# PaddlePaddle/PaddleRec

Measured on AMD Instinct MI355X. Metric: CTR samples/sec, Criteo DeepFM bs=65536 (train step: fwd+bwd+optimizer), higher is better.
Workload: dtype f32 (MLP GEMMs: f32 operands as 3 bf16 terms, 6 bf16 MFMAs per product, f32 accumulate); 1 GPU; DeepFM full Criteo: 26 sparse slots x 1000000 rows x dim 16, 13 dense, MLP 400,400,400, batch 65536 per GPU, lazy Adam, uniform ids; global_batch=65536, parallelism=single, table_rows_total=26000000, index_oob_flag=0

## Files before the change

include/recengine.h:

```cpp
#ifndef RECENGINE_H_
#define RECENGINE_H_

#include <stddef.h>
#include <stdint.h>

#ifdef __cplusplus
extern "C" {
#endif

typedef enum {
  REC_OK = 0,
  REC_EINVAL = -1,
  REC_ESHAPE = -2,
  REC_EWORKSPACE = -3,
  REC_EHIP = -4,
  REC_ENCCL = -5
} rec_status;

#define REC_FLAG_INDEX_OOB 1
#define REC_FLAG_EXCHANGE_OVERFLOW 2

const char* rec_last_error(void);
int rec_version(void);

// ... 220 lines not shown

int rec_adam_rows_all_l2(int64_t num_rows, int32_t emb_dim, int32_t row_stride, int32_t state_stride,
                         const int32_t* n_uniq, const int64_t* uniq_rows, const int32_t* seg_offset,
                         const int32_t* sorted_pos, const float* grad, const rec_grad_layout* grad_layout,
                         const float* grad_scale, float* P, float* M, float* V, const rec_adam_hyper* hyper,
                         float l2_coeff, void* stream);

int rec_adam_record_all(int64_t num_rows, int32_t emb_dim, int32_t rec_stride, int32_t state_stride,
                        int32_t v_offset, const int32_t* n_uniq, const int64_t* uniq_rows,
                        const int32_t* seg_offset, const int32_t* sorted_pos, const float* grad,
                        const rec_grad_layout* grad_layout, const float* grad1,
                        const rec_grad_layout* grad1_layout, const float* grad_scale, float* rec, float* MV,
                        const rec_adam_hyper* hyper, void* stream);

int rec_adam_dense(int64_t n, float* p, float* m, float* v, const float* g, const float* grad_scale,
                   const rec_adam_hyper* hyper, void* stream);

int rec_sumsq_workspace_bytes(size_t* bytes);
int rec_sumsq(int64_t n, const float* x, float* out, int32_t accumulate, void* workspace,
              size_t workspace_bytes, void* stream);
int rec_sparse_rows_sumsq(int64_t n_max, int32_t emb_dim, const int32_t* n_uniq,
                          const int32_t* seg_offset, const int32_t* sorted_pos, const float* grad,
                          const rec_grad_layout* grad_layout, float* out, int32_t accumulate,
                          void* workspace, size_t workspace_bytes, void* stream);
int rec_clip_scale(const float* sumsq, float clip_norm, float* scale, void* stream);

int rec_cross_bwd_prep(int64_t m, int32_t n, const float* dX, int32_t ld_dx, const float* X0,
                       int32_t ld_x0, const float* U, int32_t ld_u, float* dU, int32_t ld_du,
                       float* dX0_acc, int32_t ld_acc, int32_t accumulate, void* stream);

typedef struct {
  int64_t batch;
  int32_t max_len;
  int32_t item_dim, cat_dim;
  int32_t hidden1, hidden2;
  int64_t item_rows, cat_rows;
  int32_t item_stride, cat_stride;
} rec_din_desc;

int rec_din_saves_act1(const rec_din_desc* desc);
int rec_din_attention_pool_fwd(const rec_din_desc* desc, const int64_t* hist_item,
                               const int64_t* hist_cat, const int64_t* tgt_item_seq,
                               const int64_t* tgt_cat_seq, const int64_t* mask,
                               const float* w_hist_item, const float* w_hist_cat,
                               const float* w_tgt_item_seq, const float* w_tgt_cat_seq,
                               const float* att_w1, const float* att_b1, const float* att_w2,
                               const float* att_b2, const float* att_w3, const float* att_b3,
                               float* out, float* att_weight, float* act1, int32_t* status, void* stream);
int rec_din_attention_pool_fwd_workspace_bytes(const rec_din_desc* desc, size_t* bytes);
int rec_din_attention_pool_fwd_ws(const rec_din_desc* desc, const int64_t* hist_item,
                                  const int64_t* hist_cat, const int64_t* tgt_item_seq,
                                  const int64_t* tgt_cat_seq, const int64_t* mask,
                                  const float* w_hist_item, const float* w_hist_cat,
                                  const float* w_tgt_item_seq, const float* w_tgt_cat_seq,
                                  const float* att_w1, const float* att_b1, const float* att_w2,
                                  const float* att_b2, const float* att_w3, const float* att_b3,
                                  float* out, float* att_weight, float* act1, int32_t* status, void* workspace,
                                  size_t workspace_bytes, void* stream);

int rec_din_attention_pool_bwd(const rec_din_desc* desc, const int64_t* hist_item,
                               const int64_t* hist_cat, const int64_t* tgt_item_seq,
                               const int64_t* tgt_cat_seq, const float* w_hist_item,
                               const float* w_hist_cat, const float* w_tgt_item_seq,
                               const float* w_tgt_cat_seq, const float* att_w1,
                               const float* att_w1_t, const float* att_b1, const float* att_w2,
                               const float* att_b2, const float* att_w3, const float* att_weight,
                               const float* out_saved, const float* act1_saved,
                               const float* d_out, float* d_hist, float* d_tgt_seq, void* stream);

int rec_din_attention_pool_bwd_workspace_bytes(const rec_din_desc* desc, size_t* bytes);
int rec_din_attention_pool_bwd_ws(const rec_din_desc* desc, const int64_t* hist_item,
                                  const int64_t* hist_cat, const int64_t* tgt_item_seq,
                                  const int64_t* tgt_cat_seq, const float* w_hist_item,
                                  const float* w_hist_cat, const float* w_tgt_item_seq,
                                  const float* w_tgt_cat_seq, const float* att_w1,
                                  const float* att_w1_t, const float* att_b1, const float* att_w2,
                                  const float* att_b2, const float* att_w3, const float* att_weight,
                                  const float* out_saved, const float* act1_saved,
                                  const float* d_out, float* d_hist, float* d_tgt_seq, void* workspace,
                                  size_t workspace_bytes, void* stream);

int rec_moe_bwd_prep(int64_t m, int32_t n, const float* dX, int32_t ld_dx, const float* X0,
                     int32_t ld_x0, const float* U, int32_t ld_u, const float* prob, int32_t prob_stride,
                     float* dU, int32_t ld_du, float* dX0_acc, int32_t ld_acc, int32_t accumulate,
                     float* dp, int32_t dp_stride, void* stream);
int rec_softmax_rows_bwd(int64_t m, int32_t n, const float* p, int32_t ldp, const float* dp,
                         int32_t lddp, float* dz, int32_t lddz, void* stream);

int rec_softmax_rows(int64_t m, int32_t n, const float* x, int32_t ldx, float* y, int32_t ldy,
                     void* stream);

typedef struct {
  int64_t stride_b;
  int32_t stride_j, stride_d;
} rec_cin_view;

int rec_cin_outer_fwd(int64_t batch, int32_t emb_dim, int32_t F, int32_t S, const float* X0,
                      const rec_cin_view* v0, const float* Xk, const rec_cin_view* vk, float* Z, int64_t ldz,
                      void* stream);
int rec_cin_outer_bwd(int64_t batch, int32_t emb_dim, int32_t F, int32_t S, const float* dZ, int64_t ldz,
                      const float* X0, const rec_cin_view* v0, const float* Xk, const rec_cin_view* vk,
                      float* dX0, const rec_cin_view* dv0, int32_t accumulate_dx0, float* dXk,
                      const rec_cin_view* dvk, int32_t accumulate_dxk, const float* dpool, int64_t ld_dpool,
                      void* stream);
int rec_cin_contract_fwd(int64_t batch, int32_t emb_dim, int32_t F, int32_t C, const float* Y, int64_t ldy,
                         const float* X0, const rec_cin_view* v0, float* XT, int64_t ldx, void* stream);
int rec_cin_contract_bwd(int64_t batch, int32_t emb_dim, int32_t F, int32_t C, const float* Y, int64_t ldy,
                         const float* dXT, int64_t ldx, const float* X0, const rec_cin_view* v0, float* dY,
                         int64_t lddy, float* dX0, const rec_cin_view* dv0, int32_t accumulate_dx0, void* stream);
int rec_cin_sumpool(int64_t batch, int32_t emb_dim, int32_t C, const float* XT, int64_t ldx, float* out,
                    int64_t ldo, void* stream);
int rec_cin_sumpool_bwd(int64_t batch, int32_t emb_dim, int32_t C, const float* dpool, int64_t ldp,
                        float* dXT, int64_t ldx, void* stream);

int rec_batchnorm_workspace_bytes(int64_t m, int32_t n, size_t* bytes);
int rec_batchnorm_fwd(int64_t m, int32_t n, const float* X, int64_t ldx, const float* gamma, const float* beta,
                      float* running_mean, float* running_var, float momentum, float eps, int32_t training,
                      float* Y, int64_t ldy, float* save_mean, float* save_invstd, void* workspace,
                      size_t workspace_bytes, void* stream);
int rec_batchnorm_bwd(int64_t m, int32_t n, const float* X, int64_t ldx, const float* dY, int64_t lddy,
                      const float* gamma, const float* save_mean, const float* save_invstd, int32_t relu_mask,
                      float* dX, int64_t lddx, float* dgamma, float* dbeta, void* workspace,
                      size_t workspace_bytes, void* stream);
int rec_dot_interact_fwd(int64_t batch, int32_t F, int32_t D, const float* T, int64_t ldt, float* R, int64_t ldr,
                         void* stream);
int rec_dot_interact_bwd(int64_t batch, int32_t F, int32_t D, const float* T, int64_t ldt, const float* dR,
                         int64_t ldr, float* dT, int64_t lddt, void* stream);
int rec_accuracy_count(int64_t n, const float* pred, const int64_t* label, int64_t* counts, void* stream);

typedef enum {
  REC_EPI_NONE = 0,
  REC_EPI_BIAS = 1,
  REC_EPI_BIAS_RELU = 2,
  REC_EPI_RELU_MASK = 3,
  REC_EPI_CROSS = 4,
  REC_EPI_BIAS_SIGMOID = 5,
  REC_EPI_BIAS_TANH = 6,
  REC_EPI_ADD = 7,
  REC_EPI_DTANH = 10,
  REC_EPI_DSIGMOID = 9,
  REC_EPI_MOE = 8
} rec_epilogue;

typedef struct {
  int64_t m;
  int32_t n, k;
  int32_t lda, ldb, ldc;
  int32_t trans_a, trans_b;
  int32_t epilogue;
  int32_t split_k;
  int32_t num_cus;
} rec_gemm_desc;

typedef struct {
  const float* bias;
  const float* aux0;
  int32_t ld_aux0;
  const float* aux1;
  int32_t ld_aux1;
  const float* row_scale;
  int32_t row_scale_stride;
  float* out2;
  int32_t ld_out2;
  float* b_colsum;
  const void* b_image;
  void* relu_bits;
} rec_gemm_epilogue_args;

int rec_gemm_f32_workspace_bytes(const rec_gemm_desc* desc, size_t* bytes);
int rec_gemm_relu_bits_bytes(const rec_gemm_desc* desc, int32_t* eligible, size_t* bytes);
int rec_gemm_plan_splits(const rec_gemm_desc* desc, int32_t num_cus, int32_t* splits);
int rec_gemm_f32(const rec_gemm_desc* desc, const float* A, const float* B, float* C,
                 const rec_gemm_epilogue_args* args , void* workspace,
                 size_t workspace_bytes, void* stream);
int rec_gemm_f32_pair(const rec_gemm_desc* desc0, const float* A0, const float* B0, float* C0,
                      const rec_gemm_epilogue_args* args0 , const rec_gemm_desc* desc1, const float* A1,
                      const float* B1, float* C1, const rec_gemm_epilogue_args* args1 , void* workspace,
                      size_t workspace_bytes, void* stream);
typedef enum {
  REC_GEMM_ROUTE_SKINNY_ROWS = 0,
  REC_GEMM_ROUTE_SKINNY_DW = 1,
  REC_GEMM_ROUTE_X3_DW = 2,
  REC_GEMM_ROUTE_X3 = 3,
  REC_GEMM_ROUTE_PANEL = 4,
  REC_GEMM_ROUTE_GLDS = 5,
  REC_GEMM_ROUTE_DIRECT = 6,
  REC_GEMM_ROUTE_TILED = 7
} rec_gemm_route_family;
enum {
  REC_GEMM_ROUTE_FAST = 1,
  REC_GEMM_ROUTE_PIPE = 2,
  REC_GEMM_ROUTE_VEC = 4,
  REC_GEMM_ROUTE_KS4 = 8,
  REC_GEMM_ROUTE_FOLD = 16,
  REC_GEMM_ROUTE_VEC_A = 32,
  REC_GEMM_ROUTE_PAIR = 64
};
typedef struct {
  int32_t family;
  int32_t cfg;
  int32_t splits;
  int32_t flags;
} rec_gemm_route;
int rec_gemm_last_route(rec_gemm_route* out);
typedef struct {
  const float* B;
  int32_t ldb, k, n, trans_b;
  void* image;
} rec_gemm_b_image;
int rec_gemm_b_image_bytes(int32_t k, int32_t n, int32_t* eligible, size_t* bytes);
int rec_gemm_b_images(int32_t count, const rec_gemm_b_image* items, void* stream);

int rec_colsum_workspace_bytes(int64_t m, int32_t n, size_t* bytes);
int rec_colsum(int64_t m, int32_t n, int32_t ld, const float* G, float* out, void* workspace,
               size_t workspace_bytes, void* stream);

typedef struct {
  int64_t batch;
  int32_t d;
  int32_t ld_x0, ld_xl, ld_out, ld_u;
} rec_crossnet_v2_desc;
int rec_crossnet_v2_layer_workspace_bytes(const rec_crossnet_v2_desc* desc, size_t* fwd_bytes, size_t* bwd_bytes);
int rec_crossnet_v2_layer_fwd(const rec_crossnet_v2_desc* desc, const float* X0, const float* Xl, const float* W,
                              const float* bias, float* Xnext, float* U_saved, void* workspace,
                              size_t workspace_bytes, void* stream);
int rec_crossnet_v2_layer_bwd(const rec_crossnet_v2_desc* desc, const float* X0, const float* Xl, const float* W,
                              const float* U_saved, const float* dXnext, int32_t ld_dxnext, float* dX0_acc,
                              int32_t ld_acc, int32_t accumulate_dx0, int32_t fold_dx0, float* dXl,
                              int32_t ld_dxl, float* dW, float* db, void* workspace, size_t workspace_bytes,
                              void* stream);

typedef struct {
  int64_t batch;
  int32_t d, rank, experts;
  int32_t ld_x0, ld_xl, ld_out;
} rec_crossnet_mix_desc;
int rec_crossnet_mix_layer_workspace_bytes(const rec_crossnet_mix_desc* desc, size_t* fwd_bytes, size_t* bwd_bytes);
int rec_crossnet_mix_layer_fwd(const rec_crossnet_mix_desc* desc, const float* X0, const float* Xl, const float* U,
                               const float* V, const float* C, const float* bias, const float* gate_w,
                               const float* gate_b, float* Xnext, float* t1, float* t2, float* prob,
                               void* workspace, size_t workspace_bytes, void* stream);
int rec_crossnet_mix_layer_bwd(const rec_crossnet_mix_desc* desc, const float* X0, const float* Xl, const float* U,
                               const float* V, const float* C, const float* bias, const float* gate_w,
                               const float* t1, const float* t2, const float* prob, const float* dXnext,
                               int32_t ld_dxnext, float* dX0_acc, int32_t ld_acc, int32_t accumulate_dx0,
                               int32_t fold_dx0, float* dXl, int32_t ld_dxl, float* gU, float* gV, float* gC,
                               float* gbias, float* g_gate_w, float* g_gate_b, int32_t accumulate_gate,
                               void* workspace, size_t workspace_bytes, void* stream);

int rec_logloss_workspace_bytes(int64_t batch, size_t* bytes);
int rec_sigmoid_logloss(int64_t batch, int64_t mean_over, const float* y1, const float* y2,
                        const float* y_dnn,
                        const int64_t* label, float eps, float clip_lo, float clip_hi, float* pred,
                        float* dz, float* loss_out, void* workspace, size_t workspace_bytes, void* stream);

int rec_bce_with_logits(int64_t batch, int64_t mean_over, const float* logit, const float* label,
                        float* pred, float* dz, float* loss_out, void* workspace, size_t workspace_bytes,
                        void* stream);

int rec_auc_histogram(int64_t batch, const float* pred, const int64_t* label,
                      int32_t num_thresholds, int64_t* stat_pos, int64_t* stat_neg, void* stream);

int rec_shard_route_workspace_bytes(int64_t n, int32_t num_shards, size_t* bytes);
int rec_shard_route(int64_t n, int32_t num_slots, int64_t num_rows, int64_t padding_idx,
                    int32_t num_shards, const int64_t* ids, const int64_t* slot_offset,
                    int64_t* send_local_row, int64_t* send_pos, int64_t* send_sample,
                    int64_t* slot_of_pos, int64_t* send_counts, int32_t* status, void* workspace,
                    size_t workspace_bytes, void* stream);

int rec_dedup_plan_workspace_bytes(int64_t n, int32_t num_shards, int64_t local_rows, size_t* bytes);
int rec_dedup_plan(int64_t n, int32_t num_slots, int64_t num_rows, int64_t padding_idx, int32_t num_shards,
                   int64_t local_rows, int32_t cap, const int64_t* ids, const int64_t* slot_offset, int32_t* sorted_pos,
                   int64_t* uniq_rows, int32_t* seg_offset, int32_t* n_uniq, int64_t* send_rows, int64_t* slot_of_pos,
                   int64_t* slot_of_uniq, int64_t* counts, int32_t* status, void* workspace, size_t workspace_bytes,
                   void* stream);

int rec_comm_unique_id(void* id128);
int rec_comm_init(const void* id128, int32_t world, int32_t rank, void** comm);
int rec_comm_destroy(void* comm);
int rec_comm_size(void* comm, int32_t* world);
int rec_comm_available(void);
int rec_alltoall_exchange(void* comm, const void* send, const int64_t* send_counts, void* recv,
                          const int64_t* recv_counts, int32_t row_bytes, void* stream);
int rec_allreduce_sum_f32(void* comm, float* buf, int64_t n, void* stream);

uint32_t rec_xxh32(const void* bytes, size_t len, uint32_t seed);
int rec_xxh32_hash_mod(const char* const* strings, const int32_t* field_idx, int64_t n,
                       uint32_t hash_dim, int64_t* out);

int rec_count_lines(const char* buf, size_t len, int32_t threads, int64_t* n_lines);
int rec_blank_lines(const char* buf, size_t len, int32_t threads, int64_t max_out, int64_t* idx, int64_t* n_blank);
int rec_csr_cut(int32_t num_slots, int32_t n_pieces, const int64_t* const* values, const int64_t* const* lod,
                const int64_t* lod_stride, const int64_t* const* base, const int64_t* l0, const int64_t* l1,
                int32_t threads, int64_t* out_values, int64_t max_values, int64_t* out_lod, int64_t* out_base);
int rec_count_byte(const char* buf, size_t len, int32_t byte, int32_t threads, int64_t* n);
int rec_parse_slot_text(const char* buf, size_t len, int32_t n_sparse, int32_t n_dense,
                        int32_t log1p_dense, int64_t max_lines, int32_t threads, int64_t* label,
                        int64_t* ids, float* dense, int64_t* n_lines);
int rec_parse_criteo_tsv(const char* buf, size_t len, int32_t n_dense, int32_t n_sparse,
                         const float* cont_min, const float* cont_diff, uint32_t hash_dim,
                         int64_t max_lines, int32_t threads, int64_t* label, int64_t* ids, float* dense,
                         int64_t* n_lines);

int rec_parse_feasign_slots(const char* buf, size_t len, int32_t first_slot, int32_t num_slots,
                            uint64_t hash_rows, int64_t max_lines, int64_t max_values, int32_t threads,
                            int64_t* values, int64_t* lod, int64_t* slot_base, int64_t* n_lines,
                            int64_t* n_values);

int rec_fill_uniform(int64_t n, float* buf, float lo, float hi, uint64_t seed, void* stream);

int rec_copy_async(void* dst, const void* src, size_t bytes, void* stream);
int rec_copy_2d_async(void* dst, size_t dst_pitch_bytes, const void* src, size_t src_pitch_bytes, size_t width_bytes,
                      size_t rows, void* stream);
int rec_transpose_f32(int64_t rows, int64_t cols, const float* in, float* out, void* stream);
int rec_cast_f32_i64(int64_t n, const float* src, int64_t src_stride, int64_t* dst, void* stream);

int rec_link_emulate(size_t bytes, float gbytes_per_s, float fixed_us, int32_t blocks, const void* src, void* dst,
                     size_t ring_bytes, void* stream);

int rec_stream_spin(int32_t micros, void* stream);
// ... 324 lines not shown
```

paddlerec_amd/_lib.py:

```python
import ctypes as C
import os

_HERE = os.path.dirname(os.path.abspath(__file__))
LIB_PATH = os.path.join(_HERE, "librecengine.so")

REC_FLAG_INDEX_OOB = 1
REC_FLAG_EXCHANGE_OVERFLOW = 2
REC_FLEN_MAX_GROUPS = 8
REC_AUTOFIS_MAX_FIELDS, REC_AUTOFIS_MAX_DIM, REC_AUTOFIS_MAX_PAIRS = 64, 64, 2016


class RecError(RuntimeError):
    pass


class DeepFMDesc(C.Structure):
    _fields_ = [("batch", C.c_int64), ("num_slots", C.c_int32), ("num_dense", C.c_int32),
                ("emb_dim", C.c_int32), ("row_stride", C.c_int32), ("num_rows", C.c_int64),
                ("padding_idx", C.c_int64), ("w1_stride", C.c_int32), ("compact_dense", C.c_int32),
                ("feat_stride", C.c_int64)]


class FFMDesc(C.Structure):
    _fields_ = [("batch", C.c_int64), ("num_slots", C.c_int32), ("num_dense", C.c_int32), ("dim", C.c_int32),
                ("num_rows", C.c_int64), ("row_stride", C.c_int32), ("grad_stride", C.c_int32)]


class FatFFMDesc(C.Structure):
    _fields_ = [("ffm", FFMDesc), ("ld_attn", C.c_int64), ("ld_pair", C.c_int64)]


class FEFMDesc(C.Structure):
    _fields_ = [("batch", C.c_int64), ("num_slots", C.c_int32), ("num_dense", C.c_int32), ("dim", C.c_int32),
                ("num_rows", C.c_int64), ("row_stride", C.c_int32), ("grad_stride", C.c_int32), ("ld", C.c_int64)]


class DcnCrossDesc(C.Structure):
    _fields_ = [("batch", C.c_int64), ("d", C.c_int32), ("num_layers", C.c_int32), ("ld_x0", C.c_int64),
                ("ld_out", C.c_int64), ("ld_dxl", C.c_int64), ("ld_dx0", C.c_int64), ("l2_coeff", C.c_float),
                ("accumulate_dx0", C.c_int32)]


class DeepFMNet(C.Structure):
    MAX_LINEAR = 8
    _fields_ = [("num_slots", C.c_int32), ("dim", C.c_int32), ("dense_dim", C.c_int32), ("n_linear", C.c_int32),
                ("widths", C.c_int32 * 8), ("table_rows", C.c_int64), ("num_rows", C.c_int64),
                ("padding_idx", C.c_int64), ("slot_rows", C.c_int64), ("slot_offset", C.c_void_p),
                ("rec", C.c_void_p), ("rec_stride", C.c_int32), ("mv", C.c_void_p), ("mv_stride", C.c_int32),
                ("v_offset", C.c_int32), ("dense_w", C.c_void_p), ("dense_w_one", C.c_void_p),
                ("g_dense_w", C.c_void_p), ("g_dense_w_one", C.c_void_p), ("w", C.c_void_p * 8), ("b", C.c_void_p * 8),
                ("gw", C.c_void_p * 8), ("gb", C.c_void_p * 8), ("flat_param", C.c_void_p), ("flat_grad", C.c_void_p),
                ("flat_m", C.c_void_p), ("flat_v", C.c_void_p), ("flat_numel", C.c_int64), ("w0_folded", C.c_void_p),
                ("layer0_width", C.c_int32)]


class DinNet(C.Structure):
    _fields_ = ([("item_dim", C.c_int32), ("cat_dim", C.c_int32), ("item_rows", C.c_int64), ("cat_rows", C.c_int64),
                 ("att_hidden1", C.c_int32), ("att_hidden2", C.c_int32), ("mlp_hidden1", C.c_int32),
                 ("mlp_hidden2", C.c_int32)] +
                [(n, C.c_void_p) for n in (
                    "w_hist_item", "w_hist_cat", "w_tgt_item_seq", "w_tgt_cat_seq", "w_tgt_item", "w_tgt_cat", "w_item_b",
                    "att_w1", "att_w1_t", "att_b1", "att_w2", "att_b2", "att_w3", "att_b3",
                    "w_con", "b_con", "w_l0", "b_l0", "w_l1", "b_l1", "w_l2", "b_l2",
                    "g_w_con", "g_b_con", "g_w_l0", "g_b_l0", "g_w_l1", "g_b_l1", "g_w_l2", "g_b_l2",
                    "flat_param", "flat_grad")] + [("flat_numel", C.c_int64)])


DCN_MAX_LAYERS = 8


class DcnV2Net(C.Structure):
    _fields_ = ([("num_slots", C.c_int32), ("dim", C.c_int32), ("dense_dim", C.c_int32), ("num_rows", C.c_int64),
                 ("padding_idx", C.c_int64), ("emb_stride", C.c_int32), ("state_stride", C.c_int32),
                 ("emb", C.c_void_p), ("emb_m", C.c_void_p), ("emb_v", C.c_void_p),
                 ("cross_num", C.c_int32), ("n_dnn", C.c_int32), ("widths", C.c_int32 * DCN_MAX_LAYERS),
                 ("is_stacked", C.c_int32), ("low_rank_mix", C.c_int32), ("num_experts", C.c_int32),
                 ("low_rank", C.c_int32), ("dropout_rate", C.c_float), ("l2_dnn", C.c_float), ("clip_norm", C.c_float),
                 ("dropout_seed", C.c_uint64)] +
                [(n, C.c_void_p) for n in ("dense_emb_w", "dense_emb_b", "g_dense_emb_w", "g_dense_emb_b")] +
                [(n, C.c_void_p * DCN_MAX_LAYERS) for n in ("cross_w", "cross_b", "g_cross_w", "g_cross_b", "mix_u", "mix_v", "mix_c",
                                                "mix_bias", "g_mix_u", "g_mix_v", "g_mix_c", "g_mix_bias")] +
                [(n, C.c_void_p) for n in ("gate_w", "gate_b", "g_gate_w", "g_gate_b")] +
                [(n, C.c_void_p * DCN_MAX_LAYERS) for n in ("dnn_w", "dnn_b", "g_dnn_w", "g_dnn_b")] +
                [(n, C.c_void_p) for n in ("fc_w", "fc_b", "g_fc_w", "g_fc_b", "flat_param", "flat_grad", "flat_m",
                                           "flat_v")] + [("flat_numel", C.c_int64)])


class AdamHyper(C.Structure):
    _fields_ = [("lr", C.c_float), ("beta1", C.c_float), ("beta2", C.c_float), ("eps", C.c_float),
                ("step", C.c_int64)]


class AdagradHyper(C.Structure):
    _fields_ = [("lr", C.c_float), ("initial_g2sum", C.c_float), ("min_bound", C.c_float),
                ("max_bound", C.c_float)]


class GradLayout(C.Structure):
    _fields_ = [("div", C.c_int32), ("group", C.c_int32), ("group_stride", C.c_int64),
                ("partials", C.c_void_p), ("index", C.c_void_p), ("sorted", C.c_int32)]


class SmallSgdJob(C.Structure):
    _fields_ = [("n", C.c_int64), ("emb_dim", C.c_int32), ("row_stride", C.c_int32), ("num_rows", C.c_int64),
                ("padding_idx", C.c_int64), ("ids", C.c_void_p), ("grad", C.c_void_p), ("grad_layout", GradLayout),
                ("P", C.c_void_p)]


class CinView(C.Structure):
    _fields_ = [("stride_b", C.c_int64), ("stride_j", C.c_int32), ("stride_d", C.c_int32)]


class PsAccessor(C.Structure):
    _fields_ = [("lr", C.c_float), ("initial_g2sum", C.c_float), ("min_bound", C.c_float), ("max_bound", C.c_float),
                ("initial_range", C.c_float),
                ("x_lr", C.c_float), ("x_initial_g2sum", C.c_float), ("x_min_bound", C.c_float),
                ("x_max_bound", C.c_float), ("x_initial_range", C.c_float),
                ("embedx_threshold", C.c_float), ("nonclk_coeff", C.c_float), ("click_coeff", C.c_float),
                ("grad_scale", C.c_float), ("show_scale", C.c_int32), ("embed_zero_init", C.c_int32),
                ("seed", C.c_uint64), ("row_mul", C.c_int64), ("row_add", C.c_int64)]


class LazyInit(C.Structure):
    _fields_ = [("state_offset", C.c_int32), ("init_dims", C.c_int32), ("init_range", C.c_float),
                ("seed", C.c_uint64), ("row_mul", C.c_int64), ("row_add", C.c_int64)]


class PsLayout(C.Structure):
    _fields_ = [("row_stride", C.c_int32), ("embed_off", C.c_int32), ("embedx_off", C.c_int32),
                ("embedx_dim", C.c_int32), ("stat_off", C.c_int32)]


class GradSrc(C.Structure):
    _fields_ = [("grad", C.c_void_p), ("layout", GradLayout), ("pitch", C.c_int32), ("col", C.c_int32)]


class MultislotDesc(C.Structure):
    _fields_ = [("batch", C.c_int64), ("num_slots", C.c_int32), ("emb_dim", C.c_int32),
                ("row_stride", C.c_int32), ("key_mode", C.c_int32), ("num_rows", C.c_int64),
                ("padding_idx", C.c_int64), ("lod_stride", C.c_int64), ("out_stride", C.c_int64),
                ("state_offset", C.c_int32), ("init_dims", C.c_int32), ("init_range", C.c_float),
                ("init_seed", C.c_uint64)]


class DinDesc(C.Structure):
    _fields_ = [("batch", C.c_int64), ("max_len", C.c_int32), ("item_dim", C.c_int32),
                ("cat_dim", C.c_int32), ("hidden1", C.c_int32), ("hidden2", C.c_int32),
                ("item_rows", C.c_int64), ("cat_rows", C.c_int64), ("item_stride", C.c_int32),
                ("cat_stride", C.c_int32)]


class CrossV2Desc(C.Structure):
    _fields_ = [("batch", C.c_int64), ("d", C.c_int32), ("ld_x0", C.c_int32), ("ld_xl", C.c_int32),
                ("ld_out", C.c_int32), ("ld_u", C.c_int32)]


class CrossMixDesc(C.Structure):
    _fields_ = [("batch", C.c_int64), ("d", C.c_int32), ("rank", C.c_int32), ("experts", C.c_int32),
                ("ld_x0", C.c_int32), ("ld_xl", C.c_int32), ("ld_out", C.c_int32)]


class GemmDesc(C.Structure):
    _fields_ = [("m", C.c_int64), ("n", C.c_int32), ("k", C.c_int32), ("lda", C.c_int32),
                ("ldb", C.c_int32), ("ldc", C.c_int32), ("trans_a", C.c_int32),
                ("trans_b", C.c_int32), ("epilogue", C.c_int32), ("split_k", C.c_int32), ("num_cus", C.c_int32)]


class GemmEpilogueArgs(C.Structure):
    _fields_ = [("bias", C.c_void_p), ("aux0", C.c_void_p), ("ld_aux0", C.c_int32),
                ("aux1", C.c_void_p), ("ld_aux1", C.c_int32), ("row_scale", C.c_void_p),
                ("row_scale_stride", C.c_int32), ("out2", C.c_void_p), ("ld_out2", C.c_int32),
                ("b_colsum", C.c_void_p), ("b_image", C.c_void_p), ("relu_bits", C.c_void_p)]


class GemmRoute(C.Structure):
    _fields_ = [("family", C.c_int32), ("cfg", C.c_int32), ("splits", C.c_int32), ("flags", C.c_int32)]


GEMM_ROUTE_FAMILIES = ("skinny_rows", "skinny_dw", "x3_dw", "x3", "panel", "glds", "direct", "tiled")
GEMM_ROUTE_FLAGS = dict(fast=1, pipe=2, vec=4, ks4=8, fold=16, vec_a=32, pair=64)
GEMM_CFGS = ("128x80", "256x80", "256x128", "128x128", "80x80", "64x80", "128x80_o4", "144x80")


class GemmBImage(C.Structure):
    _fields_ = [("B", C.c_void_p), ("ldb", C.c_int32), ("k", C.c_int32), ("n", C.c_int32), ("trans_b", C.c_int32),
                ("image", C.c_void_p)]


EPI = dict(none=0, bias=1, bias_relu=2, relu_mask=3, cross=4, bias_sigmoid=5, bias_tanh=6, add=7, moe=8,
           dsigmoid=9, dtanh=10)

_P = C.c_void_p
_I64, _I32, _F, _SZ = C.c_int64, C.c_int32, C.c_float, C.c_size_t

SIGNATURES = {
    "rec_last_error": (C.c_char_p, []),
    "rec_version": (C.c_int, []),
    "rec_deepfm_fm_fwd": (C.c_int, [C.POINTER(DeepFMDesc)] + [_P] * 13),
    "rec_deepfm_fm_bwd_workspace_bytes": (C.c_int, [C.POINTER(DeepFMDesc), C.POINTER(_SZ)]),
    "rec_deepfm_fm_bwd": (C.c_int, [C.POINTER(DeepFMDesc)] + [_P] * 11 + [_SZ, _P]),
    "rec_deepfm_fm_bwd_sorted": (C.c_int, [C.POINTER(DeepFMDesc)] + [_P] * 12 + [_SZ, _P]),
    "rec_ffm_fwd": (C.c_int, [C.POINTER(FFMDesc)] + [_P] * 10),
    "rec_ffm_bwd_workspace_bytes": (C.c_int, [C.POINTER(FFMDesc), C.POINTER(_SZ)]),
    "rec_ffm_bwd": (C.c_int, [C.POINTER(FFMDesc)] + [_P] * 9 + [_SZ, _P, _P]),
    "rec_fatffm_pool_fwd": (C.c_int, [C.POINTER(FatFFMDesc)] + [_P] * 7),
    "rec_fatffm_inter_fwd": (C.c_int, [C.POINTER(FatFFMDesc)] + [_P] * 9),
    "rec_fatffm_attn_bwd": (C.c_int, [C.POINTER(FatFFMDesc)] + [_P] * 10),
    "rec_fatffm_bwd_workspace_bytes": (C.c_int, [C.POINTER(FatFFMDesc), C.POINTER(_SZ)]),
    "rec_fatffm_bwd": (C.c_int, [C.POINTER(FatFFMDesc)] + [_P] * 11 + [_SZ, _P, _P]),
    "rec_fefm_fwd_workspace_bytes": (C.c_int, [C.POINTER(FEFMDesc), C.POINTER(_SZ)]),
    "rec_fefm_fwd": (C.c_int, [C.POINTER(FEFMDesc)] + [_P] * 11 + [_SZ, _P, _P]),
    "rec_fefm_bwd_workspace_bytes": (C.c_int, [C.POINTER(FEFMDesc), _I32, C.POINTER(_SZ)]),
    "rec_fefm_bwd": (C.c_int, [C.POINTER(FEFMDesc)] + [_P] * 10 + [_SZ, _P, _P]),
    "rec_dcn_cross_bwd_workspace_bytes": (C.c_int, [C.POINTER(DcnCrossDesc), C.POINTER(_SZ)]),
    "rec_dcn_cross_fwd": (C.c_int, [C.POINTER(DcnCrossDesc)] + [_P] * 7 + [_SZ, _P]),
    "rec_dcn_cross_bwd": (C.c_int, [C.POINTER(DcnCrossDesc)] + [_P] * 11 + [_SZ, _P]),
    "rec_gate_emb_fwd": (C.c_int, [_I64, _I32, _I32, _I32, _I64, _I64, _P, _P, _P, _P, _I64, _P, _P]),
    "rec_gate_emb_bwd_workspace_bytes": (C.c_int, [_I64, _I32, C.POINTER(_SZ)]),
    "rec_gate_emb_bwd": (C.c_int, [_I64, _I32, _I32, _I32, _I64, _I64, _P, _P, _P, _P, _I64, _P, _P, _P, _SZ, _P]),
    "rec_gate_hidden_fwd": (C.c_int, [_I64, _I32, _P, _I64, _P, _I64, _P, _I64, _P]),
    "rec_gate_hidden_bwd": (C.c_int, [_I64, _I32, _P, _I64, _P, _I64, _P, _I64, _P, _I64, _P, _I64, _P]),
    "rec_relu_mask_inplace": (C.c_int, [_I64, _I32, _P, _I64, _P, _I64, _P]),
    "rec_flen_fwd": (C.c_int, [_I64, _I32, _I32, _I32, _I32, _I64, _P, _P, C.POINTER(C.c_int32), _P, _P, _I64, _P, _I64,
                               _P, _P, _P]),
    "rec_flen_bwd_workspace_bytes": (C.c_int, [_I64, _I32, _I32, _I32, C.POINTER(_SZ)]),
    "rec_flen_bwd": (C.c_int, [_I64, _I32, _I32, _I32, _I64, _P, C.POINTER(C.c_int32), _P, _P, _P, _I64, _P, _I64, _P, _P,
                               _P, _SZ, _P]),
    "rec_adagrad_rows": (C.c_int, [_I64, _I32, _I32, _I32, _P, _P, _P, _P, _P, C.POINTER(GradLayout), _P, _P, _F, _F, _P]),
    "rec_adagrad_dense": (C.c_int, [_I64, _P, _P, _P, _F, _F, _P]),
    "rec_autofis_plan_ints": (C.c_int, [_I32, _I32, C.POINTER(_SZ)]),
    "rec_autofis_plan": (C.c_int, [_I32, _I32, C.POINTER(C.c_int32), C.POINTER(C.c_int32), C.POINTER(C.c_int32)]),
    "rec_autofis_fwd_workspace_bytes": (C.c_int, [_I64, _I32, _I32, _I32, C.POINTER(_SZ)]),
    "rec_autofis_fwd": (C.c_int, [_I64, _I32, _I32, _I32, _I32, _I64, _P, _P, _P, _I32, C.POINTER(C.c_int32),
                                  C.POINTER(C.c_int32), _P, _P, _P, _P, _P, _P, _F, _F, _I32, _I32, _P, _I64, _P, _I64, _P,
                                  _P, _P, _P, _P, _SZ, _P]),
    "rec_autofis_bwd_workspace_bytes": (C.c_int, [_I64, _I32, _I32, _I32, C.POINTER(_SZ)]),
    "rec_autofis_bwd": (C.c_int, [_I64, _I32, _I32, _I32, C.POINTER(C.c_int32), C.POINTER(C.c_int32), _P, _P, _P, _I64, _P,
                                  _I64, _P, _P, _P, _P, _P, _P, _I64, _P, _P, _P, _P, _SZ, _P]),
    "rec_batchnorm_relu_fwd": (C.c_int, [_I64, _I32, _P, _I64, _P, _P, _P, _P, _F, _F, _I32, _P, _I64, _P, _P, _P, _SZ, _P]),
    "rec_batchnorm_relu_bwd": (C.c_int, [_I64, _I32, _P, _I64, _P, _I64, _P, _I64, _P, _P, _P, _P, _I64, _P, _P, _P, _SZ,
                                         _P]),
    "rec_grda_step": (C.c_int, [_I64, _P, _P, _P, _F, _F, _I32, _P]),
    "rec_gru_seq_fwd": (C.c_int, [_I64, _I32, _I32, _P, _P, _P, _P, _P, _P]),
    "rec_gru_seq_bwd": (C.c_int, [_I64, _I32, _I32, _P, _P, _P, _P, _P, _P, _P]),
    "rec_dien_aux_workspace_bytes": (C.c_int, [_I64, _I32, C.POINTER(_SZ)]),
    "rec_dien_aux_fwd": (C.c_int, [_I64, _I32, _I32, _I32, _P, _P, _P, _P, _P, _I32, _I64, _P, _I32, _I64, _I64, _P, _P, _P,
                                   _SZ, _P]),
    "rec_dien_aux_bwd": (C.c_int, [_I64, _I32, _I32, _I32, _P, _P, _P, _P, _P, _I32, _I64, _P, _I32, _I64, _I64, _F, _P, _P,
                                   _I32, _P, _P, _P]),
    "rec_dien_att_feat_fwd": (C.c_int, [_I64, _I32, _P, _P, _P, _P]),
    "rec_dien_att_feat_bwd": (C.c_int, [_I64, _I32, _P, _P, _P, _P, _I32, _P, _P]),
    "rec_dien_attention_seq_fwd": (C.c_int, [_I64, _I32, _I32, _P, _P, _P, _F, _P, _P, _P]),
    "rec_dien_attention_seq_bwd": (C.c_int, [_I64, _I32, _I32, _P, _P, _P, _F, _P, _P, _I32, _P]),
    "rec_dmr_prefix_pool_fwd": (C.c_int, [_I64, _I32, _I32, _P, _P, _I64, _P, _I64, _I32, _P, _P, _I64, _P, _I64, _P, _P]),
    "rec_dmr_prefix_pool_bwd": (C.c_int, [_I64, _I32, _I32, _P, _I64, _P, _I64, _I32, _P, _P, _P, _I64, _P, _I64, _P, _P,
                                          _I64, _I32, _P]),
    "rec_prelu_fwd": (C.c_int, [_I64, _I32, _P, _I64, _P, _I32, _I32, _I32, _I32, _P, _I64, _P]),
    "rec_prelu_workspace_bytes": (C.c_int, [_I64, _I32, _I32, _I32, C.POINTER(_SZ)]),
    "rec_prelu_bwd": (C.c_int, [_I64, _I32, _P, _I64, _P, _I64, _P, _I32, _I32, _I32, _I32, _P, _I64, _P, _P, _SZ, _P]),
    "rec_dmr_match_loss_workspace_bytes": (C.c_int, [_I64, _I64, _I32, C.POINTER(_SZ), C.POINTER(_SZ)]),
    "rec_dmr_match_loss_fwd": (C.c_int, [_I64, _I64, _I32, _P, _I64, _P, _I64, _P, _P, _I64, _P, _P, _P, _P, _SZ, _P]),
    "rec_dmr_match_loss_bwd": (C.c_int, [_I64, _I64, _I32, _P, _I64, _P, _I64, _P, _P, _I64, _P, _F, _P, _I64, _P, _I64,
                                         _I32, _P, _SZ, _P]),
    "rec_dmr_tail_fwd": (C.c_int, [_I64, _I32, _I32, _P, _I64, _P, _I64, _P, _P, _I64, _P, _I64, _I64, _P, _P, _I64, _P,
                                   _I64, _P, _I64, _P, _P, _P]),
    "rec_dmr_tail_bwd_match": (C.c_int, [_I64, _I32, _P, _P, _I64, _P, _P, _I64, _P, _I64, _I64, _P, _P, _P, _I64, _P]),
    "rec_dmr_tail_bwd_hist": (C.c_int, [_I64, _I32, _I32, _P, _P, _P, _I64, _P, _I64, _P, _I64, _P, _I64, _P, _I64, _P,
                                        _I64, _P, _I64, _P, _I64, _P]),
    "rec_mha_fwd": (C.c_int, [_I64, _I32, _I32, _I32, _I32, _P, _I64, _P, _I64, _P, _I64, _F, _F, C.c_uint64, C.c_uint64, _P,
                              _I64, _P, _P]),
    "rec_mha_bwd": (C.c_int, [_I64, _I32, _I32, _I32, _I32, _P, _I64, _P, _I64, _P, _I64, _F, _F, C.c_uint64, C.c_uint64, _P,
                              _I64, _P, _I64, _P, _P, _P, _I64, _P, _I64, _P, _I64, _P]),
    "rec_add_layer_norm_fwd": (C.c_int, [_I64, _I32, _P, _I64, _P, _I64, _F, _P, _I64, _I64, _I64, _P, _P, _P]),
    "rec_add_layer_norm_bwd": (C.c_int, [_I64, _I32, _P, _I64, _I64, _I64, _P, _P, _I64, _P, _I64, _P]),
    "rec_leaky_relu_fwd": (C.c_int, [_I64, _I32, _P, _I64, _F, _P, _I64, _P]),
    "rec_leaky_relu_bwd": (C.c_int, [_I64, _I32, _P, _I64, _P, _I64, _F, _P, _I64, _P]),
    "rec_bst_add": (C.c_int, [_I64, _I64, _P, _I64, _P, _I64, _P, _I64, _P]),
    "rec_bst_embed_fwd": (C.c_int, [_I64, _I32, C.POINTER(_P), C.POINTER(_I64), C.POINTER(_P), C.POINTER(_I64),
                                    C.POINTER(_I32), _P, _I64, _P, _I64, _P, _P]),
    "rec_bst_embed_bwd": (C.c_int, [_I64, _I32, C.POINTER(_I32), _P, _I64, C.POINTER(_P), _P]),
    "rec_bst_possum_fwd": (C.c_int, [_I64, _I32, _P, _P, _P, _P]),
    "rec_bst_possum_bwd": (C.c_int, [_I64, _I32, _P, _P, _P, _P]),
    "rec_dense_fold_fwd": (C.c_int, [_I32, _I32, _I32, _I32, _P, _P, _P, _P]),
    "rec_dense_fold_bwd": (C.c_int, [_I32, _I32, _I32, _I32, _P, _P, _P, _P, _P, _I32, _P]),
    "rec_dense_fold_fwd_full": (C.c_int, [_I32, _I32, _I32, _I32, _P, _P, _P, _P]),
    "rec_dense_fold_bwd_full": (C.c_int, [_I32, _I32, _I32, _I32, _P, _P, _P, _P, _P, _I32, _P]),
    "rec_emb_gather": (C.c_int, [_I64, _I32, _I32, _I64, _I64, _P, _P, _P, _I32, _I64, _P, _P]),
    "rec_emb_gather_sumpool": (C.c_int, [_I64, _I32, _I32, _I64, _I64, _P, _P, _P, _P, _P, _P, _P]),
    "rec_emb_sumpool_bwd": (C.c_int, [_I64, _I32, _P, _P, _P, _P]),
    "rec_ids_group_workspace_bytes": (C.c_int, [_I64, _I64, C.POINTER(_SZ)]),
    "rec_ids_group": (C.c_int, [_I64, _I32, _I64, _I64, _P, _P, _P, _P, _P, _P, _P, _P, _SZ, _P]),
    "rec_ids_group_payload": (C.c_int, [_I64, _I32, _I64, _I64, _P, _P, _P, _P, _P, _P, _P, _P, _P, _SZ, _P]),
    "rec_ids_group_slots_workspace_bytes": (C.c_int, [_I64, _I32, _I64, C.POINTER(_SZ)]),
    "rec_ids_group_slots": (C.c_int, [_I64, _I32, _I64, _I64, _P, _P, _P, _P, _P, _P, _P, _P, _SZ, _P]),
    "rec_ids_rank": (C.c_int, [_I64, _P, _P, _P, _P]),
    "rec_segment_partials_bytes": (C.c_int, [_I64, _I32, C.POINTER(C.c_size_t)]),
    "rec_segment_partials": (C.c_int, [_I64, _I32, _P, _P, _P, _P, C.POINTER(GradLayout), _P, _P]),
    "rec_sparse_adam_rows": (C.c_int, [_I64, _I32, _I32, _I32, _P, _P, _P, _P, _P, C.POINTER(GradLayout), _P,
                                       _P, _P, _P, C.POINTER(AdamHyper), _P]),
    "rec_sparse_adam_rows_l2": (C.c_int, [_I64, _I32, _I32, _I32, _P, _P, _P, _P, _P, C.POINTER(GradLayout), _P,
                                          _P, _P, _P, C.POINTER(AdamHyper), _F, _P]),
    "rec_sparse_adam_record": (C.c_int, [_I64, _I32, _I32, _I32, _I32, _P, _P, _P, _P, _P, C.POINTER(GradLayout), _P,
                                         C.POINTER(GradLayout), _P, _P, _P, C.POINTER(AdamHyper), _P]),
    "rec_adam_record_all": (C.c_int, [_I64, _I32, _I32, _I32, _I32, _P, _P, _P, _P, _P, C.POINTER(GradLayout), _P,
                                      C.POINTER(GradLayout), _P, _P, _P, C.POINTER(AdamHyper), _P]),
    "rec_multislot_sumpool_fwd": (C.c_int, [C.POINTER(MultislotDesc)] + [_P] * 10),
    "rec_multislot_sumpool_bwd": (C.c_int, [C.POINTER(MultislotDesc), _I64, _P, _P, _P, _P]),
    "rec_feasign_rows": (C.c_int, [_I64, _I64, _P, _P, _P]),
    "rec_feasign_rows_host": (C.c_int, [_I64, _I64, _P, _P]),
    "rec_record_gather": (C.c_int, [_I64, _I32, _I32, _I64, _P, _P, _P, _P, C.POINTER(LazyInit), _P, _P]),
    "rec_dedup_plan_workspace_bytes": (C.c_int, [_I64, _I32, _I64, C.POINTER(_SZ)]),
    "rec_dedup_plan": (C.c_int, [_I64, _I32, _I64, _I64, _I32, _I64, _I32] + [_P] * 11 + [_P, _SZ, _P]),
    "rec_link_emulate": (C.c_int, [_SZ, _F, _F, _I32, _P, _P, _SZ, _P]),
    "rec_comm_unique_id": (C.c_int, [_P]),
    "rec_comm_init": (C.c_int, [_P, _I32, _I32, C.POINTER(C.c_void_p)]),
    "rec_comm_destroy": (C.c_int, [_P]),
    "rec_comm_size": (C.c_int, [_P, C.POINTER(C.c_int32)]),
    "rec_comm_available": (C.c_int, []),
    "rec_alltoall_exchange": (C.c_int, [_P, _P, C.POINTER(_I64), _P, C.POINTER(_I64), _I32, _P]),
    "rec_allreduce_sum_f32": (C.c_int, [_P, _P, _I64, _P]),
    "rec_ps_push_rows": (C.c_int, [_I64, _I32, C.POINTER(PsLayout), _P, _P, _P, _P, C.POINTER(GradSrc),
                                   C.POINTER(GradSrc), _P, _P, _P, C.POINTER(PsAccessor), _P]),
    "rec_ps_init_value_host": (C.c_float, [C.c_uint64, _I64, _I32, _F]),
    "rec_ps_shrink_rows": (C.c_int, [_I64, C.POINTER(PsLayout), _P, _F, _F, _F, C.POINTER(PsAccessor), _P, _P]),
    "rec_ps_save_select": (C.c_int, [_I64, C.POINTER(PsLayout), _P, _I32, _F, _F, _F, C.POINTER(PsAccessor), _P, _P,
                                     _P]),
    "rec_sparse_adagrad_rows": (C.c_int, [_I64, _I32, _I32, _I32, _P, _P, _P, _P, _P, C.POINTER(GradLayout), _P,
                                          _P, C.POINTER(AdagradHyper), _P]),
    "rec_adam_rows_all": (C.c_int, [_I64, _I32, _I32, _I32, _P, _P, _P, _P, _P, C.POINTER(GradLayout), _P,
                                    _P, _P, _P, C.POINTER(AdamHyper), _P]),
    "rec_adam_rows_all_l2": (C.c_int, [_I64, _I32, _I32, _I32, _P, _P, _P, _P, _P, C.POINTER(GradLayout), _P,
                                       _P, _P, _P, C.POINTER(AdamHyper), _F, _P]),
    "rec_adam_dense": (C.c_int, [_I64, _P, _P, _P, _P, _P, C.POINTER(AdamHyper), _P]),
    "rec_sumsq_workspace_bytes": (C.c_int, [C.POINTER(_SZ)]),
    "rec_sumsq": (C.c_int, [_I64, _P, _P, _I32, _P, _SZ, _P]),
    "rec_sparse_rows_sumsq": (C.c_int, [_I64, _I32, _P, _P, _P, _P, C.POINTER(GradLayout), _P, _I32, _P,
                                        _SZ, _P]),
    "rec_clip_scale": (C.c_int, [_P, _F, _P, _P]),
    "rec_mlp_head_bwd_workspace_bytes": (C.c_int, [_I64, _I32, C.POINTER(C.c_size_t)]),
    "rec_mlp_head_bwd": (C.c_int, [_I64, _I32, _P, _I64, _P, _P, _I32, _P, _I64, _P, _P, _P, _SZ, _P]),
    "rec_dropout": (C.c_int, [_I64, _I32, _I64, _I64, _P, _P, _F, C.c_uint64, C.c_uint64, C.c_uint64, _I32, _P]),
    "rec_l2_decay_grad": (C.c_int, [_I64, _P, _P, _F, _P, _P]),
    "rec_din_saves_act1": (C.c_int, [C.POINTER(DinDesc)]),
    "rec_din_attention_pool_fwd": (C.c_int, [C.POINTER(DinDesc)] + [_P] * 20),
    "rec_din_attention_pool_fwd_workspace_bytes": (C.c_int, [C.POINTER(DinDesc), C.POINTER(C.c_size_t)]),
    "rec_din_attention_pool_fwd_ws": (C.c_int, [C.POINTER(DinDesc)] + [_P] * 20 + [_SZ, _P]),
    "rec_din_attention_pool_bwd": (C.c_int, [C.POINTER(DinDesc)] + [_P] * 21),
    "rec_din_attention_pool_bwd_workspace_bytes": (C.c_int, [C.POINTER(DinDesc), C.POINTER(C.c_size_t)]),
    "rec_din_attention_pool_bwd_ws": (C.c_int, [C.POINTER(DinDesc)] + [_P] * 21 + [_SZ, _P]),
    "rec_sparse_sgd_rows": (C.c_int, [_I64, _I32, _I32, _P, _P, _P, _P, _P, C.POINTER(GradLayout), _P, _F, _P]),
    "rec_sgd_dense": (C.c_int, [_I64, _P, _P, _F, _P]),
    "rec_crossnet_v2_layer_workspace_bytes": (C.c_int, [C.POINTER(CrossV2Desc), C.POINTER(_SZ), C.POINTER(_SZ)]),
    "rec_crossnet_v2_layer_fwd": (C.c_int, [C.POINTER(CrossV2Desc), _P, _P, _P, _P, _P, _P, _P, _SZ, _P]),
    "rec_crossnet_v2_layer_bwd": (C.c_int, [C.POINTER(CrossV2Desc), _P, _P, _P, _P, _P, _I32, _P, _I32, _I32, _I32, _P,
                                            _I32, _P, _P, _P, _SZ, _P]),
    "rec_crossnet_mix_layer_workspace_bytes": (C.c_int, [C.POINTER(CrossMixDesc), C.POINTER(_SZ), C.POINTER(_SZ)]),
    "rec_crossnet_mix_layer_fwd": (C.c_int, [C.POINTER(CrossMixDesc)] + [_P] * 13 + [_SZ, _P]),
    "rec_crossnet_mix_layer_bwd": (C.c_int, [C.POINTER(CrossMixDesc)] + [_P] * 11 + [_I32, _P, _I32, _I32, _I32, _P, _I32]
                                   + [_P] * 6 + [_I32, _P, _SZ, _P]),
    "rec_sparse_sgd_small": (C.c_int, [_I64, _I32, _I32, _I64, _I64, _P, _P, C.POINTER(GradLayout), _P, _F, _P, _P]),
    "rec_sparse_sgd_small_multi": (C.c_int, [_I32, C.POINTER(SmallSgdJob), _F, _P, _P]),
    "rec_sparse_adam_record_small": (C.c_int, [_I64, _I32, _I32, _I32, _I32, _I32, _I64, _I64, _P, _P, _P, C.POINTER(GradLayout),
                                               _P, C.POINTER(GradLayout), _P, _P, _P, C.POINTER(AdamHyper), _P, _P, _P]),
    "rec_bce_with_logits": (C.c_int, [_I64, _I64, _P, _P, _P, _P, _P, _P, _SZ, _P]),
    "rec_moe_bwd_prep": (C.c_int, [_I64, _I32, _P, _I32, _P, _I32, _P, _I32, _P, _I32, _P, _I32, _P, _I32, _I32,
                                   _P, _I32, _P]),
    "rec_softmax_rows_bwd": (C.c_int, [_I64, _I32, _P, _I32, _P, _I32, _P, _I32, _P]),
    "rec_softmax_rows": (C.c_int, [_I64, _I32, _P, _I32, _P, _I32, _P]),
    "rec_batchnorm_workspace_bytes": (C.c_int, [_I64, _I32, C.POINTER(_SZ)]),
    "rec_batchnorm_fwd": (C.c_int, [_I64, _I32, _P, _I64, _P, _P, _P, _P, _F, _F, _I32, _P, _I64, _P, _P, _P, _SZ, _P]),
    "rec_batchnorm_bwd": (C.c_int, [_I64, _I32, _P, _I64, _P, _I64, _P, _P, _P, _I32, _P, _I64, _P, _P, _P, _SZ, _P]),
    "rec_dot_interact_fwd": (C.c_int, [_I64, _I32, _I32, _P, _I64, _P, _I64, _P]),
    "rec_dot_interact_bwd": (C.c_int, [_I64, _I32, _I32, _P, _I64, _P, _I64, _P, _I64, _P]),
    "rec_accuracy_count": (C.c_int, [_I64, _P, _P, _P, _P]),
    "rec_cin_outer_fwd": (C.c_int, [_I64, _I32, _I32, _I32, _P, C.POINTER(CinView), _P, C.POINTER(CinView), _P, _I64, _P]),
    "rec_cin_outer_bwd": (C.c_int, [_I64, _I32, _I32, _I32, _P, _I64, _P, C.POINTER(CinView), _P, C.POINTER(CinView),
                                    _P, C.POINTER(CinView), _I32, _P, C.POINTER(CinView), _I32, _P, _I64, _P]),
    "rec_cin_contract_fwd": (C.c_int, [_I64, _I32, _I32, _I32, _P, _I64, _P, C.POINTER(CinView), _P, _I64, _P]),
    "rec_cin_contract_bwd": (C.c_int, [_I64, _I32, _I32, _I32, _P, _I64, _P, _I64, _P, C.POINTER(CinView), _P, _I64,
                                       _P, C.POINTER(CinView), _I32, _P]),
    "rec_cin_sumpool": (C.c_int, [_I64, _I32, _I32, _P, _I64, _P, _I64, _P]),
    "rec_cin_sumpool_bwd": (C.c_int, [_I64, _I32, _I32, _P, _I64, _P, _I64, _P]),
    "rec_cross_bwd_prep": (C.c_int, [_I64, _I32, _P, _I32, _P, _I32, _P, _I32, _P, _I32, _P, _I32, _I32, _P]),
    "rec_logloss_workspace_bytes": (C.c_int, [_I64, C.POINTER(_SZ)]),
    "rec_sigmoid_logloss": (C.c_int, [_I64, _I64, _P, _P, _P, _P, _F, _F, _F, _P, _P, _P, _P, _SZ, _P]),
    "rec_auc_histogram": (C.c_int, [_I64, _P, _P, _I32, _P, _P, _P]),
    "rec_shard_route_workspace_bytes": (C.c_int, [_I64, _I32, C.POINTER(_SZ)]),
    "rec_shard_route": (C.c_int, [_I64, _I32, _I64, _I64, _I32] + [_P] * 9 + [_SZ, _P]),
    "rec_gemm_f32_workspace_bytes": (C.c_int, [C.POINTER(GemmDesc), C.POINTER(_SZ)]),
    "rec_gemm_last_route": (C.c_int, [C.POINTER(GemmRoute)]),
    "rec_gemm_plan_splits": (C.c_int, [C.POINTER(GemmDesc), _I32, C.POINTER(_I32)]),
    "rec_gemm_relu_bits_bytes": (C.c_int, [C.POINTER(GemmDesc), C.POINTER(_I32), C.POINTER(_SZ)]),
    "rec_gemm_b_image_bytes": (C.c_int, [_I32, _I32, C.POINTER(_I32), C.POINTER(_SZ)]),
    "rec_gemm_b_images": (C.c_int, [_I32, C.POINTER(GemmBImage), _P]),
    "rec_gemm_f32": (C.c_int, [C.POINTER(GemmDesc), _P, _P, _P, C.POINTER(GemmEpilogueArgs), _P, _SZ, _P]),
    "rec_gemm_f32_pair": (C.c_int, [C.POINTER(GemmDesc), _P, _P, _P, C.POINTER(GemmEpilogueArgs), C.POINTER(GemmDesc), _P, _P,
                                    _P, C.POINTER(GemmEpilogueArgs), _P, _SZ, _P]),
    "rec_colsum_workspace_bytes": (C.c_int, [_I64, _I32, C.POINTER(_SZ)]),
    "rec_colsum": (C.c_int, [_I64, _I32, _I32, _P, _P, _P, _SZ, _P]),
    "rec_xxh32": (C.c_uint32, [C.c_char_p, _SZ, C.c_uint32]),
    "rec_xxh32_hash_mod": (C.c_int, [C.POINTER(C.c_char_p), C.POINTER(_I32), _I64, C.c_uint32,
                                     C.POINTER(_I64)]),
    "rec_count_lines": (C.c_int, [C.c_char_p, _SZ, _I32, C.POINTER(_I64)]),
    "rec_blank_lines": (C.c_int, [C.c_char_p, _SZ, _I32, _I64, _P, C.POINTER(_I64)]),
    "rec_count_byte": (C.c_int, [C.c_char_p, _SZ, _I32, _I32, C.POINTER(_I64)]),
    "rec_csr_cut": (C.c_int, [_I32, _I32, _P, _P, _P, _P, _P, _P, _I32, _P, _I64, _P, _P]),
    "rec_parse_slot_text": (C.c_int, [C.c_char_p, _SZ, _I32, _I32, _I32, _I64, _I32, _P, _P, _P,
                                      C.POINTER(_I64)]),
    "rec_parse_criteo_tsv": (C.c_int, [C.c_char_p, _SZ, _I32, _I32, _P, _P, C.c_uint32, _I64, _I32, _P, _P, _P,
                                       C.POINTER(_I64)]),
    "rec_parse_feasign_slots": (C.c_int, [C.c_char_p, _SZ, _I32, _I32, C.c_uint64, _I64, _I64, _I32, _P, _P, _P,
                                          C.POINTER(_I64), C.POINTER(_I64)]),
    "rec_fill_uniform": (C.c_int, [_I64, _P, _F, _F, C.c_uint64, _P]),
    "rec_stream_spin": (C.c_int, [_I32, _P]),
    "rec_copy_async": (C.c_int, [_P, _P, _SZ, _P]),
    "rec_copy_2d_async": (C.c_int, [_P, _SZ, _P, _SZ, _SZ, _SZ, _P]),
    "rec_transpose_f32": (C.c_int, [_I64, _I64, _P, _P, _P]),
    "rec_cast_f32_i64": (C.c_int, [_I64, _P, _I64, _P, _P]),
    "rec_stream_create_cu_range": (C.c_int, [_I32, _I32, C.POINTER(C.c_void_p)]),
    "rec_stream_create_cu_stride": (C.c_int, [_I32, _I32, _I32, C.POINTER(C.c_void_p)]),
    "rec_ctr_head_workspace_bytes": (C.c_int, [_I64, _I32, C.POINTER(C.c_size_t)]),
    "rec_ctr_head_fwd_bwd": (C.c_int, [_I64, _I32, _I64, _P, _I64, _P, _P, _P, _P, _P, C.c_float, C.c_float, C.c_float,
                                       _I32, _P, _P, _P, _P, _P, _I64, _P, _P, _P, _SZ, _P]),
    "rec_din_train_step_workspace_bytes": (C.c_int, [C.POINTER(DinNet), _I64, _I32, C.POINTER(C.c_size_t)]),
    "rec_din_train_step": (C.c_int, [C.POINTER(DinNet), _I64, _I32, _P, _P, _P, _P, _P, _P, _P, _P, _F, _P, _P, _P, _P,
                                     _SZ, _P, _P]),
    "rec_dcn_v2_train_step_workspace_bytes": (C.c_int, [C.POINTER(DcnV2Net), _I64, C.POINTER(C.c_size_t)]),
    "rec_dcn_v2_train_step": (C.c_int, [C.POINTER(DcnV2Net), _I64, _P, _P, _P, C.POINTER(AdamHyper), _P, _P, _I32, _P, _P,
                                        _P, _P, _SZ, _P]),
    "rec_deepfm_train_step_workspace_bytes": (C.c_int, [C.POINTER(DeepFMNet), _I64, C.POINTER(C.c_size_t)]),
    "rec_deepfm_train_step": (C.c_int, [C.POINTER(DeepFMNet), _I64, _P, _P, _P, C.POINTER(AdamHyper), _P, _P, _I32, _P, _P,
                                        _P, _P, _SZ, _P, _P]),
    "rec_stream_destroy": (C.c_int, [_P]),
}

_lib = None


def lib():
    global _lib
    if _lib is None:
        if not os.path.exists(LIB_PATH):
            raise RecError(
                "librecengine.so not found at %s — run `python -m paddlerec_amd.build` "
                "(there is no CPU fallback)" % LIB_PATH)
        import torch
        h = C.CDLL(LIB_PATH)
        for name, (res, args) in SIGNATURES.items():
            fn = getattr(h, name)
            fn.restype, fn.argtypes = res, args
        _lib = h
    return _lib


def check(rc, what=""):
    if rc != 0:
        msg = lib().rec_last_error().decode("utf-8", "replace")
        raise RecError("%s failed (rc=%d): %s" % (what or "recengine call", rc, msg))
```

paddlerec_amd/csrc/deepfm_step.hip:

```cpp
#include <stdlib.h>

#include <map>
#include <mutex>
#include <tuple>

#include "rec_common.h"
#include "tail_roles.h"

using namespace rec;

namespace {

struct Carve {
  char* base;
  size_t off = 0;
  explicit Carve(void* p) : base((char*)p) {}
  template <class T>
  T* take(size_t count) {
    T* p = base ? (T*)(base + off) : nullptr;
    off += align_up(count * sizeof(T), 256);
    return p;
  }
  void* bytes(size_t n) { return take<char>(n); }
};

struct Shape {
  int S, D, Dn, n;
  bool compact;
  int fp;
  int in0;
  int in0_real;
  bool pad;
  int in0_full;
  int max_w;
  bool small;
  bool head;
  bool ctr_head;
};

int shape_of(const rec_deepfm_net* net, int64_t B, Shape* s) {
  REC_REQUIRE(net, REC_EINVAL, "net is NULL");
  REC_REQUIRE(net->num_slots > 0 && net->dim > 0 && net->dense_dim >= 0 && net->n_linear >= 1 &&
                  net->n_linear <= REC_DEEPFM_MAX_LINEAR, REC_EINVAL, "bad net sizes");
  REC_REQUIRE(B > 0 && B * net->num_slots < (1ll << 31), REC_EINVAL, "bad batch");
  REC_REQUIRE(net->widths[net->n_linear - 1] == 1, REC_EINVAL, "the last Linear must have one output (net.py:150)");
  s->S = net->num_slots; s->D = net->dim; s->Dn = net->dense_dim; s->n = net->n_linear;
  s->compact = s->Dn > 0 && s->Dn <= s->D;
  s->fp = s->compact ? s->S + 1 : s->S + s->Dn;
  s->in0_real = s->fp * s->D;
  s->pad = !s->compact && net->layer0_width > s->in0_real;
  REC_REQUIRE(net->layer0_width == 0 || s->pad || net->layer0_width == s->in0_real, REC_EINVAL,
              "layer0_width %d: a padded width needs a net without the dense fold and >= %d", net->layer0_width,
              s->in0_real);
  REC_REQUIRE(!s->pad || net->layer0_width % 4 == 0, REC_EINVAL, "layer0_width must be a multiple of 4");
  s->in0 = s->pad ? net->layer0_width : s->in0_real;
  s->in0_full = (s->S + s->Dn) * s->D;
  s->max_w = s->in0;
  for (int i = 0; i < s->n; ++i) {
    REC_REQUIRE(net->widths[i] > 0, REC_EINVAL, "bad layer width");
    if (net->widths[i] > s->max_w) s->max_w = net->widths[i];
  }
  static const bool small_env = [] { const char* v = getenv("REC_SMALL_MERGE"); return !(v && *v == '0'); }();
  s->small = small_env && B * s->S <= 15360;
  static const bool head_env = [] { const char* v = getenv("REC_MLP_HEAD_FUSED"); return !(v && *v == '0'); }();
  const int nh = s->n > 1 ? net->widths[s->n - 2] : 0;
  s->head = head_env && s->n > 1 && nh % 4 == 0 && nh <= 512 && B >= 64 &&
            ((uintptr_t)net->w[s->n - 1]) % 16 == 0;
  static const bool ctr_env = [] { const char* v = getenv("REC_CTR_HEAD_FUSED"); return !(v && *v == '0'); }();
  s->ctr_head = ctr_env && s->n > 1 && nh % 4 == 0 && nh <= 512 && ((uintptr_t)net->w[s->n - 1]) % 16 == 0;
  return REC_OK;
}

struct Buffers {
  float *y1, *y2, *feat, *sum_emb, *act[REC_DEEPFM_MAX_LINEAR], *y_dnn, *dz, *g[2], *row_grad, *dm;
  float *pp, *pp1, *dw0p;
  int32_t* small_scratch;
  int32_t *sorted_pos, *seg_offset, *n_uniq;
  int64_t* uniq_rows;
  void* ws;
  size_t ws_bytes;
  void* ws_head;
  size_t ws_head_bytes;
  void* ws_side;
  size_t ws_side_bytes;
  void* img_f[REC_DEEPFM_MAX_LINEAR];
  void* img_t[REC_DEEPFM_MAX_LINEAR];
  void* relu_bits[REC_DEEPFM_MAX_LINEAR];
};

int call_workspace(const rec_deepfm_net* net, const Shape& s, int64_t B, size_t* out) {
  size_t need = 0, b = 0;
  auto up = [&](size_t x) { if (x > need) need = x; };
  rec_gemm_desc d{};
  auto gemm_ws = [&](int64_t m, int n, int k, int ta, int tb) {
    d = rec_gemm_desc{m, n, k, 1, 1, n, ta, tb, REC_EPI_NONE, 0};
    d.lda = ta ? (int)m : k; d.ldb = tb ? k : n; d.ldc = n;
    if (rec_gemm_f32_workspace_bytes(&d, &b) == REC_OK) up(b);
  };
  int in = s.in0;
  for (int i = 0; i < s.n; ++i) {
    const int w = net->widths[i];
    gemm_ws(B, w, in, 0, 0);
    gemm_ws(B, in, w, 0, 1);
    gemm_ws(in, w, (int)B, 1, 0);
    in = w;
  }
  if (int rc = rec_logloss_workspace_bytes(B, &b)) return rc;
  up(b);
  rec_deepfm_desc fd{B, s.S, s.Dn, s.D, s.D, 1, -1, 1, s.compact ? 1 : 0};
  if (int rc = rec_deepfm_fm_bwd_workspace_bytes(&fd, &b)) return rc;
  up(b);
  if (s.head) {
    if (int rc = rec_mlp_head_bwd_workspace_bytes(B, net->widths[s.n - 2], &b)) return rc;
    up(b);
  }
  if (s.ctr_head) {
    if (int rc = rec_ctr_head_workspace_bytes(B, net->widths[s.n - 2], &b)) return rc;
    up(b);
  }
  *out = align_up(need, 256);
  return REC_OK;
}

int group_workspace(const rec_deepfm_net* net, const Shape& s, int64_t B, size_t* out) {
  size_t b = 0;
  if (net->slot_rows > 0) {
    if (int rc = rec_ids_group_slots_workspace_bytes(B, s.S, net->slot_rows, &b)) return rc;
  } else {
    if (int rc = rec_ids_group_workspace_bytes(B * s.S, net->num_rows, &b)) return rc;
  }
  *out = align_up(b, 256);
  return REC_OK;
}

int carve(const rec_deepfm_net* net, const Shape& s, int64_t B, void* workspace, Buffers* bf, size_t* total) {
  Carve c(workspace);
  const size_t n = (size_t)B * s.S;
  bf->y1 = c.take<float>(B);
  bf->y2 = c.take<float>(B);
  bf->feat = c.take<float>((size_t)B * s.in0);
  bf->sum_emb = c.take<float>((size_t)B * s.D);
  bf->act[0] = bf->feat;
  for (int i = 1; i < s.n; ++i) bf->act[i] = c.take<float>((size_t)B * net->widths[i - 1]);
  bf->y_dnn = c.take<float>(B);
  bf->dz = c.take<float>(B);
  bf->g[0] = c.take<float>((size_t)B * s.max_w);
  bf->g[1] = c.take<float>((size_t)B * s.max_w);
  bf->row_grad = c.take<float>(n * s.D);
  bf->dm = c.take<float>((size_t)(s.Dn > 0 ? s.Dn : 1) * net->widths[0]);
  bf->dw0p = (s.pad || s.compact) ? c.take<float>((size_t)s.in0 * net->widths[0]) : nullptr;
  bf->small_scratch = c.take<int32_t>(1);
  bf->pp = bf->pp1 = nullptr;
  bf->sorted_pos = bf->seg_offset = bf->n_uniq = nullptr;
  bf->uniq_rows = nullptr;
  bf->ws_side = nullptr;
  bf->ws_side_bytes = 0;
  if (!s.small) {
    size_t pb = 0, pb1 = 0;
    if (int rc = rec_segment_partials_bytes((int64_t)n, s.D, &pb)) return rc;
    if (int rc = rec_segment_partials_bytes((int64_t)n, 1, &pb1)) return rc;
    bf->pp = (float*)c.bytes(pb > 4 ? pb : 4);
    bf->pp1 = (float*)c.bytes(pb1 > 4 ? pb1 : 4);
    bf->sorted_pos = c.take<int32_t>(n);
    bf->uniq_rows = c.take<int64_t>(n);
    bf->seg_offset = c.take<int32_t>(n + 1);
    bf->n_uniq = c.take<int32_t>(4);
    size_t gw = 0;
    if (int rc = group_workspace(net, s, B, &gw)) return rc;
    bf->ws_side = c.bytes(gw);
    bf->ws_side_bytes = gw;
  }
  static const bool img_env = [] { const char* v = getenv("REC_GEMM_IMAGES"); return !(v && *v == '0'); }();
  {
    int in = s.in0;
    for (int i = 0; i < s.n; ++i) {
      bf->img_f[i] = bf->img_t[i] = nullptr;
      const int w = net->widths[i];
      if (img_env && B >= 8192) {
        int32_t ok = 0;
        size_t ib = 0;
        if (rec_gemm_b_image_bytes(in, w, &ok, &ib) == REC_OK && ok) bf->img_f[i] = c.bytes(ib);
        if (rec_gemm_b_image_bytes(w, in, &ok, &ib) == REC_OK && ok) bf->img_t[i] = c.bytes(ib);
      }
      in = w;
    }
  }
  static const bool bits_env = [] { const char* v = getenv("REC_RELU_BITS"); return !(v && *v == '0'); }();
  for (int i = 0; i < s.n; ++i) {
    bf->relu_bits[i] = nullptr;
    if (i == 0 || !bits_env) continue;
    const int wi = net->widths[i - 1], kin = i == 1 ? s.in0 : net->widths[i - 2];
    rec_gemm_desc df{B, wi, kin, kin, wi, wi, 0, 0, REC_EPI_BIAS_RELU, 0, 0};
    rec_gemm_desc db{B, wi, net->widths[i], net->widths[i], net->widths[i], wi, 0, 1, REC_EPI_RELU_MASK, 0, 0};
    int32_t okf = 0, okb = 0;
    size_t nf = 0, nb = 0;
    if (rec_gemm_relu_bits_bytes(&df, &okf, &nf) == REC_OK && rec_gemm_relu_bits_bytes(&db, &okb, &nb) == REC_OK && okf && okb &&
        nf == nb)
      bf->relu_bits[i] = c.bytes(nf);
  }
  size_t cw = 0;
  if (int rc = call_workspace(net, s, B, &cw)) return rc;
  bf->ws = c.bytes(cw);
  bf->ws_bytes = cw;
  bf->ws_head = nullptr;
  bf->ws_head_bytes = 0;
  if (s.small && s.ctr_head) {
    size_t hb = 0;
    if (int rc = rec_ctr_head_workspace_bytes(B, net->widths[s.n - 2], &hb)) return rc;
    bf->ws_head = c.bytes(hb);
    bf->ws_head_bytes = hb;
  }
  *total = c.off;
  return REC_OK;
}

int gemm(int64_t m, int n, int k, bool ta, bool tb, int epi, const float* A, const float* Bm, float* C,
         const float* bias, const float* aux0, int ld0, float* b_colsum, int split_k, const Buffers& bf, void* st,
         const void* b_image = nullptr, int num_cus = 0, void* relu_bits = nullptr) {
  rec_gemm_desc d{};
  d.num_cus = num_cus;
  d.m = m; d.n = n; d.k = k;
  d.lda = ta ? (int)m : k;
  d.ldb = tb ? k : n;
  d.ldc = n;
  d.trans_a = ta; d.trans_b = tb; d.epilogue = epi; d.split_k = split_k;
  rec_gemm_epilogue_args x{};
  x.bias = bias; x.aux0 = aux0; x.ld_aux0 = ld0; x.b_colsum = b_colsum; x.b_image = b_image; x.relu_bits = relu_bits;
  return rec_gemm_f32(&d, A, Bm, C, &x, bf.ws, bf.ws_bytes, st);
}

int linear_backward(int64_t B, int in, int w, const float* X, const float* G, const float* W, float* dW, float* db,
                    float* dX, const float* mask, const Buffers& bf, void* st, const void* b_image_t,
                    void* mask_bits = nullptr) {
  rec_gemm_desc d0{}, d1{};
  d0.m = in; d0.n = w; d0.k = (int)B; d0.lda = in; d0.ldb = w; d0.ldc = w; d0.trans_a = 1; d0.epilogue = REC_EPI_NONE;
  d1.m = B; d1.n = in; d1.k = w; d1.lda = w; d1.ldb = w; d1.ldc = in; d1.trans_b = 1;
  d1.epilogue = mask ? REC_EPI_RELU_MASK : REC_EPI_NONE;
  rec_gemm_epilogue_args x0{}, x1{};
  x0.b_colsum = db;
  x1.aux0 = mask; x1.ld_aux0 = mask ? in : 0; x1.b_image = b_image_t; x1.relu_bits = mask ? mask_bits : nullptr;
  return rec_gemm_f32_pair(&d0, X, G, dW, &x0, &d1, G, W, dX, &x1, bf.ws, bf.ws_bytes, st);
}

}

extern "C" int rec_deepfm_train_step_workspace_bytes(const rec_deepfm_net* net, int64_t batch, size_t* bytes) {
  REC_REQUIRE(bytes, REC_EINVAL, "bytes is NULL");
  Shape s;
  if (int rc = shape_of(net, batch, &s)) return rc;
  Buffers bf;
  return carve(net, s, batch, nullptr, &bf, bytes);
}

#define REC_TRY(call)            \
  do {                           \
    if (int rc_ = (call)) return rc_; \
  } while (0)

int rec::step_events(void* stream, void* side_stream, hipEvent_t** out) {
  struct Set { hipEvent_t ev[kStepEvents]; };
  static std::mutex mu;
  static std::map<std::tuple<int, void*, void*>, Set> cache;
  int dev = 0;
  REC_REQUIRE(hipGetDevice(&dev) == hipSuccess, REC_EHIP, "hipGetDevice failed");
  std::lock_guard<std::mutex> lock(mu);
  auto key = std::make_tuple(dev, stream, side_stream);
  auto it = cache.find(key);
  if (it == cache.end()) {
    Set st{};
    for (auto& e : st.ev)
      REC_REQUIRE(hipEventCreateWithFlags(&e, hipEventDisableTiming) == hipSuccess, REC_EHIP, "hipEventCreate failed");
    it = cache.emplace(key, st).first;
  }
  *out = it->second.ev;
  return REC_OK;
}

extern "C" int rec_deepfm_train_step(const rec_deepfm_net* net, int64_t batch, const int64_t* ids, const float* dense,
                                     const int64_t* label, const rec_adam_hyper* hyper, int64_t* auc_pos,
                                     int64_t* auc_neg, int32_t num_thresholds, float* loss_out, float* pred_out,
                                     int32_t* status, void* workspace, size_t workspace_bytes, void* stream,
                                     void* side_stream) {
  Shape s;
  if (int rc = shape_of(net, batch, &s)) return rc;
  REC_REQUIRE(ids && label && hyper && loss_out && pred_out && (dense || s.Dn == 0), REC_EINVAL,
              "null pointer argument");
  REC_REQUIRE(net->rec && net->mv && net->flat_param && net->flat_grad && net->flat_m && net->flat_v, REC_EINVAL,
              "net: null parameter pointer");
  REC_REQUIRE(!(s.compact || s.pad) || net->w0_folded, REC_EINVAL,
              "net: w0_folded is needed with 0 < dense_dim <= dim and with a padded layer0_width");
  REC_REQUIRE((auc_pos == nullptr) == (auc_neg == nullptr), REC_EINVAL, "auc_pos / auc_neg: both or neither");
  Buffers bf;
  size_t need = 0;
  if (int rc = carve(net, s, batch, workspace, &bf, &need)) return rc;
  REC_REQUIRE(workspace && workspace_bytes >= need, REC_EWORKSPACE, "workspace %zu < %zu", workspace_bytes, need);
  const int64_t B = batch;
  const int S = s.S, D = s.D, Dn = s.Dn, n = s.n;
  const size_t f4 = sizeof(float);

  const bool overlap = side_stream != nullptr && side_stream != stream && !s.small;
  void* sst = overlap ? side_stream : stream;
  hipEvent_t* ev = nullptr;
  if (overlap) REC_TRY(step_events(stream, side_stream, &ev));
  auto order = [&](int k, void* from, void* to) -> int {
    REC_REQUIRE(hipEventRecord(ev[k], (hipStream_t)from) == hipSuccess &&
                    hipStreamWaitEvent((hipStream_t)to, ev[k], 0) == hipSuccess, REC_EHIP, "stream ordering failed");
    return REC_OK;
  };
  const int64_t nlook = B * S;
  if (!s.small) {
    if (overlap) REC_TRY(order(0, stream, sst));
    if (net->slot_rows > 0) {
      REC_TRY(rec_ids_group_slots(B, S, net->slot_rows, net->padding_idx, ids, bf.sorted_pos, bf.uniq_rows,
                                  bf.seg_offset, bf.n_uniq, nullptr, status, bf.ws_side, bf.ws_side_bytes, sst));
    } else {
      REC_TRY(rec_ids_group_payload(nlook, S, net->num_rows, net->padding_idx, ids, net->slot_offset, nullptr,
                                    bf.sorted_pos, bf.uniq_rows, bf.seg_offset, bf.n_uniq, status, bf.ws_side,
                                    bf.ws_side_bytes, sst));
    }
  }
  rec_deepfm_desc fd{B, S, Dn, D, net->rec_stride, net->table_rows, net->padding_idx, net->rec_stride,
                     s.compact ? 1 : 0, s.pad ? (int64_t)s.in0 : 0};
  static const bool fold_ride = [] { const char* v = getenv("REC_SMALL_TAIL"); return !(v && *v == '0'); }();
  bool fold_rode = false, pad_zeroed = false;
  FoldFwd ff{};
  if (s.compact && s.small && fold_ride)
    ff = dense_fold_fwd_plan(S, Dn, D, net->widths[0], net->dense_w, net->w[0], net->w0_folded);
  ff.zero_feat_pad = s.pad && s.small && fold_ride ? 1 : 0;
  REC_TRY(deepfm_fm_fwd_fold(&fd, ids, dense, net->rec, net->rec + D, net->dense_w, net->dense_w_one, net->slot_offset,
                             bf.y1, bf.y2, bf.feat, bf.sum_emb, status, stream, ff, &fold_rode, &pad_zeroed));
  if (s.pad && !pad_zeroed)
    REC_REQUIRE(hipMemset2DAsync(bf.feat + s.in0_real, (size_t)s.in0 * f4, 0, (size_t)(s.in0 - s.in0_real) * f4,
                                 (size_t)B, (hipStream_t)stream) == hipSuccess, REC_EHIP, "hipMemset2DAsync failed");
  const float* w0 = net->w[0];
  float* gw0 = net->gw[0];
  if (s.compact) {
    if (!fold_rode)
      REC_TRY(rec_dense_fold_fwd_full(S, Dn, D, net->widths[0], net->dense_w, net->w[0], net->w0_folded, stream));
    w0 = net->w0_folded;
    gw0 = bf.dw0p;
  }
  const bool pad_copy = s.pad && net->w0_folded != net->w[0];
  if (pad_copy) {
    REC_TRY(rec_copy_async(net->w0_folded, net->w[0], (size_t)s.in0_real * net->widths[0] * f4, stream));
    w0 = net->w0_folded;
    gw0 = bf.dw0p;
  }
  const int n_fwd = s.ctr_head ? n - 1 : n;
  {
    rec_gemm_b_image items[2 * REC_DEEPFM_MAX_LINEAR];
    int cnt = 0, in = s.in0;
    for (int i = 0; i < n; ++i) {
      const int w = net->widths[i];
      const float* wi = i == 0 ? w0 : net->w[i];
      if (bf.img_f[i]) items[cnt++] = rec_gemm_b_image{wi, w, in, w, 0, bf.img_f[i]};
      if (bf.img_t[i]) items[cnt++] = rec_gemm_b_image{wi, w, w, in, 1, bf.img_t[i]};
      in = w;
    }
    if (cnt) REC_TRY(rec_gemm_b_images(cnt, items, stream));
  }
  {
    int in = s.in0;
    for (int i = 0; i < n_fwd; ++i) {
      const bool last = i == n - 1;
      float* out = last ? bf.y_dnn : bf.act[i + 1];
      REC_TRY(gemm(B, net->widths[i], in, false, false, last ? REC_EPI_BIAS : REC_EPI_BIAS_RELU, bf.act[i],
                   i == 0 ? w0 : net->w[i], out, net->b[i], nullptr, 0, nullptr, 0, bf, stream, bf.img_f[i], 0,
                   last ? nullptr : bf.relu_bits[i + 1]));
      in = net->widths[i];
    }
  }
  const float* g = bf.dz;
  int gi = 0;
  int n_run = n;
  const float* P0 = net->flat_param;
  const float* G0 = net->flat_grad;
  auto flat_pair = [&](const float* pp, const float* gg, int64_t cnt) {
    return pp && gg && pp >= P0 && pp + cnt <= P0 + net->flat_numel && pp - P0 == gg - G0;
  };
  const bool pad_copy_ = s.pad && net->w0_folded != net->w[0];
  bool tail = s.small && s.ctr_head && !pad_copy_ && small_tail_eligible(nlook, D, net->slot_offset, S) &&
              flat_pair(net->w[n - 1], net->gw[n - 1], net->widths[n - 2]) && flat_pair(net->b[n - 1], net->gb[n - 1], 1) &&
              flat_pair(net->w[0], net->gw[0], (int64_t)s.in0_full * net->widths[0]) &&
              (Dn == 0 || (flat_pair(net->dense_w, net->g_dense_w, (int64_t)Dn * D) &&
                           flat_pair(net->dense_w_one, net->g_dense_w_one, Dn)));
  int head_nblk = 0;
  float head_inv = 0.f;
  if (s.ctr_head) {
    const int nh = net->widths[n - 2];
    if (tail)
      REC_TRY(ctr_head_fwd_bwd_partial(B, nh, 0, bf.act[n - 1], nh, net->w[n - 1], net->b[n - 1], bf.y1, bf.y2, label, 1e-4f,
                                       0.f, 0.f, 1, nullptr, pred_out, bf.dz, bf.g[gi], nh, bf.ws_head, bf.ws_head_bytes,
                                       stream, &head_nblk, &head_inv));
    else
    REC_TRY(rec_ctr_head_fwd_bwd(B, nh, 0, bf.act[n - 1], nh, net->w[n - 1], net->b[n - 1], bf.y1, bf.y2, label, 1e-4f,
                                 0.f, 0.f, 1, nullptr, pred_out, bf.dz, loss_out, bf.g[gi], nh, net->gw[n - 1],
                                 net->gb[n - 1], bf.ws, bf.ws_bytes, stream));
    g = bf.g[gi];
    gi ^= 1;
    n_run = n - 1;
  } else {
    REC_TRY(rec_sigmoid_logloss(B, 0, bf.y1, bf.y2, bf.y_dnn, label, 1e-4f, 0.f, 0.f, pred_out, bf.dz, loss_out, bf.ws,
                                bf.ws_bytes, stream));
  }
  if (auc_pos) REC_TRY(rec_auc_histogram(B, pred_out, label, num_thresholds, auc_pos, auc_neg, stream));
  if (!s.ctr_head && s.head) {
    const int nh = net->widths[n - 2];
    REC_TRY(rec_mlp_head_bwd(B, nh, bf.act[n - 1], nh, bf.dz, net->w[n - 1], 1, bf.g[gi], nh, net->gw[n - 1],
                             net->gb[n - 1], bf.ws, bf.ws_bytes, stream));
    g = bf.g[gi];
    gi ^= 1;
    n_run = n - 1;
  }
  const float* g0 = nullptr;
  float* d_flat = nullptr;
  bool dw0_done = false;
  for (int i = n_run - 1; i >= 0; --i) {
    const int in = i == 0 ? s.in0 : net->widths[i - 1], w = net->widths[i];
    if (i == 0) {
      g0 = g;
      d_flat = bf.g[gi];
      if (s.small) {
        dw0_done = true;
        REC_TRY(linear_backward(B, in, w, bf.feat, g, w0, gw0, net->gb[0], d_flat, nullptr, bf, stream, bf.img_t[0]));
        break;
      }
      REC_TRY(gemm(B, in, w, false, true, REC_EPI_NONE, g, w0, d_flat, nullptr, nullptr, 0, nullptr, 0, bf, stream,
                   bf.img_t[0]));
      break;
    }
    REC_TRY(linear_backward(B, in, w, bf.act[i], g, net->w[i], net->gw[i], net->gb[i], bf.g[gi], bf.act[i], bf, stream,
                            bf.img_t[i], bf.relu_bits[i]));
    g = bf.g[gi];
    gi ^= 1;
  }
  rec_deepfm_desc bd{B, S, Dn, D, D, 1, -1, 1, s.compact ? 1 : 0, s.pad ? (int64_t)s.in0 : 0};
  int fm_nblk = 0;
  if (tail)
    REC_TRY(deepfm_fm_bwd_partial(&bd, dense, bf.feat, bf.sum_emb, d_flat, bf.dz, bf.dz, net->dense_w, bf.row_grad, bf.ws,
                                  bf.ws_bytes, stream, &fm_nblk));
  else
  REC_TRY(rec_deepfm_fm_bwd(&bd, dense, bf.feat, bf.sum_emb, d_flat, bf.dz, bf.dz, net->dense_w, bf.row_grad,
                            net->g_dense_w, net->g_dense_w_one, bf.ws, bf.ws_bytes, stream));
  rec_grad_layout gl{1, 0, 0, nullptr, nullptr, 0}, gl1{S, 0, 0, nullptr, nullptr, 0};
  if (tail) {
    TailRoles t{};
    const int nh = net->widths[n - 2], NO = net->widths[0];
    t.head_blocks = (nh + 2 + 15) / 16;
    t.head_nblk = head_nblk; t.head_n2 = nh + 2; t.head_partial = (const float*)bf.ws_head; t.head_invB = head_inv;
    t.head_dw = net->gw[n - 1]; t.head_db = net->gb[n - 1]; t.loss = loss_out;
    t.head_w_off = net->w[n - 1] - P0; t.head_b_off = net->b[n - 1] - P0;
    t.n_skip = 0;
    auto skip = [&](int64_t lo, int64_t cnt) { t.skip_lo[t.n_skip] = lo; t.skip_hi[t.n_skip] = lo + cnt; ++t.n_skip; };
    skip(t.head_w_off, nh);
    skip(t.head_b_off, 1);
    t.fm_blocks = Dn * D + Dn;
    t.fm_nblk = fm_nblk; t.fm_split = Dn * D; t.fm_partial = (const float*)bf.ws;
    t.ddw = net->g_dense_w; t.ddw1 = net->g_dense_w_one;
    if (Dn > 0) {
      t.dw_off = net->dense_w - P0; t.dw1_off = net->dense_w_one - P0;
      skip(t.dw_off, (int64_t)Dn * D);
      skip(t.dw1_off, Dn);
    }
    t.w0_off = net->w[0] - P0;
    t.f = FoldedLayer0{S, Dn, D, NO, nullptr, nullptr, nullptr, nullptr};
    t.w0_blocks = 0;
    if (s.compact) {
      t.f.dW0f = gw0; t.f.dW0 = net->gw[0]; t.f.W0 = net->w[0]; t.f.dense_w = net->dense_w;
      skip(t.w0_off, (int64_t)s.in0_full * NO);
      const int64_t we = (int64_t)S * D * NO;
      t.w0_blocks = (int)((we + 4 * 1024 - 1) / (4 * 1024));
    }
    t.flat_numel = net->flat_numel; t.flat_grad = net->flat_grad;
    t.adam.p = net->flat_param; t.adam.m = net->flat_m; t.adam.v = net->flat_v;
    t.rest_blocks = (int)((net->flat_numel + 4 * 1024 - 1) / (4 * 1024));
    if (t.rest_blocks > 256) t.rest_blocks = 256;
    REC_TRY(sparse_adam_record_small_tail(nlook, S, D, net->rec_stride, net->mv_stride, net->v_offset, net->table_rows,
                                          net->padding_idx, ids, net->slot_offset, bf.row_grad, &gl, bf.dz, &gl1, net->rec,
                                          net->mv, hyper, status, t, stream));
    return REC_OK;
  }
  if (s.small) {
    REC_TRY(rec_sparse_adam_record_small(nlook, S, D, net->rec_stride, net->mv_stride, net->v_offset, net->table_rows,
                                         net->padding_idx, ids, net->slot_offset, bf.row_grad, &gl, bf.dz, &gl1,
                                         nullptr, net->rec, net->mv, hyper, status, bf.small_scratch, stream));
  } else {
    if (overlap) REC_TRY(order(1, stream, sst));
    REC_TRY(rec_segment_partials(nlook, D, bf.n_uniq, bf.seg_offset, bf.sorted_pos, bf.row_grad, &gl, bf.pp, sst));
    REC_TRY(rec_segment_partials(nlook, 1, bf.n_uniq, bf.seg_offset, bf.sorted_pos, bf.dz, &gl1, bf.pp1, sst));
    gl.partials = bf.pp;
    gl1.partials = bf.pp1;
    REC_TRY(rec_sparse_adam_record(nlook, D, net->rec_stride, net->mv_stride, net->v_offset, bf.n_uniq, bf.uniq_rows,
                                   bf.seg_offset, bf.sorted_pos, bf.row_grad, &gl, bf.dz, &gl1, nullptr, net->rec,
                                   net->mv, hyper, sst));
  }
  static const int dw0_split = [] { const char* v = getenv("REC_DW0_SPLIT"); return v && *v ? atoi(v) : 16; }();
  static const int dw0_cus = [] { const char* v = getenv("REC_DW0_CUS"); return v && *v ? atoi(v) : 192; }();
  if (!dw0_done)
    REC_TRY(gemm(s.in0, net->widths[0], (int)B, true, false, REC_EPI_NONE, bf.feat, g0, gw0, nullptr, nullptr, 0,
                 net->gb[0], overlap && B >= 16384 ? dw0_split : 0, bf, stream, nullptr,
                 overlap && B >= 16384 ? dw0_cus : 0));
  if (s.compact)
    REC_TRY(rec_dense_fold_bwd_full(S, Dn, D, net->widths[0], net->dense_w, net->w[0], gw0, net->gw[0],
                                    net->g_dense_w, 1, stream));
  if (pad_copy) REC_TRY(rec_copy_async(net->gw[0], gw0, (size_t)s.in0_real * net->widths[0] * f4, stream));
  REC_TRY(rec_adam_dense(net->flat_numel, net->flat_param, net->flat_m, net->flat_v, net->flat_grad, nullptr, hyper,
                         stream));
  if (overlap) REC_TRY(order(2, sst, stream));
  return REC_OK;
}
```

paddlerec_amd/csrc/gemm_f32.hip:

```cpp
#include <stdlib.h>

#include "rec_common.h"

#include "gemm_epi.h"
#include "gemm_direct.h"
#include "gemm_glds.h"
#include "gemm_panel.h"
#include "gemm_pipe.h"
#include "gemm_bf16x3.h"
namespace rec {

template <int BM, int BN, int WAVES_M, int WAVES_N, int OCC, bool TA, bool TB, int EPI>
__global__ __launch_bounds__(WAVES_M* WAVES_N* kWave, (OCC * WAVES_M * WAVES_N + 3) / 4) void gemm_f32_kernel(
    int64_t M, int N, int K, const float* __restrict__ A, int64_t lda, const float* __restrict__ B,
    int64_t ldb, float* __restrict__ C, int64_t ldc, EpiArgs epi, int tiles_n, int64_t tiles_total,
    int k_chunk, bool vec_a, bool vec_b, bool fast, float* __restrict__ partial,
    float* __restrict__ colsum_partial, int splits_in_x) {
  constexpr int NTHR = WAVES_M * WAVES_N * kWave;
  constexpr int WTM = BM / WAVES_M, WTN = BN / WAVES_N;
  constexpr int MT = WTM / 16, NT = WTN / 16;
  static_assert(WTM % 16 == 0 && WTN % 16 == 0, "wave tile must be a multiple of the 16x16 MFMA tile");
  constexpr int LDA_S = TA ? BM + 4 : kBK + 4, LDB_S = BN + 4;
  constexpr int A_ELEMS = TA ? kBK * LDA_S : BM * LDA_S, B_ELEMS = kBK * LDB_S;
  extern __shared__ __attribute__((aligned(16))) float gemm_smem[];
// ... 22 lines not shown
  const int wm = wave / WAVES_N, wn = wave % WAVES_N;
  const int li = lane & 15, g = lane >> 4;

  TileLoader<BM, kBK, TA, NTHR> la;
  TileLoader<kBK, BN, TB, NTHR> lb;

  f32x4_t acc[MT][NT];
#pragma unroll
  for (int a = 0; a < MT; ++a)
#pragma unroll
    for (int b = 0; b < NT; ++b) acc[a][b] = f32x4_t{0.f, 0.f, 0.f, 0.f};

  const bool do_colsum = TA && colsum_partial != nullptr && tm == 0;
  float csum = 0.f;

  const int nkt = (k_end - k_begin + kBK - 1) / kBK;
  const bool tail = !fast || (k_end - k_begin) % kBK != 0;
  const int n_fast = fast ? (tail ? nkt - 1 : nkt) : 0;

  auto load_tile = [&](int kt, auto mode_tag) {
    constexpr int MODE = decltype(mode_tag)::value;
    const int k0 = k_begin + kt * kBK;
    la.template load<MODE>(A, lda, m0, k0, M, k_end, vec_a, tid);
    lb.template load<MODE>(B, ldb, k0, n0, k_end, N, vec_b, tid);
  };
  auto store_tile = [&](int buf) {
    la.template store<false>(As + buf * A_ELEMS, tid);
    lb.template store<TB>(Bs + buf * B_ELEMS, tid);
  };
  auto compute = [&](int cur) {
    const float* as = As + cur * A_ELEMS;
    const float* bs = Bs + cur * B_ELEMS;
    float af[MT][4], bf[NT][4];
#pragma unroll
    for (int a = 0; a < MT; ++a) {
      const int row = wm * WTM + a * 16 + li;
      if (!TA) {
        const float4 t = *reinterpret_cast<const float4*>(as + row * LDA_S + g * 4);
        af[a][0] = t.x; af[a][1] = t.y; af[a][2] = t.z; af[a][3] = t.w;
      } else {
#pragma unroll
        for (int s_ = 0; s_ < 4; ++s_) af[a][s_] = as[(g * 4 + s_) * LDA_S + row];
      }
    }
#pragma unroll
    for (int b = 0; b < NT; ++b) {
      const int col = wn * WTN + b * 16 + li;
#pragma unroll
      for (int s_ = 0; s_ < 4; ++s_) bf[b][s_] = bs[(g * 4 + s_) * LDB_S + col];
    }
#pragma unroll
    for (int s_ = 0; s_ < 4; ++s_)
#pragma unroll
      for (int a = 0; a < MT; ++a)
#pragma unroll
        for (int b = 0; b < NT; ++b)
          acc[a][b] = __builtin_amdgcn_mfma_f32_16x16x4f32(af[a][s_], bf[b][s_], acc[a][b], 0, 0, 0);
    if constexpr (TA) {
      if (do_colsum && tid < BN) {
#pragma unroll
        for (int kk = 0; kk < kBK; ++kk) csum += bs[kk * LDB_S + tid];
      }
    }
  };
  using Checked = std::integral_constant<int, 2>;
  auto steady = [&](auto mode_tag) {
    load_tile(0, mode_tag);
    store_tile(0);
    __syncthreads();
    int kt = 0;
    for (; kt + 1 < n_fast; ++kt) {
      load_tile(kt + 1, mode_tag);
      __builtin_amdgcn_sched_barrier(0);
      compute(kt & 1);
      __builtin_amdgcn_sched_barrier(0);
      store_tile((kt + 1) & 1);
      __syncthreads();
    }
    return kt;
  };
  int kt = 0;
  if (n_fast > 0) {
    const bool interior = m0 + BM <= M && n0 + BN <= N;
    kt = interior ? steady(std::integral_constant<int, 0>{}) : steady(std::integral_constant<int, 1>{});
  } else if (nkt > 0) {
    load_tile(0, Checked{});
    store_tile(0);
    __syncthreads();
  }
  for (; kt < nkt; ++kt) {
    const bool next = kt + 1 < nkt;
    if (next) load_tile(kt + 1, Checked{});
    compute(kt & 1);
    __builtin_amdgcn_sched_barrier(0);
    if (next) store_tile((kt + 1) & 1);
    __syncthreads();
  }
  if (do_colsum && tid < BN && n0 + tid < N)
    colsum_partial[(int64_t)kz * N + n0 + tid] = csum;

  float* out = partial ? partial + (int64_t)kz * M * ldc : C;
  float bj[NT];
#pragma unroll
  for (int b = 0; b < NT; ++b) {
    const int j = n0 + wn * WTN + b * 16 + li;
    bj[b] = (!partial && j < N) ? load_bias<EPI>(j, epi) : 0.f;
  }
#pragma unroll
  for (int a = 0; a < MT; ++a) {
    float x0[4][NT], x1[4][NT];
    if ((EpiUses<EPI>::aux0 || EpiUses<EPI>::aux1) && !partial) {
#pragma unroll
      for (int r = 0; r < 4; ++r) {
        const int64_t i = m0 + wm * WTM + a * 16 + g * 4 + r;
#pragma unroll
        for (int b = 0; b < NT; ++b) {
          const int j = n0 + wn * WTN + b * 16 + li;
          const bool ok = i < M && j < N;
          x0[r][b] = ok ? load_aux0<EPI>(i, j, epi) : 0.f;
          x1[r][b] = ok ? load_aux1<EPI>(i, j, epi) : 0.f;
        }
      }
    }
#pragma unroll
    for (int r = 0; r < 4; ++r) {
      const int64_t i = m0 + wm * WTM + a * 16 + g * 4 + r;
      if (i < M) {
#pragma unroll
        for (int b = 0; b < NT; ++b) {
          const int j = n0 + wn * WTN + b * 16 + li;
          if (j < N) {
            const float v = acc[a][b][r];
            out[i * ldc + j] = partial ? v : apply_epi<EPI>(v, x0[r][b], x1[r][b], bj[b], i, epi);
            if (EPI == REC_EPI_CROSS && !partial && epi.out2) epi.out2[i * epi.ld2 + j] = v + bj[b];
          }
        }
      }
    }
  }
}

__device__ __forceinline__ float colsum_fold(int N, int splits, const float* __restrict__ partial, int j) {
  float a8[8] = {0.f, 0.f, 0.f, 0.f, 0.f, 0.f, 0.f, 0.f};
  int z = 0;
  for (; z + 8 <= splits; z += 8) {
#pragma unroll
    for (int u = 0; u < 8; ++u) a8[u] += partial[(int64_t)(z + u) * N + j];
  }
  for (; z < splits; ++z) a8[z & 7] += partial[(int64_t)z * N + j];
  return ((a8[0] + a8[1]) + (a8[2] + a8[3])) + ((a8[4] + a8[5]) + (a8[6] + a8[7]));
}

template <int EPI>
__global__ __launch_bounds__(kBlock) void splitk_reduce_kernel(int64_t M, int N, int64_t ldc,
                                                               int splits,
                                                               const float* __restrict__ partial,
                                                               float* __restrict__ C, EpiArgs epi,
                                                               const float* __restrict__ cpartial,
                                                               float* __restrict__ colsum_out, int colsum_blocks) {
  const int rblocks = (int)gridDim.x - colsum_blocks;
  if ((int)blockIdx.x >= rblocks) {
    const int j = ((int)blockIdx.x - rblocks) * kBlock + threadIdx.x;
    if (j < N) colsum_out[j] = colsum_fold(N, splits, cpartial, j);
    return;
  }
  const int64_t total = M * N;
  for (int64_t e = (int64_t)blockIdx.x * kBlock + threadIdx.x; e < total;
       e += (int64_t)rblocks * kBlock) {
    const int64_t i = e / N;
    const int j = (int)(e % N);
    const float* pp = partial + i * ldc + j;
    const int64_t zs = M * ldc;
    float a8[8] = {0.f, 0.f, 0.f, 0.f, 0.f, 0.f, 0.f, 0.f};
    int z = 0;
    for (; z + 8 <= splits; z += 8) {
#pragma unroll
      for (int u = 0; u < 8; ++u) a8[u] += pp[(int64_t)(z + u) * zs];
    }
    for (; z < splits; ++z) a8[z & 7] += pp[(int64_t)z * zs];
    const float t = ((a8[0] + a8[1]) + (a8[2] + a8[3])) + ((a8[4] + a8[5]) + (a8[6] + a8[7]));
    C[i * ldc + j] = apply_epi<EPI>(t, i, j, epi);
    if (EPI == REC_EPI_CROSS && epi.out2) epi.out2[i * epi.ld2 + j] = t + epi.bias[j];
  }
}

__global__ __launch_bounds__(kBlock) void colsum_reduce_kernel(int N, int splits,
                                                               const float* __restrict__ partial,
                                                               float* __restrict__ out) {
  const int j = blockIdx.x * kBlock + threadIdx.x;
  if (j < N) out[j] = colsum_fold(N, splits, partial, j);
}

constexpr int kSkinnyN = 4;

template <int EPI>
__global__ __launch_bounds__(kBlock) void gemv_rows_kernel(int64_t M, int N, int K, const float* __restrict__ A,
                                                           int64_t lda, const float* __restrict__ B, int64_t ldb,
                                                           bool trans_b, float* __restrict__ C, int64_t ldc,
                                                           EpiArgs epi, bool vec_a) {
  extern __shared__ __attribute__((aligned(16))) float bs[];
  for (int i = threadIdx.x; i < N * K; i += kBlock) {
    const int n = i / K, k = i % K;
    bs[i] = trans_b ? B[(int64_t)n * ldb + k] : B[(int64_t)k * ldb + n];
  }
  __syncthreads();
  const int lane = threadIdx.x % kWave;
  const int64_t wpb = kBlock / kWave;
  for (int64_t i = (int64_t)blockIdx.x * wpb + threadIdx.x / kWave; i < M; i += (int64_t)gridDim.x * wpb) {
    float acc[kSkinnyN] = {0.f, 0.f, 0.f, 0.f};
    const float* a = A + i * lda;
    if (vec_a) {
      for (int k = lane * 4; k + 3 < K; k += kWave * 4) {
        const float4 x = *reinterpret_cast<const float4*>(a + k);
#pragma unroll
        for (int n = 0; n < kSkinnyN; ++n)
          if (n < N) {
            const float4 w = *reinterpret_cast<const float4*>(bs + n * K + k);
            acc[n] += x.x * w.x + x.y * w.y + x.z * w.z + x.w * w.w;
          }
      }
      for (int k = (K / 4) * 4 + lane; k < K; k += kWave)
#pragma unroll
        for (int n = 0; n < kSkinnyN; ++n)
          if (n < N) acc[n] += a[k] * bs[n * K + k];
    } else {
      for (int k = lane; k < K; k += kWave)
#pragma unroll
        for (int n = 0; n < kSkinnyN; ++n)
          if (n < N) acc[n] += a[k] * bs[n * K + k];
    }
#pragma unroll
    for (int n = 0; n < kSkinnyN; ++n)
#pragma unroll
      for (int o = kWave / 2; o > 0; o >>= 1) acc[n] += __shfl_xor(acc[n], o, kWave);
    if (lane == 0)
#pragma unroll
      for (int n = 0; n < kSkinnyN; ++n)
        if (n < N) {
          C[i * ldc + n] = apply_epi<EPI>(acc[n], i, n, epi);
          if (EPI == REC_EPI_CROSS && epi.out2) epi.out2[i * epi.ld2 + n] = acc[n] + epi.bias[n];
        }
  }
}

constexpr int kSkinnyKC = 128;
constexpr int kSkinnyMT = 4;
__global__ __launch_bounds__(kBlock) void skinny_dw_kernel(int M, int N, int64_t K, const float* __restrict__ A,
                                                           int64_t lda, const float* __restrict__ B, int64_t ldb,
                                                           int64_t ldc, float* __restrict__ partial,
                                                           float* __restrict__ colsum_partial) {
  __shared__ float bs[kSkinnyKC * kSkinnyN];
  const int64_t k0 = (int64_t)blockIdx.x * kSkinnyKC;
  const int kc = (int)((K - k0 < kSkinnyKC) ? K - k0 : kSkinnyKC);
  for (int i = threadIdx.x; i < kc * N; i += kBlock) bs[(i / N) * kSkinnyN + i % N] = B[(k0 + i / N) * ldb + i % N];
  __syncthreads();
  float acc[kSkinnyMT][kSkinnyN];
#pragma unroll
  for (int c = 0; c < kSkinnyMT; ++c)
#pragma unroll
    for (int n = 0; n < kSkinnyN; ++n) acc[c][n] = 0.f;
  for (int kb = 0; kb < kc; kb += 8) {
    float x[8][kSkinnyMT];
#pragma unroll
    for (int u = 0; u < 8; ++u) {
      const float* a = A + (k0 + kb + u) * lda;
#pragma unroll
      for (int c = 0; c < kSkinnyMT; ++c) {
        const int m = threadIdx.x + c * kBlock;
        x[u][c] = (kb + u < kc && m < M) ? a[m] : 0.f;
      }
    }
#pragma unroll
    for (int u = 0; u < 8; ++u)
#pragma unroll
      for (int c = 0; c < kSkinnyMT; ++c)
#pragma unroll
        for (int n = 0; n < kSkinnyN; ++n)
          if (n < N) acc[c][n] += x[u][c] * ((kb + u < kc) ? bs[(kb + u) * kSkinnyN + n] : 0.f);
  }
  float* out = partial + (int64_t)blockIdx.x * M * ldc;
#pragma unroll
  for (int c = 0; c < kSkinnyMT; ++c) {
    const int m = threadIdx.x + c * kBlock;
    if (m < M)
#pragma unroll
      for (int n = 0; n < kSkinnyN; ++n)
        if (n < N) out[(int64_t)m * ldc + n] = acc[c][n];
  }
  if (colsum_partial && (int)threadIdx.x < N) {
    float t = 0.f;
    for (int k = 0; k < kc; ++k) t += bs[k * kSkinnyN + threadIdx.x];
    colsum_partial[(int64_t)blockIdx.x * N + threadIdx.x] = t;
  }
}

__global__ __launch_bounds__(kBlock) void skinny_dw_narrow_kernel(int M, int N, int64_t K, const float* __restrict__ A,
                                                                  int64_t lda, const float* __restrict__ B, int64_t ldb,
                                                                  int64_t ldc, float* __restrict__ partial,
                                                                  float* __restrict__ colsum_partial) {
  __shared__ float bs[kSkinnyKC * kSkinnyN];
  __shared__ float red[kBlock * kSkinnyN];
  const int64_t k0 = (int64_t)blockIdx.x * kSkinnyKC;
  const int kc = (int)((K - k0 < kSkinnyKC) ? K - k0 : kSkinnyKC);
  for (int i = threadIdx.x; i < kc * N; i += kBlock) bs[(i / N) * kSkinnyN + i % N] = B[(k0 + i / N) * ldb + i % N];
  __syncthreads();
  const int G = kBlock / M, g = (int)threadIdx.x / M, m = (int)threadIdx.x % M;
  float acc[kSkinnyN] = {0.f, 0.f, 0.f, 0.f};
  if (g < G) {
    for (int kb = g; kb < kc; kb += 8 * G) {
      float x[8];
#pragma unroll
      for (int u = 0; u < 8; ++u) {
        const int k = kb + u * G;
        x[u] = k < kc ? A[(k0 + k) * lda + m] : 0.f;
      }
#pragma unroll
      for (int u = 0; u < 8; ++u) {
        const int k = kb + u * G;
#pragma unroll
        for (int n = 0; n < kSkinnyN; ++n)
          if (n < N && k < kc) acc[n] += x[u] * bs[k * kSkinnyN + n];
      }
    }
#pragma unroll
    for (int n = 0; n < kSkinnyN; ++n) red[threadIdx.x * kSkinnyN + n] = acc[n];
  }
  __syncthreads();
  if (g == 0) {
    for (int o = 1; o < G; ++o)
#pragma unroll
      for (int n = 0; n < kSkinnyN; ++n) acc[n] += red[(o * M + m) * kSkinnyN + n];
    float* out = partial + (int64_t)blockIdx.x * M * ldc;
#pragma unroll
    for (int n = 0; n < kSkinnyN; ++n)
      if (n < N) out[(int64_t)m * ldc + n] = acc[n];
  }
// ... 214 lines not shown
  if constexpr (kPipeCfg) {
    static const bool pipe_env = [] { const char* v = getenv("REC_GEMM_PIPE"); return !(v && *v == '0'); }();
    if (pipe_env && fast && d->m % BM == 0 && d->n % BN == 0 && d->k % kBK == 0 && d->lda < (1 << 23) &&
        d->ldb < (1 << 23)) {
      hipLaunchKernelGGL((gemm_f32_pipe_kernel<BM, BN, WM_, WN_, OCC, TA, TB, EPI>), grid, dim3(WM_ * WN_ * kWave), shmem,
                         st, d->m, d->n, d->k, A, (int64_t)d->lda, B, (int64_t)d->ldb, C, (int64_t)d->ldc, e, p.tiles_n,
                         p.tiles_total, p.k_chunk, partial, cpart, fold ? p.splits : 1);
      set_route(REC_GEMM_ROUTE_TILED, p.cfg, p.splits,
                REC_GEMM_ROUTE_FAST | REC_GEMM_ROUTE_PIPE | (fold ? REC_GEMM_ROUTE_FOLD : 0));
      return;
    }
  }
  set_route(REC_GEMM_ROUTE_TILED, p.cfg, p.splits, (fast ? REC_GEMM_ROUTE_FAST : 0) | (fold ? REC_GEMM_ROUTE_FOLD : 0));
  hipLaunchKernelGGL((gemm_f32_kernel<BM, BN, WM_, WN_, OCC, TA, TB, EPI>), grid, dim3(WM_ * WN_ * kWave),
                     shmem, st, d->m, d->n, d->k, A, (int64_t)d->lda, B, (int64_t)d->ldb, C,
                     (int64_t)d->ldc, e, p.tiles_n, p.tiles_total, p.k_chunk, vec_a, vec_b, fast, partial, cpart,
                     fold ? p.splits : 1);
}

template <bool TA, bool TB, int EPI>
static void launch_cfg(const rec_gemm_desc* d, const GemmPlan& p, const float* A, const float* B,
                       float* C, const EpiArgs& e, float* partial, float* cpart, hipStream_t st) {
  switch (p.cfg) {
    case CFG_128x80: launch_one<128, 80, 4, 1, 5, TA, TB, EPI>(d, p, A, B, C, e, partial, cpart, st); break;
    case CFG_256x80: launch_one<256, 80, 8, 1, 2, TA, TB, EPI>(d, p, A, B, C, e, partial, cpart, st); break;
    case CFG_256x128: launch_one<256, 128, 4, 2, 2, TA, TB, EPI>(d, p, A, B, C, e, partial, cpart, st); break;
    case CFG_80x80: launch_one<80, 80, 5, 1, 4, TA, TB, EPI>(d, p, A, B, C, e, partial, cpart, st); break;
    case CFG_64x80: launch_one<64, 80, 4, 1, 6, TA, TB, EPI>(d, p, A, B, C, e, partial, cpart, st); break;
    case CFG_128x80_O4: launch_one<128, 80, 4, 1, 4, TA, TB, EPI>(d, p, A, B, C, e, partial, cpart, st); break;
    case CFG_144x80:
      if constexpr (TA && !TB && EPI == REC_EPI_NONE) {
        launch_one<144, 80, 9, 1, 2, TA, TB, EPI>(d, p, A, B, C, e, partial, cpart, st);
      } else {
        launch_one<80, 80, 5, 1, 4, TA, TB, EPI>(d, p, A, B, C, e, partial, cpart, st);
      }
      break;
    default: launch_one<128, 128, 2, 2, 4, TA, TB, EPI>(d, p, A, B, C, e, partial, cpart, st); break;
  }
}

template <int EPI>
static void launch_epi(const rec_gemm_desc* d, const GemmPlan& p, const float* A, const float* B,
                       float* C, const EpiArgs& e, float* partial, float* cpart, hipStream_t st) {
  if (!d->trans_a && !d->trans_b) launch_cfg<false, false, EPI>(d, p, A, B, C, e, partial, cpart, st);
  else if (!d->trans_a && d->trans_b) launch_cfg<false, true, EPI>(d, p, A, B, C, e, partial, cpart, st);
  else if (d->trans_a && !d->trans_b) launch_cfg<true, false, EPI>(d, p, A, B, C, e, partial, cpart, st);
  else launch_cfg<true, true, EPI>(d, p, A, B, C, e, partial, cpart, st);
}

static int device_cus() {
  static const int cus = [] {
    int dev = 0, v = kNumCU;
    if (hipGetDevice(&dev) == hipSuccess) (void)hipDeviceGetAttribute(&v, hipDeviceAttributeMultiprocessorCount, dev);
    return v > 0 ? v : kNumCU;
  }();
  return cus;
}

template <int BM, int BN, bool TB>
static bool launch_glds_cfg(const rec_gemm_desc* d, const float* A, const float* B, float* C, const EpiArgs& e,
                            hipStream_t st) {
  const int tiles_n = d->n / BN;
  const int64_t tiles_total = (d->m / BM) * tiles_n;
  constexpr size_t shmem = (size_t)kGldsStages * (BM + BN) * 64;
  static_assert(shmem <= 64 * 1024, "LDS ring too large for the default dynamic-LDS limit");
  static const int cus = [] {
    int dev = 0, v = kNumCU;
    if (hipGetDevice(&dev) == hipSuccess) (void)hipDeviceGetAttribute(&v, hipDeviceAttributeMultiprocessorCount, dev);
    return v > 0 ? v : kNumCU;
  }();
  static const int bpc = [] { const char* v = getenv("REC_GEMM_GLDS_BPC"); return v && *v ? atoi(v) : 2; }();
  static const int skew = [] { const char* v = getenv("REC_GEMM_GLDS_SKEW"); return v && *v ? atoi(v) : 0; }();
  int64_t grid = (int64_t)cus * bpc;
  grid -= grid % 8;
  if (grid > tiles_total) grid = tiles_total;
#define REC_GLDS_CASE(E)                                                                                         \
  case E:                                                                                                        \
    hipLaunchKernelGGL((gemm_f32_glds_kernel<BM, BN, TB, E>), dim3((unsigned)grid), dim3(512), shmem, st,        \
                       d->m, d->n, d->k, A, (int64_t)d->lda, B, (int64_t)d->ldb, C, (int64_t)d->ldc, e, tiles_n, \
                       tiles_total, skew);                                                                       \
    return true;
  switch (d->epilogue) {
    REC_GLDS_CASE(REC_EPI_NONE)
    REC_GLDS_CASE(REC_EPI_BIAS)
    REC_GLDS_CASE(REC_EPI_BIAS_RELU)
    REC_GLDS_CASE(REC_EPI_RELU_MASK)
  }
#undef REC_GLDS_CASE
  return false;
}

static bool launch_glds(const rec_gemm_desc* d, const float* A, const float* B, float* C, const EpiArgs& e,
                        hipStream_t st) {
  static const bool on = [] { const char* v = getenv("REC_GEMM_GLDS"); return !(v && *v == '0'); }();
  if (!on || d->trans_a || d->split_k > 1 || d->m < 8192 || d->k % kBK != 0 || d->k < 2 * kBK) return false;
  if (d->lda % 4 || d->ldb % 4 || ((uintptr_t)A) % 16 || ((uintptr_t)B) % 16) return false;
  if (d->ldc % 4 || ((uintptr_t)C) % 16) return false;
  if (d->epilogue == REC_EPI_RELU_MASK && (e.ld0 % 4 || ((uintptr_t)e.aux0) % 16)) return false;
  const int e_ = d->epilogue;
  if (!(e_ == REC_EPI_NONE || e_ == REC_EPI_BIAS || e_ == REC_EPI_BIAS_RELU || e_ == REC_EPI_RELU_MASK)) return false;
  static const int bm128 = [] { const char* v = getenv("REC_GEMM_GLDS_BM"); return v && atoi(v) == 128; }();
  if (bm128 && d->n % 80 == 0 && d->m % 128 == 0)
    return d->trans_b ? launch_glds_cfg<128, 80, true>(d, A, B, C, e, st)
                      : launch_glds_cfg<128, 80, false>(d, A, B, C, e, st);
  const char* v80 = getenv("REC_GEMM_GLDS_80");
  const bool n80 = v80 && *v80 == '1';
  if (n80 && d->n % 80 == 0 && d->m % 256 == 0 && (d->m / 256) * (int64_t)(d->n / 80) < (1ll << 31))
    return d->trans_b ? launch_glds_cfg<256, 80, true>(d, A, B, C, e, st)
                      : launch_glds_cfg<256, 80, false>(d, A, B, C, e, st);
  if (d->n % 208 == 0 && d->m % 128 == 0 && (d->m / 128) * (int64_t)(d->n / 208) < (1ll << 31))
    return d->trans_b ? launch_glds_cfg<128, 208, true>(d, A, B, C, e, st)
                      : launch_glds_cfg<128, 208, false>(d, A, B, C, e, st);
  if (d->n % 144 == 0 && d->m % 128 == 0 && (d->m / 128) * (int64_t)(d->n / 144) < (1ll << 31))
    return d->trans_b ? launch_glds_cfg<128, 144, true>(d, A, B, C, e, st)
                      : launch_glds_cfg<128, 144, false>(d, A, B, C, e, st);
  return false;
}

constexpr bool kX3Default = true;
static bool x3_enabled() {
  const char* v = getenv("REC_GEMM_BF16X3");
  return v && *v ? *v != '0' : kX3Default;
}
static bool x3_eligible(const rec_gemm_desc* d) {
  if (!x3_enabled() || d->trans_a || d->split_k > 1 || d->m < 8192 || d->n % 4 || d->k % 8 || d->k < 64)
    return false;
  return x3_cols(d->n).nt > 0 && x3_epilogue_ok(d->epilogue);
}
static bool launch_x3(const rec_gemm_desc* d, const float* A, const float* B, float* C, const EpiArgs& e,
                      const void* b_image, void* workspace, size_t workspace_bytes, hipStream_t st) {
  if (!x3_eligible(d)) return false;
  if (!x3_shape_ok(d->m, d->n, d->k, d->lda, d->ldc, A, C)) return false;
  if (e.aux0 && (e.ld0 % 4 || ((uintptr_t)e.aux0) % 16)) return false;
  if (e.aux1 && (e.ld1 % 4 || ((uintptr_t)e.aux1) % 16)) return false;
  if (e.out2 && (e.ld2 % 4 || ((uintptr_t)e.out2) % 16)) return false;
  if (b_image && ((uintptr_t)b_image) % 16 == 0)
    return x3_launch_gemm(d->epilogue, d->m, d->n, d->k, A, d->lda, (const char*)b_image, C, d->ldc, e, st) == REC_OK;
  if (!workspace || ((uintptr_t)workspace) % 16 || workspace_bytes < x3_image_bytes(d->k, d->n)) return false;
  char* img = (char*)workspace;
  if (x3_launch_split(B, d->ldb, d->k, d->n, d->trans_b ? 1 : 0, img, st) != REC_OK) return false;
  return x3_launch_gemm(d->epilogue, d->m, d->n, d->k, A, d->lda, img, C, d->ldc, e, st) == REC_OK;
}

template <int EPI>
static void launch_reduce(const rec_gemm_desc* d, const GemmPlan& p, const float* partial, float* C,
                          const EpiArgs& e, hipStream_t st, const float* cpart = nullptr, float* colsum_out = nullptr) {
  int64_t grid = (d->m * d->n + kBlock - 1) / kBlock;
  if (grid > kNumCU * 8) grid = kNumCU * 8;
  const int cblocks = cpart && colsum_out ? (d->n + kBlock - 1) / kBlock : 0;
  hipLaunchKernelGGL(splitk_reduce_kernel<EPI>, dim3((unsigned)(grid + cblocks)), dim3(kBlock), 0, st, d->m,
                     d->n, (int64_t)d->ldc, p.splits, partial, C, e, cpart, colsum_out, cblocks);
}

static bool x3_dw_eligible(const rec_gemm_desc* d, X3DwPlan* pl) {
  const char* v = getenv("REC_GEMM_BF16X3");
  const bool forced = !(v && *v == '1');
  const char* vd = getenv("REC_GEMM_BF16X3_DW");
  if (vd && *vd == '0') return false;
  if (!x3_enabled() || !d->trans_a || d->trans_b || (d->split_k != 0 && !forced && d->num_cus <= 0) ||
      d->epilogue != REC_EPI_NONE)
    return false;
  if (d->k < 8192 || d->m < 336 || d->m > 448 || d->n < 336 || d->n > 416) return false;
  if (d->lda % 4 || d->ldb % 4 || d->ldc % 4) return false;
  const int cus = d->num_cus > 0 && d->num_cus < device_cus() ? d->num_cus : device_cus();
  return x3_dw_plan((int)d->m, d->n, d->k, cus, pl);
}
static size_t x3_dw_bytes(const rec_gemm_desc* d, const X3DwPlan& pl) {
  return align_up((size_t)pl.slices * d->m * d->ldc * sizeof(float), 256) + align_up((size_t)pl.slices * d->n * sizeof(float), 256);
}
static bool launch_x3_dw(const rec_gemm_desc* d, const float* A, const float* B, float* C, const EpiArgs& e, float* b_colsum,
                         void* workspace, size_t workspace_bytes, hipStream_t st) {
  X3DwPlan pl;
  if (!x3_dw_eligible(d, &pl)) return false;
  if (((uintptr_t)A) % 16 || ((uintptr_t)B) % 16 || ((uintptr_t)C) % 16) return false;
  if (!workspace || ((uintptr_t)workspace) % 16 || workspace_bytes < x3_dw_bytes(d, pl)) return false;
  float* partial = (float*)workspace;
  float* cpart = (float*)((char*)workspace + align_up((size_t)pl.slices * d->m * d->ldc * sizeof(float), 256));
  if (x3_launch_dw(pl, (int)d->m, d->n, d->k, A, d->lda, B, d->ldb, partial, d->ldc, b_colsum ? cpart : nullptr, st) != REC_OK)
    return false;
  GemmPlan sp{};
  sp.splits = pl.slices;
  launch_reduce<REC_EPI_NONE>(d, sp, partial, C, e, st, b_colsum ? cpart : nullptr, b_colsum);
  set_route(REC_GEMM_ROUTE_X3_DW, -1, pl.slices);
  return true;
}

}

using namespace rec;

static size_t plain_workspace_bytes(const rec_gemm_desc* desc) {
  if (skinny_dw(desc)) {
    const size_t z = (size_t)((desc->k + kSkinnyKC - 1) / kSkinnyKC);
    return align_up(z * desc->m * desc->ldc * sizeof(float), 256) + align_up(z * desc->n * sizeof(float), 256);
  }
  const GemmPlan p = plan_gemm(desc);
  return (p.splits > 1 ? align_up((size_t)p.splits * desc->m * desc->ldc * sizeof(float), 256) : 0) +
         align_up((size_t)p.splits * desc->n * sizeof(float), 256);
}

static bool relu_bits_ok(const rec_gemm_desc* d) {
  return (d->epilogue == REC_EPI_BIAS_RELU || d->epilogue == REC_EPI_RELU_MASK) && x3_eligible(d) && d->lda % 4 == 0 &&
         d->ldc % 4 == 0;
}
extern "C" int rec_gemm_relu_bits_bytes(const rec_gemm_desc* desc, int32_t* eligible, size_t* bytes) {
  if (int rc = check_gemm(desc)) return rc;
  REC_REQUIRE(bytes, REC_EINVAL, "bytes is NULL");
  const bool ok = relu_bits_ok(desc);
  if (eligible) *eligible = ok ? 1 : 0;
  *bytes = ok ? align_up(x3_relu_bits_bytes(desc->m, desc->n), 256) : 0;
  return REC_OK;
}

extern "C" int rec_gemm_f32_workspace_bytes(const rec_gemm_desc* desc, size_t* bytes) {
  if (int rc = check_gemm(desc)) return rc;
  REC_REQUIRE(bytes, REC_EINVAL, "bytes is NULL");
  if (skinny_dw(desc)) {
    const size_t z = (size_t)((desc->k + kSkinnyKC - 1) / kSkinnyKC);
    *bytes = align_up(z * desc->m * desc->ldc * sizeof(float), 256) + align_up(z * desc->n * sizeof(float), 256);
    return REC_OK;
  }
  const GemmPlan p = plan_gemm(desc);
  *bytes = (p.splits > 1 ? align_up((size_t)p.splits * desc->m * desc->ldc * sizeof(float), 256) : 0) +
           align_up((size_t)p.splits * desc->n * sizeof(float), 256);
  if (x3_eligible(desc) && *bytes < x3_image_bytes(desc->k, desc->n)) *bytes = align_up(x3_image_bytes(desc->k, desc->n), 256);
  X3DwPlan dwp;
  if (x3_dw_eligible(desc, &dwp) && *bytes < x3_dw_bytes(desc, dwp)) *bytes = x3_dw_bytes(desc, dwp);
  return REC_OK;
}

extern "C" int rec_gemm_b_image_bytes(int32_t k, int32_t n, int32_t* eligible, size_t* bytes) {
  REC_REQUIRE(k > 0 && n > 0 && bytes, REC_EINVAL, "bad arguments");
  const bool ok = n % 4 == 0 && k % 8 == 0 && k >= 64 && x3_cols(n).nt > 0;
  if (eligible) *eligible = ok ? 1 : 0;
  *bytes = ok ? align_up(x3_image_bytes(k, n), 256) : 0;
  return REC_OK;
}

extern "C" int rec_gemm_b_images(int32_t count, const rec_gemm_b_image* items, void* stream) {
  REC_REQUIRE(count >= 0 && (count == 0 || items), REC_EINVAL, "bad arguments");
  for (int32_t at = 0; at < count; at += kX3BatchMax) {
    X3SplitBatch b{};
    b.count = count - at < kX3BatchMax ? count - at : kX3BatchMax;
    int64_t blocks = 0;
    for (int i = 0; i < b.count; ++i) {
      const rec_gemm_b_image& it = items[at + i];
      REC_REQUIRE(it.B && it.image && ((uintptr_t)it.image) % 16 == 0, REC_EINVAL, "item %d: null / unaligned pointer", at + i);
      REC_REQUIRE(it.k > 0 && it.n > 0 && it.n % 4 == 0 && it.k % 8 == 0 && it.k >= 64 && x3_cols(it.n).nt > 0, REC_ESHAPE,
                  "item %d: k %d x n %d has no image form (rec_gemm_b_image_bytes)", at + i, it.k, it.n);
      REC_REQUIRE(it.ldb >= (it.trans_b ? it.k : it.n), REC_EINVAL, "item %d: ldb too small", at + i);
      const X3Cols c = x3_cols(it.n);
      b.W[i] = it.B; b.img[i] = (char*)it.image; b.ldw[i] = it.ldb; b.K[i] = it.k; b.N[i] = it.n;
      b.trans[i] = it.trans_b ? 1 : 0;
      b.nkt[i] = (it.k + 31) / 32; b.np[i] = c.nt * 16; b.ncb[i] = 2 * c.ncb;
      b.first[i] = (unsigned)blocks;
      blocks += ((int64_t)b.ncb[i] * b.nkt[i] * b.np[i] * 4 + kBlock - 1) / kBlock;
    }
    b.first[b.count] = (unsigned)blocks;
    REC_REQUIRE(blocks < (1ll << 31), REC_ESHAPE, "too many blocks");
    hipLaunchKernelGGL(x3_split_batch_kernel, dim3((unsigned)blocks), dim3(kBlock), 0, (hipStream_t)stream, b);
    if (int rc = check_launch("rec_gemm_b_images")) return rc;
  }
  return REC_OK;
}

extern "C" int rec_gemm_last_route(rec_gemm_route* out) {
  REC_REQUIRE(out, REC_EINVAL, "out is NULL");
  *out = g_gemm_route;
  return REC_OK;
}

extern "C" int rec_gemm_plan_splits(const rec_gemm_desc* desc, int32_t num_cus, int32_t* splits) {
  if (int rc = check_gemm(desc)) return rc;
  REC_REQUIRE(splits && num_cus <= kNumCU, REC_EINVAL, "bad arguments");
  rec_gemm_desc d = *desc;
  d.split_k = 0;
  *splits = plan_gemm(&d, num_cus > 0 ? num_cus : kNumCU).splits;
  return REC_OK;
}

extern "C" int rec_gemm_f32_pair(const rec_gemm_desc* desc0, const float* A0, const float* B0, float* C0,
                                 const rec_gemm_epilogue_args* x0, const rec_gemm_desc* desc1, const float* A1,
                                 const float* B1, float* C1, const rec_gemm_epilogue_args* x1, void* workspace,
                                 size_t workspace_bytes, void* stream) {
  if (int rc = check_gemm(desc0)) return rc;
  if (int rc = check_gemm(desc1)) return rc;
  static const rec_gemm_epilogue_args kNoArgs = {};
  const rec_gemm_epilogue_args* y0 = x0 ? x0 : &kNoArgs;
  const rec_gemm_epilogue_args* y1 = x1 ? x1 : &kNoArgs;
  const bool shape = desc0->m > 0 && desc1->m > 0 && A0 && B0 && C0 && A1 && B1 && C1 && desc0->trans_a &&
                     desc0->epilogue == REC_EPI_NONE && !desc1->trans_a &&
                     (desc1->epilogue == REC_EPI_NONE ||
                      ((desc1->epilogue == REC_EPI_RELU_MASK || desc1->epilogue == REC_EPI_DSIGMOID) && y1->aux0 &&
                       y1->ld_aux0 >= desc1->n)) &&
                     !y1->b_colsum;
  if (shape) {
    EpiArgs e0{}, e1{};
    e1.aux0 = y1->aux0;
    e1.ld0 = y1->ld_aux0;
    if (launch_direct_pair(desc0, A0, B0, C0, e0, y0->b_colsum, desc1, A1, B1, C1, e1, (hipStream_t)stream))
      return check_launch("rec_gemm_f32_pair");
  }
  if (int rc = rec_gemm_f32(desc0, A0, B0, C0, x0, workspace, workspace_bytes, stream)) return rc;
  return rec_gemm_f32(desc1, A1, B1, C1, x1, workspace, workspace_bytes, stream);
}

extern "C" int rec_gemm_f32(const rec_gemm_desc* desc, const float* A, const float* B, float* C,
                            const rec_gemm_epilogue_args* x, void* workspace,
                            size_t workspace_bytes, void* stream) {
  if (int rc = check_gemm(desc)) return rc;
  if (desc->m == 0) return REC_OK;
  REC_REQUIRE(A && B && C, REC_EINVAL, "null pointer argument");
  static const rec_gemm_epilogue_args kNoArgs = {};
  if (!x) x = &kNoArgs;
  const int epi = desc->epilogue;
  const float* bias = x->bias;
  const float *aux0 = x->aux0, *aux1 = x->aux1;
  const int ld_aux0 = x->ld_aux0, ld_aux1 = x->ld_aux1;
  float* b_colsum = x->b_colsum;
  REC_REQUIRE(!b_colsum || desc->trans_a, REC_EINVAL,
              "b_colsum (the bias gradient) is produced by the trans_a form dW = X^T dY only");
  REC_REQUIRE(!(epi == REC_EPI_BIAS || epi == REC_EPI_BIAS_RELU || epi == REC_EPI_CROSS ||
                epi == REC_EPI_BIAS_SIGMOID || epi == REC_EPI_MOE) || bias, REC_EINVAL,
              "epilogue needs bias");
  unsigned long long* relu_bits = (unsigned long long*)x->relu_bits;
  REC_REQUIRE(!relu_bits || ((epi == REC_EPI_BIAS_RELU || epi == REC_EPI_RELU_MASK) && relu_bits_ok(desc) &&
                             ((uintptr_t)relu_bits) % 8 == 0), REC_EINVAL,
              "relu_bits: only a BIAS_RELU / RELU_MASK call that takes the bf16 x 3 forward / dX kernel "
              "(rec_gemm_relu_bits_bytes says which)");
  REC_REQUIRE(!(epi == REC_EPI_RELU_MASK || epi == REC_EPI_CROSS || epi == REC_EPI_MOE ||
                epi == REC_EPI_DSIGMOID || epi == REC_EPI_DTANH) || (epi == REC_EPI_RELU_MASK && relu_bits) ||
                  (aux0 && ld_aux0 >= desc->n), REC_EINVAL, "epilogue needs aux0");
  REC_REQUIRE(!(epi == REC_EPI_CROSS || epi == REC_EPI_ADD || epi == REC_EPI_MOE) ||
                  (aux1 && ld_aux1 >= desc->n), REC_EINVAL, "epilogue needs aux1");
  REC_REQUIRE(epi != REC_EPI_ADD || !aux0 || ld_aux0 >= desc->n, REC_EINVAL, "bad ld_aux0");
  REC_REQUIRE(epi != REC_EPI_MOE || (x->row_scale && x->row_scale_stride >= 1), REC_EINVAL,
              "epilogue needs row_scale");
  hipStream_t st = (hipStream_t)stream;
  static const int nt_env = [] { const char* v = getenv("REC_GEMM_NT_STORE"); return v && *v ? atoi(v) : 0; }();
  const int nt_store = nt_env == 2 || (nt_env == 1 && epi == REC_EPI_RELU_MASK) ? 1 : 0;
  EpiArgs e{bias, aux0, aux1, x->row_scale, x->out2, ld_aux0, ld_aux1, x->row_scale_stride, x->ld_out2, nt_store, relu_bits};
  REC_REQUIRE(!x->out2 || x->ld_out2 >= desc->n, REC_EINVAL, "bad ld_out2");
  if (skinny_rows(desc) && !b_colsum) {
    const bool vec_a = desc->lda % 4 == 0 && ((uintptr_t)A) % 16 == 0 && desc->k % 4 == 0;
    int64_t grid = (desc->m + kBlock / kWave - 1) / (kBlock / kWave);
    if (grid > kNumCU * 8) grid = kNumCU * 8;
    const size_t shmem = (size_t)desc->n * desc->k * sizeof(float);
#define REC_GEMV_CASE(E)                                                                                   \
  case E:                                                                                                  \
    hipLaunchKernelGGL(gemv_rows_kernel<E>, dim3((unsigned)grid), dim3(kBlock), shmem, st, desc->m, desc->n, \
                       desc->k, A, (int64_t)desc->lda, B, (int64_t)desc->ldb, desc->trans_b != 0, C,       \
                       (int64_t)desc->ldc, e, vec_a);                                                      \
    break;
    switch (epi) {
      REC_GEMV_CASE(REC_EPI_NONE) REC_GEMV_CASE(REC_EPI_BIAS) REC_GEMV_CASE(REC_EPI_BIAS_RELU)
      REC_GEMV_CASE(REC_EPI_RELU_MASK) REC_GEMV_CASE(REC_EPI_CROSS) REC_GEMV_CASE(REC_EPI_BIAS_SIGMOID)
      REC_GEMV_CASE(REC_EPI_BIAS_TANH) REC_GEMV_CASE(REC_EPI_ADD) REC_GEMV_CASE(REC_EPI_MOE)
      REC_GEMV_CASE(REC_EPI_DSIGMOID) REC_GEMV_CASE(REC_EPI_DTANH)
    }
#undef REC_GEMV_CASE
    set_route(REC_GEMM_ROUTE_SKINNY_ROWS, -1, 1, vec_a ? REC_GEMM_ROUTE_VEC_A : 0);
    return check_launch("rec_gemm_f32 (skinny rows)");
  }
  if (skinny_dw(desc) && epi == REC_EPI_NONE) {
    const size_t need = plain_workspace_bytes(desc);
    REC_REQUIRE(workspace && workspace_bytes >= need, REC_EWORKSPACE, "workspace %zu < %zu", workspace_bytes, need);
    const int z = (int)((desc->k + kSkinnyKC - 1) / kSkinnyKC);
    float* part = (float*)workspace;
    float* cpart2 = (float*)((char*)workspace + align_up((size_t)z * desc->m * desc->ldc * sizeof(float), 256));
    hipLaunchKernelGGL(desc->m <= kBlock / 2 ? skinny_dw_narrow_kernel : skinny_dw_kernel, dim3(z), dim3(kBlock), 0, st,
                       (int)desc->m, desc->n, (int64_t)desc->k, A, (int64_t)desc->lda, B, (int64_t)desc->ldb,
                       (int64_t)desc->ldc, part, b_colsum ? cpart2 : nullptr);
    GemmPlan sp;
    sp.splits = z;
    launch_reduce<REC_EPI_NONE>(desc, sp, part, C, e, st);
    if (b_colsum)
      hipLaunchKernelGGL(colsum_reduce_kernel, dim3((desc->n + kBlock - 1) / kBlock), dim3(kBlock), 0, st,
                         desc->n, z, (const float*)cpart2, b_colsum);
    set_route(REC_GEMM_ROUTE_SKINNY_DW, -1, z);
    return check_launch("rec_gemm_f32 (skinny dW)");
  }
  if (launch_x3_dw(desc, A, B, C, e, b_colsum, workspace, workspace_bytes, st)) return check_launch("rec_gemm_f32 (bf16x3 dW)");
  if (!b_colsum && launch_x3(desc, A, B, C, e, x->b_image, workspace, workspace_bytes, st)) {
    set_route(REC_GEMM_ROUTE_X3);
    return check_launch("rec_gemm_f32 (bf16x3)");
  }
  REC_REQUIRE(!relu_bits, REC_EINVAL, "relu_bits: the call did not take the bf16 x 3 kernel (alignment / workspace)");
  if (!b_colsum && launch_panel(desc, A, B, C, e, st, device_cus())) {
    set_route(REC_GEMM_ROUTE_PANEL);
    return check_launch("rec_gemm_f32 (panel)");
  }
  if (!b_colsum && launch_glds(desc, A, B, C, e, st)) {
    set_route(REC_GEMM_ROUTE_GLDS);
    return check_launch("rec_gemm_f32 (glds)");
  }
  if (launch_direct(desc, A, B, C, e, b_colsum, st)) return check_launch("rec_gemm_f32 (direct)");
  const GemmPlan p = plan_gemm(desc);
  REC_REQUIRE(p.tiles_total < (1ll << 31), REC_ESHAPE, "too many tiles");
  float* partial = nullptr;
  float* cpart = nullptr;
  if (p.splits > 1 || b_colsum) {
    const size_t need = plain_workspace_bytes(desc);
    REC_REQUIRE(workspace && workspace_bytes >= need, REC_EWORKSPACE, "workspace %zu < %zu",
                workspace_bytes, need);
    size_t off = 0;
    if (p.splits > 1) {
      partial = (float*)workspace;
      off = align_up((size_t)p.splits * desc->m * desc->ldc * sizeof(float), 256);
    }
    if (b_colsum) cpart = p.splits == 1 ? b_colsum : (float*)((char*)workspace + off);
  }
  static const bool skip_reduce = [] { const char* v = getenv("REC_GEMM_SKIP_REDUCE"); return v && *v == '1'; }();
#define REC_EPI_CASE(E)                                                   \
  case E:                                                                 \
    if (partial) {                                                        \
      launch_epi<REC_EPI_NONE>(desc, p, A, B, C, e, partial, cpart, st);  \
      if (!skip_reduce) launch_reduce<E>(desc, p, partial, C, e, st, cpart, b_colsum); \
    } else {                                                              \
      launch_epi<E>(desc, p, A, B, C, e, nullptr, cpart, st);             \
    }                                                                     \
    break;
  switch (epi) {
    REC_EPI_CASE(REC_EPI_NONE)
    REC_EPI_CASE(REC_EPI_BIAS)
    REC_EPI_CASE(REC_EPI_BIAS_RELU)
    REC_EPI_CASE(REC_EPI_RELU_MASK)
    REC_EPI_CASE(REC_EPI_CROSS)
    REC_EPI_CASE(REC_EPI_BIAS_SIGMOID)
    REC_EPI_CASE(REC_EPI_BIAS_TANH)
    REC_EPI_CASE(REC_EPI_ADD)
    REC_EPI_CASE(REC_EPI_MOE)
    REC_EPI_CASE(REC_EPI_DSIGMOID)
    REC_EPI_CASE(REC_EPI_DTANH)
  }
#undef REC_EPI_CASE
  if (b_colsum && !partial && cpart != b_colsum && !skip_reduce)
    hipLaunchKernelGGL(colsum_reduce_kernel, dim3((desc->n + kBlock - 1) / kBlock), dim3(kBlock), 0,
                       st, desc->n, p.splits, (const float*)cpart, b_colsum);
  return check_launch("rec_gemm_f32");
}

extern "C" int rec_colsum_workspace_bytes(int64_t m, int32_t n, size_t* bytes) {
  REC_REQUIRE(bytes && m >= 0 && n > 0, REC_EINVAL, "bad arguments");
  const int64_t nblk = (m + kColsumRows - 1) / kColsumRows;
  *bytes = align_up((size_t)(nblk > 0 ? nblk : 1) * n * sizeof(float), 256);
  return REC_OK;
}

extern "C" int rec_colsum(int64_t m, int32_t n, int32_t ld, const float* G, float* out,
                          void* workspace, size_t workspace_bytes, void* stream) {
  REC_REQUIRE(m >= 0 && n > 0 && ld >= n && out, REC_EINVAL, "bad arguments");
  hipStream_t st = (hipStream_t)stream;
  if (m == 0) {
    (void)hipMemsetAsync(out, 0, (size_t)n * sizeof(float), st);
    return REC_OK;
  }
  REC_REQUIRE(G, REC_EINVAL, "G is NULL");
  size_t need = 0;
  rec_colsum_workspace_bytes(m, n, &need);
  REC_REQUIRE(workspace && workspace_bytes >= need, REC_EWORKSPACE, "workspace %zu < %zu",
              workspace_bytes, need);
  const int nblk = (int)((m + kColsumRows - 1) / kColsumRows);
  hipLaunchKernelGGL(colsum_partial_kernel, dim3(nblk), dim3(kBlock), 0, st, m, n, (int64_t)ld, G,
                     (float*)workspace);
  hipLaunchKernelGGL(colsum_final_kernel, dim3((n + 15) / 16), dim3(kBlock), 0, st,
                     nblk, n, (const float*)workspace, out);
  return check_launch("rec_colsum");
}

extern "C" int rec_mlp_head_bwd_workspace_bytes(int64_t batch, int32_t n, size_t* bytes) {
  REC_REQUIRE(bytes && batch >= 0 && n > 0, REC_EINVAL, "bad arguments");
  *bytes = align_up((size_t)kNumCU * 8 * (n + 1) * sizeof(float), 256);
  return REC_OK;
}

extern "C" int rec_mlp_head_bwd(int64_t batch, int32_t n, const float* act, int64_t ld_act, const float* dz,
                                const float* w, int32_t relu, float* dx, int64_t ld_dx, float* dw, float* db,
                                void* workspace, size_t workspace_bytes, void* stream) {
  REC_REQUIRE(batch >= 0 && n > 0 && n % 4 == 0 && n <= kHeadChunks * 4, REC_ESHAPE,
              "rec_mlp_head_bwd: n must be a multiple of 4 and <= %d", kHeadChunks * 4);
  REC_REQUIRE(act && dz && w && dx && dw && db && ld_act >= n && ld_dx >= n && ld_act % 4 == 0 && ld_dx % 4 == 0 &&
                  ((uintptr_t)act) % 16 == 0 && ((uintptr_t)dx) % 16 == 0 && ((uintptr_t)w) % 16 == 0,
              REC_EINVAL, "bad arguments (16-byte aligned rows required)");
  size_t need = 0;
  rec_mlp_head_bwd_workspace_bytes(batch, n, &need);
  REC_REQUIRE(workspace && workspace_bytes >= need, REC_EWORKSPACE, "workspace %zu < %zu", workspace_bytes, need);
  hipStream_t st = (hipStream_t)stream;
  float* partial = (float*)workspace;
  int64_t grid = (batch + 31) / 32;
  if (grid > kNumCU * 8) grid = kNumCU * 8;
  if (grid < 1) grid = 1;
  hipLaunchKernelGGL(mlp_head_bwd_kernel, dim3((unsigned)grid), dim3(kBlock), 0, st, batch, n, act, ld_act, dz, w, dx,
                     ld_dx, relu, partial);
  const int cols_per_block = kBlock / kWave;
  hipLaunchKernelGGL(mlp_head_fold_kernel, dim3((n + 1 + cols_per_block - 1) / cols_per_block), dim3(kBlock), 0, st,
                     (int)grid, n, (const float*)partial, dw, db);
  return check_launch("rec_mlp_head_bwd");
}
```

paddlerec_amd/deepfm.py:

```python
import math
import os
import time

import torch

from . import ops
from .slot_net import (NUM_THRESHOLDS, SlotDygraphModel, SlotLayerBase, _OnSide, _round_up,
                       auc_metrics, slot_feeds)


class _FlatParams:
    ALIGN = 64

    def __init__(self, shapes, device, reserve=None):
        self.names = [n for n, _ in shapes]
        self.shapes = dict(shapes)
        self.offsets, o = {}, 0
        for n, s in shapes:
            self.offsets[n] = o
            o += -(-max(math.prod(s), (reserve or {}).get(n, 0)) // self.ALIGN) * self.ALIGN
        self.data = torch.zeros(max(o, 1), dtype=torch.float32, device=device)
        self.grad = torch.zeros_like(self.data)
        self.m = torch.zeros_like(self.data)
        self.v = torch.zeros_like(self.data)
# ... 301 lines not shown
    def c_net(self):
        net = getattr(self, "_c_net", None)
        if net is not None:
            return net
        from . import _lib
        if self.n_linear > _lib.DeepFMNet.MAX_LINEAR:
            raise ops.RecError("rec_deepfm_train_step takes at most %d Linear layers" % _lib.DeepFMNet.MAX_LINEAR)
        self._ensure_sparse_state()
        D, st = self.sparse_feature_dim, self.sparse_state
        p, g = self.dense.p, self.dense.g
        net = _lib.DeepFMNet()
        net.num_slots, net.dim, net.dense_dim, net.n_linear = self.sparse_num_field, D, self.dense_feature_dim, self.n_linear
        sizes = self.layer_sizes + [1]
        for i in range(self.n_linear):
            net.widths[i] = sizes[i]
            net.w[i], net.b[i] = self.mlp_w[i].data_ptr(), self.mlp_b[i].data_ptr()
            net.gw[i], net.gb[i] = self.mlp_dw[i].data_ptr(), self.mlp_db[i].data_ptr()
        net.table_rows, net.num_rows = self.fm.rec.shape[0], self.sparse_feature_number
        net.padding_idx = -1 if self.fm.padding_idx is None else self.fm.padding_idx
        net.slot_rows = self.slot_rows or 0
        net.slot_offset = None if self.fm.slot_offset is None else self.fm.slot_offset.data_ptr()
        net.rec, net.rec_stride = self.fm.rec.data_ptr(), self.fm.rec.stride(0)
        net.mv, net.mv_stride, net.v_offset = st["mv"].data_ptr(), st["mv"].stride(0), _round_up(D, 4)
        net.dense_w, net.dense_w_one = p["fm.dense_w"].data_ptr(), p["fm.dense_w_one"].data_ptr()
        net.g_dense_w, net.g_dense_w_one = g["fm.dense_w"].data_ptr(), g["fm.dense_w_one"].data_ptr()
        net.flat_param, net.flat_grad = self.dense.data.data_ptr(), self.dense.grad.data_ptr()
        net.flat_m, net.flat_v, net.flat_numel = self.dense.m.data_ptr(), self.dense.v.data_ptr(), self.dense.data.numel()
        net.w0_folded = self._w0p.data_ptr() if (self.compact or self.padded) else None
        net.layer0_width = self.ld0 if self.padded else 0
        self._c_net = net
        return net

    def train_step_c(self, sparse_inputs, dense_inputs, label, lr=1e-3, auc_stats=None):
        self.sync()
        ids = self._concat_ids(sparse_inputs)
        self.step_count += 1
        if getattr(self, "_ws_c", None) is None:
            self._ws_c = self.k.Workspace(self.device)
        side = None
        if self.device.type == "cuda" and os.environ.get("REC_DEEPFM_OVERLAP", "1") != "0":
            if self._side is None:
                self._side = self.k.concurrent_stream(self.device)
            side = self._side
        self._w_key = None
        return self.k.deepfm_train_step(self.c_net(), ids, dense_inputs, label.reshape(-1), self.step_count, self._ws_c,
                                        lr=lr, auc_stats=auc_stats, num_thresholds=NUM_THRESHOLDS, status=self.status,
                                        side_stream=side)

    def train_step(self, sparse_inputs, dense_inputs, label, lr=1e-3, auc_stats=None,
                   allreduce=None):
        if self._plan_eligible(sparse_inputs, dense_inputs, label, auc_stats, allreduce):
            if self._c_step_small(sparse_inputs):
                return self.train_step_c(sparse_inputs, dense_inputs, label, lr=lr, auc_stats=auc_stats)
            self.sync()
            out = self._train_step_planned(sparse_inputs, dense_inputs, label, lr, auc_stats)
            if out is not None:
                return out
        ids = self._concat_ids(sparse_inputs)
        B, S = ids.shape
        self._ensure_sparse_state()
        self.step_count += 1
        on_gpu = self.device.type == "cuda"
        cur = torch.cuda.current_stream() if on_gpu else None
        overlap = on_gpu and os.environ.get("REC_DEEPFM_OVERLAP", "1") != "0" and not self._recording
        if overlap and self._side is None:
            self._side = self.k.concurrent_stream(self.device)
        side = self._side if overlap else None
        use_images = (on_gpu and B >= 8192 and hasattr(self.k, "GemmImages") and not self._recording
                      and os.environ.get("REC_GEMM_IMAGES", "1") != "0")
        groups = getattr(self, "_groups", None)
        if groups is None or groups.n != B * S:
            groups = self._groups = self.k.IdGroups(B * S, self.device)
        group_at = os.environ.get("REC_DEEPFM_GROUP_AT", "pre")

        small = (self.lazy_mode and B * S <= getattr(self.k, "SMALL_MERGE_MAX", 0)
                 and hasattr(self.k, "sparse_adam_record_small")
                 and os.environ.get("REC_SMALL_MERGE", "1") != "0")

        slot_sort = (not small and self.slot_rows is not None
                     and hasattr(self.k, "group_slots_eligible") and self.k.group_slots_eligible(B, S, self.slot_rows)
                     and os.environ.get("REC_DEEPFM_GROUP", "slots") != "general")
        sorted_rg = slot_sort and self.lazy_mode and os.environ.get("REC_DEEPFM_SORTED_GRAD", "0") == "1"
        gspec = os.environ.get("REC_DEEPFM_GROUP_CUS", "")
        gside = side
        pipe = (self.pipelined and side is not None and self.lazy_mode and not small and allreduce is None
                and B >= 16384 and os.environ.get("REC_DEEPFM_DEFER_ALL", "0") != "1")
        if pipe:
            if self._gside is None:
                self._gside = self.k.concurrent_stream(self.device, index=1)
            gside = self._gside
        elif self._side_pending:
            self.sync()
        if gspec and side is not None and hasattr(self.k, "cu_stride_stream"):
            if "," in gspec:
                gside = self.k.cu_range_stream(self.device, 0, int(gspec.split(",")[1]))
            else:
                gside = self.k.cu_stride_stream(self.device, 0, int(gspec))

        def issue_group():
            if small:
                return
            if self.step_count > 3 and os.environ.get("REC_DEEPFM_SKIP_GROUP", "0") == "1":
                return
            with _OnSide(gside, cur):
                if slot_sort:
                    self.k.ids_group_slots(ids, self.slot_rows, self.fm.padding_idx, self.ws_group, self.status, groups,
                                           want_rank=sorted_rg)
                else:
                    self.k.ids_group(ids, self.sparse_feature_number, self.fm.padding_idx, self.ws_group,
                                     self.fm.slot_offset, self.status, groups)
        if group_at == "pre":
            issue_group()
        if self._adam_done is not None and "adam" in os.environ.get("REC_PIPE_SKIP", ""):
            self._adam_done = None
        if self._adam_done is not None:
            cur.wait_event(self._adam_done)
            self._adam_done = None
        if os.environ.get("REC_PIPE_JOIN", "early") == "early":
            self.sync()
        with self._timed("fm_fwd"):
            y1, y2, feat, sum_emb, _ = self._fm_fwd(ids, dense_inputs)
        self.sync()
        if group_at == "fwd":
            issue_group()
        mlp_w, mlp_dw = self._mlp_weights(use_images)
        img_f, img_t = self._image_lists() if use_images else (None, None)
        nl = self.n_linear
        ikw_f = lambda n_: dict(images=img_f[:n_]) if img_f is not None else {}
        ikw_t = lambda n_: dict(images_t=img_t[:n_]) if img_t is not None else {}
        fused_head = self.n_linear > 1 and hasattr(self.k, "ctr_head") and self.k.ctr_head_ok(mlp_w[-1], mlp_dw[-1])
        with self._timed("mlp_fwd"):
            if fused_head:
                h, acts = self.k.mlp_forward(feat.view(B, -1), mlp_w[:-1], self.mlp_b[:-1], self.ws_mlp, relu_last=True,
                                             **ikw_f(nl - 1))
                pred, dz, loss, g_head = self.k.ctr_head(h, mlp_w[-1], self.mlp_b[-1], y1, y2, label, self.ws,
                                                         mlp_dw[-1], self.mlp_db[-1])
            else:
                y_dnn, acts = self.k.mlp_forward(feat.view(B, -1), mlp_w, self.mlp_b, self.ws_mlp, **ikw_f(nl))
        if not fused_head:
            pred, dz, loss = self.k.sigmoid_logloss(y1, y2, y_dnn, label, self.ws)
        if group_at == "bwd":
            issue_group()
        if auc_stats is not None:
            self.k.auc_histogram(pred, label, auc_stats[0], auc_stats[1], NUM_THRESHOLDS)
        defer_all = os.environ.get("REC_DEEPFM_DEFER_ALL", "0") == "1"
        kw = dict(defer_all=True) if defer_all else dict(defer_first=True) if not small else {}
        if overlap and not defer_all and not small and B >= 16384:
            kw.update(defer_split=int(os.environ.get("REC_DW0_SPLIT", "16")))
            kw.update(defer_cus=int(os.environ.get("REC_DW0_CUS", "192")))
        if on_gpu and not defer_all and not self._recording and os.environ.get("REC_MLP_DW_STREAM", "0") == "1":
            if getattr(self, "_dw_stream", None) is None:
                self._dw_stream, self._ws_dw = self.k.concurrent_stream(self.device), self.k.Workspace(self.device)
            kw.update(dw_stream=self._dw_stream, dw_ws=self._ws_dw)
        with self._timed("mlp_bwd"):
            if fused_head:
                res = self.k.mlp_backward(g_head, acts, mlp_w[:-1], mlp_dw[:-1], self.mlp_db[:-1], self.ws_mlp, **kw,
                                          **ikw_t(nl - 1))
            else:
                res = self.k.mlp_backward(dz, acts, mlp_w, mlp_dw, self.mlp_db, self.ws_mlp, **kw, **ikw_t(nl))
            d_flat, finish_dw0 = res if kw else (res, (lambda: None))
        if group_at == "tail":
            issue_group()
        if sorted_rg and side is not None:
            cur.wait_stream(gside)
        with self._timed("fm_bwd"):
            row_grad, _, _ = self.k.deepfm_fm_bwd(
                dense_inputs, feat, sum_emb, d_flat if self.padded else d_flat.view(B, self.fp, -1), dz, dz, S, self.ws,
                out=(self._buf("_rg", (B * S, self.sparse_feature_dim)),
                     self.dense.g["fm.dense_w"].view(self.dense_feature_dim, -1),
                     self.dense.g["fm.dense_w_one"]),
                dense_w=self.dense.p["fm.dense_w"], compact=self.compact,
                **(dict(row_rank=groups.rank) if sorted_rg else {}),
                **(dict(feat_ld=self.ld0) if self.padded else {}))
        t = self.step_count
        st = self.sparse_state
        skw = dict(grad_sorted=True) if sorted_rg else {}
        swap = (side is not None and allreduce is None and not small
                and os.environ.get("REC_DEEPFM_TAIL_SWAP", "0") == "1")
        if not sorted_rg and side is not None and (gside is not side or swap):
            cur.wait_stream(gside)

        def tail_sparse():
            with self._timed("sparse_adam"):
                upd = self.k.sparse_adam_rows if self.lazy_mode else self.k.adam_rows_all
                if small:
                    D = self.sparse_feature_dim
                    self.k.sparse_adam_record_small(ids, self.fm.slot_offset, self.fm.padding_idx, row_grad, dz, S,
                                                    self.fm.rec, st["mv"], D, t, lr, v_offset=_round_up(D, 4),
                                                    status=self.status)
                    return
                pp = self._pp = self.k.segment_partials(groups, row_grad, row_grad.shape[1],
                                                        out=getattr(self, "_pp", None), **skw)
                pp1 = self._pp1 = self.k.segment_partials(groups, dz, 1, grad_div=S, out=getattr(self, "_pp1", None))
                if self.lazy_mode:
                    D = self.sparse_feature_dim
                    self.k.sparse_adam_record(groups, row_grad, dz, S, self.fm.rec, st["mv"], D, t, lr,
                                              v_offset=_round_up(D, 4), partials=pp, partials1=pp1, **skw)
                elif hasattr(self.k, "adam_record_all") and os.environ.get("REC_NONLAZY_RECORD", "1") != "0":
                    D = self.sparse_feature_dim
                    self.k.adam_record_all(groups, row_grad, dz, S, self.fm.rec, st["mv"], D, t, lr,
                                           v_offset=_round_up(D, 4), partials=pp, partials1=pp1)
                else:
                    upd(groups, row_grad, 1, self.fm.embedding, st["m"], st["v"], t, lr, partials=pp)
                    upd(groups, dz, S, self.fm.embedding_one, st["m1"], st["v1"], t, lr, partials=pp1)

        def tail_dense():
            with self._timed("mlp_bwd_dw0"):
                finish_dw0()
                self._fold_backward()
            if allreduce is not None:
                allreduce(self.dense.grad)
            self.k.adam_dense(self.dense.data, self.dense.m, self.dense.v, self.dense.grad, t, lr)
            self._w_key = None

        if pipe:
            after_bwd = torch.cuda.Event()
            after_bwd.record(cur)
            if "gwait" not in os.environ.get("REC_PIPE_SKIP", ""):
                cur.wait_stream(gside)
            tail_sparse()
            with torch.cuda.stream(side):
                side.wait_event(after_bwd)
                tail_dense()
                self._adam_done = torch.cuda.Event()
                self._adam_done.record()
                self._refresh_weights(use_images)
                self._w_key = (self.dense.data._version, self.step_count + 1, bool(use_images))
                self._side_pending = torch.cuda.Event()
                self._side_pending.record()
            self._pending_refs = (acts, finish_dw0, d_flat, feat)
            return loss, pred
        if swap:
            with _OnSide(side, cur):
                tail_dense()
            tail_sparse()
        else:
            with _OnSide(side, cur):
                tail_sparse()
            tail_dense()
            if side is not None and use_images and os.environ.get("REC_DEEPFM_REFRESH_TAIL", "1") != "0":
                self._refresh_weights(use_images)
                self._w_key = (self.dense.data._version, self.step_count + 1, bool(use_images))
        if side is not None:
            cur.wait_stream(self._side)
        return loss, pred

    def _timed(self, name):
        return _Timed(self.timers, name)

    def time_fm_pair(self, batches, repeats=20, rounds=3):
        ids0, dense0 = batches[0]
        ids0 = self._concat_ids(ids0)
        B, S = ids0.shape
        D = self.sparse_feature_dim
        y1, y2, feat, sum_emb, _ = self._fm_fwd(ids0, dense0)
        dfeat = torch.randn(*((B, self.ld0) if self.padded else (B, self.fp, D)), device=self.device) * 1e-3
        pkw = dict(feat_ld=self.ld0) if self.padded else {}
        dz = torch.randn(B, 1, device=self.device) * 1e-3
        out = (self._buf("_rg", (B * S, D)), torch.empty(self.dense_feature_dim, D, device=self.device),
               torch.empty(self.dense_feature_dim, device=self.device))

        def fwd(i):
            ids, dense = batches[i % len(batches)]
            self.k.deepfm_fm_fwd(self._concat_ids(ids), dense, self.fm.embedding, self.fm.embedding_one,
                                 self.dense.p["fm.dense_w"], self.dense.p["fm.dense_w_one"], self.fm.padding_idx,
                                 self.fm.slot_offset, self.status, (y1, y2, feat, sum_emb), compact=self.compact, **pkw)

        rank = getattr(getattr(self, "_groups", None), "rank", None)
        rkw = dict(row_rank=rank) if rank is not None and rank.numel() >= B * S else {}

        def bwd(i):
            self.k.deepfm_fm_bwd(dense0, feat, sum_emb, dfeat, dz, dz, S, self.ws, out=out,
                                 dense_w=self.dense.p["fm.dense_w"], compact=self.compact, **rkw, **pkw)

        def run(fn):
            ts = []
            for _ in range(rounds):
                torch.cuda.synchronize()
                a, b = torch.cuda.Event(enable_timing=True), torch.cuda.Event(enable_timing=True)
                a.record()
                for i in range(repeats):
                    fn(i)
                b.record()
                torch.cuda.synchronize()
                ts.append(a.elapsed_time(b) * 1e3 / repeats)
            return sorted(ts)[len(ts) // 2]
        return run(fwd), run(bwd)

class DygraphModel(SlotDygraphModel):

    def create_model(self, config, device="cuda", kernels=None, comm=None):
        args = (config.get("hyper_parameters.sparse_feature_number"), config.get("hyper_parameters.sparse_feature_dim"),
                config.get("hyper_parameters.dense_input_dim"), config.get("hyper_parameters.sparse_inputs_slots") - 1,
                config.get("hyper_parameters.fc_sizes"))
        if comm is not None and comm.world > 1:
            from .sharded import ShardedDeepFMLayer
            return ShardedDeepFMLayer(*args, device=device, comm=comm, kernels=kernels)
        return DeepFMLayer(*args, device=device, kernels=kernels)

    def train_forward(self, dy_model, metrics_list, batch_data, config, lr=None, next_batch=None):
        label, sparse, dense = self.create_feeds(batch_data, config, dy_model.device)
        lr = lr if lr is not None else config.get("hyper_parameters.optimizer.learning_rate", 0.001)
        kw = {}
        if next_batch is not None and hasattr(dy_model, "comm"):
            kw["next_sparse_inputs"] = self.create_feeds(next_batch, config, dy_model.device)[1]
        loss, _ = dy_model.train_step(sparse, dense, label, lr, metrics_list[0] if metrics_list else None, **kw)
        return loss, metrics_list, {"loss": loss}

def auc_from_buckets(stat_pos, stat_neg):
    pos_l = stat_pos.tolist()
    neg_l = stat_neg.tolist()
    area = pos = neg = 0.0
    total = 0
    for idx in range(len(pos_l) - 1, -1, -1):
        new_pos = pos + pos_l[idx]
        new_neg = neg + neg_l[idx]
        total += pos_l[idx] + neg_l[idx]
        area += (new_neg - neg) * (pos + new_pos) / 2
        pos, neg = new_pos, new_neg
    if pos * neg == 0 or total == 0:
        return 0.5
    return area / (pos * neg)
```

paddlerec_amd/ops.py:

```python
import collections
import ctypes as C
import os

import torch

from . import _lib
from ._lib import (EPI, AdagradHyper, AdamHyper, CinView, DcnCrossDesc, DeepFMDesc, DinDesc, FatFFMDesc, FEFMDesc, FFMDesc, GemmBImage, GemmDesc, GemmEpilogueArgs, GradLayout,
                   GradSrc, LazyInit, MultislotDesc, PsAccessor, PsLayout, RecError, check)

_recorder = None


def lib():
    h = _lib.lib()
    return h if _recorder is None else _recorder.proxy(h)


_raw_stream = getattr(torch._C, "_cuda_getCurrentRawStream", None)
_raw_device = getattr(torch._C, "_cuda_getDevice", None)


def _stream():
    if _raw_stream is not None and _raw_device is not None:
        return C.c_void_p(_raw_stream(_raw_device()))
# ... 2495 lines not shown
    if out is None:
        out = torch.empty(B, d, dtype=torch.float32, device=dev)
    t1 = torch.empty(B, E * r, dtype=torch.float32, device=dev)
    t2 = torch.empty(B, E * r, dtype=torch.float32, device=dev)
    prob = torch.empty(B, E, dtype=torch.float32, device=dev)
    desc = _lib.CrossMixDesc(B, d, r, E, _ld(x0, "x0"), _ld(xl, "xl"), _ld(out, "out"))
    nb = C.c_size_t(0)
    check(lib().rec_crossnet_mix_layer_workspace_bytes(C.byref(desc), C.byref(nb), None))
    w = ws.get(nb.value)
    check(lib().rec_crossnet_mix_layer_fwd(C.byref(desc), _p(x0), _p(xl), _p(U), _p(V), _p(Cm), _p(bias), _p(gate_w),
                                           _p(gate_b), _p(out), _p(t1), _p(t2), _p(prob), _p(w),
                                           C.c_size_t(w.numel()), _stream()), "rec_crossnet_mix_layer_fwd")
    return out, t1, t2, prob


def crossnet_mix_layer_bwd(x0, xl, U, V, Cm, bias, gate_w, t1, t2, prob, dxnext, dx0_acc, accumulate_dx0, fold_dx0,
                           gU, gV, gC, gbias, g_gate_w, g_gate_b, accumulate_gate, ws, out=None):
    B, d = xl.shape
    E, _, r = U.shape
    if out is None:
        out = torch.empty(B, d, dtype=torch.float32, device=xl.device)
    desc = _lib.CrossMixDesc(B, d, r, E, _ld(x0, "x0"), _ld(xl, "xl"),
                             max(d, _ld(dxnext, "dxnext"), _ld(dx0_acc, "dx0_acc"), _ld(out, "out")))
    nb = C.c_size_t(0)
    check(lib().rec_crossnet_mix_layer_workspace_bytes(C.byref(desc), None, C.byref(nb)))
    w = ws.get(nb.value)
    check(lib().rec_crossnet_mix_layer_bwd(C.byref(desc), _p(x0), _p(xl), _p(U), _p(V), _p(Cm), _p(bias), _p(gate_w),
                                           _p(t1), _p(t2), _p(prob), _p(dxnext), _ld(dxnext, "dxnext"), _p(dx0_acc),
                                           _ld(dx0_acc, "dx0_acc"), int(accumulate_dx0), int(fold_dx0), _p(out),
                                           _ld(out, "out"), _p(gU), _p(gV), _p(gC), _p(gbias), _p(g_gate_w),
                                           _p(g_gate_b), int(accumulate_gate), _p(w), C.c_size_t(w.numel()),
                                           _stream()), "rec_crossnet_mix_layer_bwd")
    return out


class ShardRoute:

    def __init__(self, n, num_shards, device):
        self.n, self.num_shards = n, num_shards
        i64 = dict(dtype=torch.int64, device=device)
        self.send_local_row = torch.empty(max(n, 1), **i64)
        self.send_pos = torch.empty(max(n, 1), **i64)
        self.send_sample = torch.empty(max(n, 1), **i64)
        self.slot_of_pos = torch.empty(max(n, 1), **i64)
        self.send_counts = torch.zeros(num_shards + 1, **i64)


class DedupPlan:

    def __init__(self, n, num_shards, cap, device):
        self.n, self.num_shards, self.cap = n, num_shards, cap
        self.groups = IdGroups(n, device)
        i64 = dict(dtype=torch.int64, device=device)
        self.send_rows = torch.empty(num_shards * cap, **i64)
        self.slot_of_pos = torch.empty(max(n, 1), **i64)
        self.slot_of_uniq = torch.empty(max(n, 1), **i64)
        self.counts = torch.zeros(num_shards, **i64)
        self.sentinel = None


def dedup_plan(ids, num_rows, padding_idx, num_shards, local_rows, cap, ws, slot_offset=None, status=None, plan=None):
    _chk(ids, torch.int64, "ids")
    n, G, dev = ids.numel(), int(num_shards), ids.device
    if plan is None or plan.n != n or plan.cap != cap or plan.num_shards != G:
        plan = DedupPlan(n, G, cap, dev)
    if status is None:
        status = new_status(dev)
    S = ids.shape[-1] if ids.dim() > 1 else 1
    nbytes = C.c_size_t(0)
    check(lib().rec_dedup_plan_workspace_bytes(n, G, int(local_rows), C.byref(nbytes)), "rec_dedup_plan_workspace_bytes")
    w = ws.get(nbytes.value)
    g = plan.groups
    plan.sentinel = int(local_rows)
    check(lib().rec_dedup_plan(n, S, int(num_rows), -1 if padding_idx is None else int(padding_idx), G, int(local_rows),
                               int(cap), _p(ids), _p(slot_offset), _p(g.sorted_pos), _p(g.uniq_rows), _p(g.seg_offset),
                               _p(g.n_uniq), _p(plan.send_rows), _p(plan.slot_of_pos), _p(plan.slot_of_uniq),
                               _p(plan.counts), _p(status), _p(w), C.c_size_t(w.numel()), _stream()), "rec_dedup_plan")
    return plan, status


def dedup_merge(plan, grad, emb_dim, grad_div=1, out=None):
    G, cap, D = plan.num_shards, plan.cap, int(emb_dim)
    none = G * cap
    if out is None or out.shape[0] != none + 1:
        out = torch.empty(none + 1, D, dtype=torch.float32, device=grad.device)
    out.zero_()

    class _G:
        pass
    g, f = plan.groups, _G()
    f.n, f.n_uniq, f.seg_offset, f.sorted_pos, f.uniq_rows = g.n, g.n_uniq, g.seg_offset, g.sorted_pos, plan.slot_of_uniq
    sparse_sgd_rows(f, grad, out, -1.0, grad_div=grad_div)
    return out


def shard_route(ids, num_rows, padding_idx, num_shards, ws, slot_offset=None, status=None,
                route=None):
    _chk(ids, torch.int64, "ids")
    n = ids.numel()
    S = ids.shape[-1] if ids.dim() > 1 else 1
    dev = ids.device
    if route is None:
        route = ShardRoute(n, num_shards, dev)
    if status is None:
        status = new_status(dev)
    nbytes = C.c_size_t(0)
    check(lib().rec_shard_route_workspace_bytes(n, num_shards, C.byref(nbytes)))
    w = ws.get(nbytes.value)
    check(lib().rec_shard_route(n, S, num_rows, -1 if padding_idx is None else padding_idx,
                                num_shards, _p(ids), _p(slot_offset), _p(route.send_local_row),
                                _p(route.send_pos), _p(route.send_sample), _p(route.slot_of_pos),
                                _p(route.send_counts), _p(status), _p(w), C.c_size_t(w.numel()),
                                _stream()), "rec_shard_route")
    return route, status


def _chk_mat(t, name):
    if not t.is_cuda:
        raise RecError("%s must be a device tensor (no CPU fallback)" % name)
    if t.dtype != torch.float32 or t.dim() != 2:
        raise RecError("%s must be a 2-D float32 tensor" % name)
    if t.shape[1] > 1 and t.stride(1) != 1:
        raise RecError("%s must have unit column stride" % name)
    return t.stride(0) if t.shape[0] > 1 else max(t.shape[1], 1)


_gemm_ws_cache = {}


class GemmImages:

    def __init__(self, specs, device):
        self.specs, self.images = list(specs), []
        for B, trans_b in self.specs:
            n, k = (B.shape if trans_b else B.shape[::-1])
            ok, nb = C.c_int32(0), C.c_size_t(0)
            check(lib().rec_gemm_b_image_bytes(int(k), int(n), C.byref(ok), C.byref(nb)), "rec_gemm_b_image_bytes")
            self.images.append(torch.empty(nb.value, dtype=torch.uint8, device=device) if ok.value else None)
        live = [(B, t, img) for (B, t), img in zip(self.specs, self.images) if img is not None]
        self._items = (GemmBImage * max(1, len(live)))()
        self._n = len(live)
        for it, (B, t, img) in zip(self._items, live):
            n, k = (B.shape if t else B.shape[::-1])
            it.B, it.ldb, it.k, it.n, it.trans_b, it.image = B.data_ptr(), _chk_mat(B, "B"), int(k), int(n), int(t), img.data_ptr()

    def refresh(self):
        if self._n:
            check(lib().rec_gemm_b_images(self._n, self._items, _stream()), "rec_gemm_b_images")

    def get(self, i):
        return self.images[i]


def gemm(A, B, ws, trans_a=False, trans_b=False, epilogue="none", bias=None, aux0=None, aux1=None,
         out=None, split_k=0, b_colsum=None, row_scale=None, out2=None, num_cus=0, b_image=None, relu_bits=None):
    d, x, out, need = _gemm_prepare(A, B, trans_a, trans_b, epilogue, bias, aux0, aux1, out, split_k, b_colsum, row_scale,
                                    out2, num_cus, b_image)
    if relu_bits is not None:
        nb = _relu_bits_bytes(d)
        if epilogue == "bias_relu":
            t = torch.empty(nb // 8, dtype=torch.int64, device=A.device) if nb else None
            relu_bits.append(t)
            relu_bits = t
        elif nb == 0 or relu_bits.numel() * 8 < nb:
            relu_bits = None
        if relu_bits is not None:
            x.relu_bits = relu_bits.data_ptr()
            if _recorder is not None:
                _recorder.keep.append(relu_bits)
    w = ws.get(need)
    check(lib().rec_gemm_f32(C.byref(d), _p(A), _p(B), _p(out), C.byref(x), _p(w),
                             C.c_size_t(w.numel()), _stream()), "rec_gemm_f32")
    return out


def linear_backward(X, G, W, ws, dW, db, relu_src=None, b_image=None, epilogue=None, aux0=None, relu_bits=None, out=None):
    if epilogue is None:
        epilogue, aux0 = ("relu_mask", relu_src) if relu_src is not None else ("none", None)
    d0, x0, _, need0 = _gemm_prepare(X, G, True, False, "none", None, None, None, dW, 0, db, None, None, 0, None)
    d1, x1, dX, need1 = _gemm_prepare(G, W, False, True, epilogue, None, aux0, None, out, 0, None, None, None, 0, b_image)
    if relu_bits is not None and epilogue == "relu_mask":
        nb = _relu_bits_bytes(d1)
        if nb and relu_bits.numel() * 8 >= nb:
            x1.relu_bits = relu_bits.data_ptr()
            if _recorder is not None:
                _recorder.keep.append(relu_bits)
    w = ws.get(max(need0, need1))
    check(lib().rec_gemm_f32_pair(C.byref(d0), _p(X), _p(G), _p(dW), C.byref(x0), C.byref(d1), _p(G), _p(W), _p(dX),
                                  C.byref(x1), _p(w), C.c_size_t(w.numel()), _stream()), "rec_gemm_f32_pair")
    return dX


GemmRouteInfo = collections.namedtuple("GemmRouteInfo", "family cfg splits flags")


def gemm_last_route():
    r = _lib.GemmRoute()
    check(lib().rec_gemm_last_route(C.byref(r)), "rec_gemm_last_route")
    return GemmRouteInfo(_lib.GEMM_ROUTE_FAMILIES[r.family] if r.family >= 0 else None,
                         _lib.GEMM_CFGS[r.cfg] if r.cfg >= 0 else None, r.splits,
                         frozenset(n for n, b in _lib.GEMM_ROUTE_FLAGS.items() if r.flags & b))


_relu_bits_cache = {}


def _relu_bits_bytes(d):
    if os.environ.get("REC_RELU_BITS") == "0":
        return 0
    key = (d.m, d.n, d.k, d.lda, d.ldb, d.ldc, d.trans_a, d.trans_b, d.epilogue, d.split_k, os.environ.get("REC_GEMM_BF16X3"))
    nb = _relu_bits_cache.get(key)
    if nb is None:
        ok, nbytes = C.c_int32(0), C.c_size_t(0)
        check(lib().rec_gemm_relu_bits_bytes(C.byref(d), C.byref(ok), C.byref(nbytes)), "rec_gemm_relu_bits_bytes")
        nb = _relu_bits_cache[key] = nbytes.value if ok.value else 0
    return nb


def _gemm_prepare(A, B, trans_a, trans_b, epilogue, bias, aux0, aux1, out, split_k, b_colsum, row_scale, out2, num_cus,
                  b_image):
    lda, ldb = _chk_mat(A, "A"), _chk_mat(B, "B")
    K, M = (A.shape if trans_a else A.shape[::-1])
    N, K2 = (B.shape if trans_b else B.shape[::-1])
    if K != K2:
        raise RecError("inner dimensions differ: %d vs %d" % (K, K2))
    if out is None:
        out = torch.empty(M, N, dtype=torch.float32, device=A.device)
    ldc = _chk_mat(out, "out")
    if tuple(out.shape) != (M, N):
        raise RecError("out has shape %s, expected %s" % (tuple(out.shape), (M, N)))
    ld0 = ld1 = 0
    if aux0 is not None:
        ld0 = _chk_mat(aux0, "aux0")
    if aux1 is not None:
        ld1 = _chk_mat(aux1, "aux1")
    if bias is not None:
        _chk(bias, torch.float32, "bias")
        if bias.numel() != N:
            raise RecError("bias must have N elements")
    if b_colsum is not None:
        _chk(b_colsum, torch.float32, "b_colsum")
        if b_colsum.numel() != N:
            raise RecError("b_colsum must have N elements")
    rs_stride = 0
    if row_scale is not None:
        if not row_scale.is_cuda or row_scale.dtype != torch.float32 or row_scale.shape[0] != M:
            raise RecError("row_scale must be a float32 device tensor with M rows")
        rs_stride = row_scale.stride(0) if M > 1 else 1
    ld2 = 0
    if out2 is not None:
        ld2 = _chk_mat(out2, "out2")
        if tuple(out2.shape) != (M, N):
            raise RecError("out2 must have the shape of out")
    d = GemmDesc(M, N, K, lda, ldb, ldc, int(trans_a), int(trans_b), EPI[epilogue], int(split_k), int(max(num_cus, 0)))
    if num_cus > 0 and split_k <= 0:
        sp = C.c_int32(0)
        check(lib().rec_gemm_plan_splits(C.byref(d), int(num_cus), C.byref(sp)), "rec_gemm_plan_splits")
        d.split_k = sp.value
    pv = lambda t: None if t is None else t.data_ptr()
    x = GemmEpilogueArgs(pv(bias), pv(aux0), ld0, pv(aux1), ld1, pv(row_scale), rs_stride, pv(out2),
                         ld2, pv(b_colsum), pv(b_image))
    if _recorder is not None:
        _recorder.keep.extend(t for t in (bias, aux0, aux1, row_scale, out2, b_colsum, b_image) if t is not None)
    key = (M, N, K, lda, ldb, ldc, d.trans_a, d.trans_b, d.epilogue, d.split_k, d.num_cus,
           os.environ.get("REC_GEMM_BF16X3"), os.environ.get("REC_GEMM_BF16X3_DW"))
    need = _gemm_ws_cache.get(key)
    if need is None:
        nbytes = C.c_size_t(0)
        check(lib().rec_gemm_f32_workspace_bytes(C.byref(d), C.byref(nbytes)))
        need = _gemm_ws_cache[key] = nbytes.value
    return d, x, out, need


def colsum(G, ws, out=None):
    ld = _chk_mat(G, "G")
    M, N = G.shape
    if out is None:
        out = torch.empty(N, dtype=torch.float32, device=G.device)
    nbytes = C.c_size_t(0)
    check(lib().rec_colsum_workspace_bytes(M, N, C.byref(nbytes)))
    w = ws.get(nbytes.value)
    check(lib().rec_colsum(M, N, ld, _p(G), _p(out), _p(w), C.c_size_t(w.numel()), _stream()),
          "rec_colsum")
    return out


class _Acts(list):
    relu_bits = None


def mlp_forward(x, weights, biases, ws, relu_last=False, out_last=None, images=None):
    acts = _Acts()
    bits = [None]
    n = len(weights)
    for i in range(n):
        acts.append(x)
        last = i == n - 1
        relu = not last or relu_last
        x = gemm(x, weights[i], ws, epilogue="bias_relu" if relu else "bias",
                 bias=biases[i], out=out_last if last else None, b_image=images[i] if images is not None else None,
                 relu_bits=bits if relu else None)
        if not relu:
            bits.append(None)
    acts.append(x)
    acts.relu_bits = bits
    return x, acts


def mlp_head_bwd(act, dz, w, ws, dw, db, relu=True, out=None):
    B, n = act.shape
    if out is None:
        out = torch.empty(B, n, dtype=torch.float32, device=act.device)
    nbytes = C.c_size_t(0)
    check(lib().rec_mlp_head_bwd_workspace_bytes(B, n, C.byref(nbytes)))
    wk = ws.get(nbytes.value)
    check(lib().rec_mlp_head_bwd(B, n, _p(act), act.stride(0), _p(dz), _p(w), 1 if relu else 0, _p(out), out.stride(0),
                                 _p(dw), _p(db), _p(wk), C.c_size_t(wk.numel()), _stream()), "rec_mlp_head_bwd")
    return out


def ctr_head_ok(w, dw):
    return (os.environ.get("REC_CTR_HEAD_FUSED", "1") != "0" and w.dim() == 2 and w.shape[1] == 1 and
            w.shape[0] % 4 == 0 and w.shape[0] <= 512 and w.is_contiguous() and w.data_ptr() % 16 == 0 and
            dw.is_contiguous())


def ctr_head(act, w, bias, y1, y2, label, ws, dw, db, eps=1e-4, clip=None, mean_over=0, relu=True, out=None):
    B, n = act.shape
    dev = act.device
    _chk(label, torch.int64, "label")
    for t, nm in ((y1, "y1"), (y2, "y2"), (bias, "bias")):
        _chk(t, torch.float32, nm)
    if label.numel() != B or (y1 is not None and y1.numel() != B) or (y2 is not None and y2.numel() != B):
        raise RecError("ctr_head: y1 / y2 / label must have one entry per row of act")
    if clip is not None and not clip[0] < clip[1]:
        raise RecError("clip must be (lo, hi) with lo < hi")
    if out is None:
        pred = torch.empty(B, 1, dtype=torch.float32, device=dev)
        dz = torch.empty(B, 1, dtype=torch.float32, device=dev)
        loss = torch.empty(1, dtype=torch.float32, device=dev)
        dx = torch.empty(B, n, dtype=torch.float32, device=dev)
    else:
        pred, dz, loss, dx = out
    nbytes = C.c_size_t(0)
    check(lib().rec_ctr_head_workspace_bytes(B, n, C.byref(nbytes)))
    wk = ws.get(nbytes.value)
    lo, hi = (float(clip[0]), float(clip[1])) if clip is not None else (0.0, 0.0)
    check(lib().rec_ctr_head_fwd_bwd(B, n, int(mean_over), _p(act), act.stride(0), _p(w), _p(bias), _p(y1), _p(y2),
                                     _p(label), float(eps), lo, hi, 1 if relu else 0, None, _p(pred), _p(dz), _p(loss),
                                     _p(dx), dx.stride(0), _p(dw), _p(db), _p(wk), C.c_size_t(wk.numel()), _stream()),
          "rec_ctr_head_fwd_bwd")
    return pred, dz, loss, dx


def _head_ok(act, w, dw, db, dy):
    return (os.environ.get("REC_MLP_HEAD_FUSED", "1") != "0" and w.dim() == 2 and w.shape[1] == 1 and
            w.shape[0] % 4 == 0 and w.shape[0] <= 512 and act.dim() == 2 and act.stride(1) == 1 and
            act.stride(0) % 4 == 0 and act.data_ptr() % 16 == 0 and w.is_contiguous() and w.data_ptr() % 16 == 0 and
            dw.is_contiguous() and dy.is_contiguous() and dy.shape[-1] == 1 and act.shape[0] >= 64)


def mlp_backward(dy, acts, weights, dws, dbs, ws, defer_first=False, defer_all=False, dw_stream=None, dw_ws=None,
                 defer_split=0, images_t=None, defer_cus=0):
    n = len(weights)
    g = dy
    imt = (lambda i: images_t[i]) if images_t is not None else (lambda i: None)
    rbl = getattr(acts, "relu_bits", None)
    rb = (lambda i: rbl[i]) if rbl is not None else (lambda i: None)
    head = n > 1 and _head_ok(acts[n - 1], weights[n - 1], dws[n - 1], dbs[n - 1], dy)
    if head:
        g = mlp_head_bwd(acts[n - 1], dy, weights[n - 1], ws, dws[n - 1], dbs[n - 1], relu=True)
        n_run = n - 1
    else:
        n_run = n
    if defer_all:
        gs = [None] * n_run
        for i in reversed(range(n_run)):
            gs[i] = g
            g = gemm(g, weights[i], ws, trans_b=True, b_image=imt(i),
                     **(dict(epilogue="relu_mask", aux0=acts[i], relu_bits=rb(i)) if i > 0 else {}))

        def finish(num_cus=0):
            for i in reversed(range(n_run)):
                gemm(acts[i], gs[i], ws, trans_a=True, out=dws[i], b_colsum=dbs[i], num_cus=num_cus)
        return g, finish
    cur = torch.cuda.current_stream() if dw_stream is not None else None
    keep = []

    def join():
        if dw_stream is not None:
            cur.wait_stream(dw_stream)
            keep.clear()
    for i in reversed(range(n_run)):
        if i == 0 and defer_first:
            g0 = g
            d_in = gemm(g0, weights[0], ws, trans_b=True, b_image=imt(0))
            join()
            return d_in, (lambda: gemm(acts[0], g0, ws, trans_a=True, out=dws[0], b_colsum=dbs[0], split_k=defer_split,
                                    num_cus=defer_cus))
        if dw_stream is not None:
            dw_stream.wait_stream(cur)
            keep.append(g)
            with torch.cuda.stream(dw_stream):
                gemm(acts[i], g, dw_ws if dw_ws is not None else ws, trans_a=True, out=dws[i], b_colsum=dbs[i])
        else:
            g = linear_backward(acts[i], g, weights[i], ws, dws[i], dbs[i], relu_src=acts[i] if i > 0 else None,
                                b_image=imt(i), relu_bits=rb(i) if i > 0 else None)
            continue
        if i > 0:
            g = gemm(g, weights[i], ws, trans_b=True, epilogue="relu_mask", aux0=acts[i], b_image=imt(i), relu_bits=rb(i))
        else:
            g = gemm(g, weights[i], ws, trans_b=True, b_image=imt(i))
    join()
    return g


def sigmoid_logloss(y1, y2, y_dnn, label, ws, eps=1e-4, want_dz=True, out=None, mean_over=0, clip=None):
    B = y1.numel()
    dev = y1.device
    _chk(y1, torch.float32, "y1")
    _chk(y2, torch.float32, "y2")
    _chk(y_dnn, torch.float32, "y_dnn")
    _chk(label, torch.int64, "label")
    if clip is not None and not clip[0] < clip[1]:
        raise RecError("clip must be (lo, hi) with lo < hi")
    if out is None:
        pred = torch.empty(B, 1, dtype=torch.float32, device=dev)
        dz = torch.empty(B, 1, dtype=torch.float32, device=dev) if want_dz else None
        loss = torch.empty(1, dtype=torch.float32, device=dev)
    else:
        pred, dz, loss = out
    nbytes = C.c_size_t(0)
    check(lib().rec_logloss_workspace_bytes(B, C.byref(nbytes)))
    w = ws.get(nbytes.value)
    lo, hi = (float(clip[0]), float(clip[1])) if clip is not None else (0.0, 0.0)
    check(lib().rec_sigmoid_logloss(B, int(mean_over), _p(y1), _p(y2), _p(y_dnn), _p(label), float(eps), lo, hi,
                                    _p(pred), _p(dz), _p(loss), _p(w), C.c_size_t(w.numel()), _stream()),
          "rec_sigmoid_logloss")
    return pred, dz, loss


def auc_histogram(pred, label, stat_pos, stat_neg, num_thresholds=4095):
    _chk(pred, torch.float32, "pred")
    _chk(label, torch.int64, "label")
    _chk(stat_pos, torch.int64, "stat_pos", (num_thresholds + 1,))
    _chk(stat_neg, torch.int64, "stat_neg", (num_thresholds + 1,))
    check(lib().rec_auc_histogram(pred.numel(), _p(pred), _p(label), num_thresholds, _p(stat_pos),
                                  _p(stat_neg), _stream()), "rec_auc_histogram")


def fill_uniform(buf, lo, hi, seed):
    _chk(buf, torch.float32, "buf")
    check(lib().rec_fill_uniform(buf.numel(), _p(buf), float(lo), float(hi), int(seed), _stream()),
          "rec_fill_uniform")
    return buf


_SIDE_STREAMS = {}


def concurrent_stream(device, tries=8, micros=200, priority=None, index=0):
    device = torch.device(device)
    main = torch.cuda.current_stream(device)
    if priority is None:
        priority = int(os.environ.get("REC_SIDE_PRIORITY", "0"))
    key = (device.index, main.cuda_stream, priority, int(index))
    if key in _SIDE_STREAMS:
        return _SIDE_STREAMS[key]
    others = [main] + [concurrent_stream(device, tries, micros, priority, j) for j in range(int(index))]

    def overlaps(s, o):
        for st in (s, o):
            check(lib().rec_stream_spin(1, C.c_void_p(st.cuda_stream)), "rec_stream_spin")
        torch.cuda.synchronize(device)
        e0, e1 = torch.cuda.Event(enable_timing=True), torch.cuda.Event(enable_timing=True)
        e0.record(o)
        check(lib().rec_stream_spin(micros, C.c_void_p(s.cuda_stream)), "rec_stream_spin")
        check(lib().rec_stream_spin(micros, C.c_void_p(o.cuda_stream)), "rec_stream_spin")
        e1.record(o)
        torch.cuda.synchronize(device)
        return e0.elapsed_time(e1) * 1e3 < 1.5 * micros
    s, keep = None, []
    with torch.cuda.device(device):
        for _ in range(tries):
            s = torch.cuda.Stream(device=device, priority=priority)
            keep.append(s)
            if all(overlaps(s, o) for o in others):
                break
    _SIDE_STREAMS[key] = s
    return s


_CU_STREAMS = {}


def cu_range_stream(device, cu_begin, cu_end):
    device = torch.device(device)
    key = (device.index, int(cu_begin), int(cu_end))
    if key not in _CU_STREAMS:
        h = C.c_void_p()
        with torch.cuda.device(device):
            check(lib().rec_stream_create_cu_range(int(cu_begin), int(cu_end), C.byref(h)),
                  "rec_stream_create_cu_range")
        _CU_STREAMS[key] = torch.cuda.ExternalStream(h.value, device=device)
    return _CU_STREAMS[key]


def cu_stride_stream(device, first, stride, cu_total=256):
    device = torch.device(device)
    key = (device.index, "stride", int(first), int(stride), int(cu_total))
    if key not in _CU_STREAMS:
        h = C.c_void_p()
        with torch.cuda.device(device):
            check(lib().rec_stream_create_cu_stride(int(first), int(stride), int(cu_total), C.byref(h)),
                  "rec_stream_create_cu_stride")
        _CU_STREAMS[key] = torch.cuda.ExternalStream(h.value, device=device)
    return _CU_STREAMS[key]


def xxh32(data: bytes, seed: int = 0) -> int:
    return int(lib().rec_xxh32(data, len(data), seed))


def hash_features(field_idx, values, hash_dim=1000001):
    n = len(values)
    arr = (C.c_char_p * n)(*[v.encode("utf-8") for v in values])
    idx = (C.c_int32 * n)(*[int(i) for i in field_idx])
    out = (C.c_int64 * n)()
    check(lib().rec_xxh32_hash_mod(arr, idx, n, hash_dim, out), "rec_xxh32_hash_mod")
    return list(out)
```

Baseline: 44.20 million samples/s.

## Defer split-K dW reductions and batch them into one launch

Weight-gradient GEMMs in the MLP backward now record their split-K reduction as a job, with each job keeping its own workspace so the partials stay valid. All jobs are then run by a single batched reduce kernel after the first-layer dW. This replaces several small reduce and colsum launches with one larger launch and keeps the data-gradient GEMM chain running back to back. It costs extra workspace memory per layer and adds a stable-pointer contract between the C host path and the Python path.

```diff
diff --git a/include/recengine.h b/include/recengine.h
--- a/include/recengine.h
+++ b/include/recengine.h
@@ -396,6 +396,7 @@
   int32_t num_cus;
 } rec_gemm_desc;
 
+struct rec_gemm_reduce_job;
 typedef struct {
   const float* bias;
   const float* aux0;
@@ -409,7 +410,19 @@
   float* b_colsum;
   const void* b_image;
   void* relu_bits;
+  struct rec_gemm_reduce_job* defer_reduce;
 } rec_gemm_epilogue_args;
+
+typedef struct rec_gemm_reduce_job {
+  const float* partial;
+  const float* colsum_partial;
+  float* c;
+  float* colsum;
+  int64_t m;
+  int32_t n, ldc;
+  int32_t splits;
+} rec_gemm_reduce_job;
+int rec_gemm_reduce_batch(int32_t count, const rec_gemm_reduce_job* jobs, void* stream);
 
 int rec_gemm_f32_workspace_bytes(const rec_gemm_desc* desc, size_t* bytes);
 int rec_gemm_relu_bits_bytes(const rec_gemm_desc* desc, int32_t* eligible, size_t* bytes);
diff --git a/paddlerec_amd/_lib.py b/paddlerec_amd/_lib.py
--- a/paddlerec_amd/_lib.py
+++ b/paddlerec_amd/_lib.py
@@ -170,7 +170,13 @@
     _fields_ = [("bias", C.c_void_p), ("aux0", C.c_void_p), ("ld_aux0", C.c_int32),
                 ("aux1", C.c_void_p), ("ld_aux1", C.c_int32), ("row_scale", C.c_void_p),
                 ("row_scale_stride", C.c_int32), ("out2", C.c_void_p), ("ld_out2", C.c_int32),
-                ("b_colsum", C.c_void_p), ("b_image", C.c_void_p), ("relu_bits", C.c_void_p)]
+                ("b_colsum", C.c_void_p), ("b_image", C.c_void_p), ("relu_bits", C.c_void_p),
+                ("defer_reduce", C.c_void_p)]
+
+
+class GemmReduceJob(C.Structure):
+    _fields_ = [("partial", C.c_void_p), ("colsum_partial", C.c_void_p), ("c", C.c_void_p), ("colsum", C.c_void_p),
+                ("m", C.c_int64), ("n", C.c_int32), ("ldc", C.c_int32), ("splits", C.c_int32)]
 
 
 class GemmRoute(C.Structure):
@@ -393,6 +399,7 @@
     "rec_gemm_relu_bits_bytes": (C.c_int, [C.POINTER(GemmDesc), C.POINTER(_I32), C.POINTER(_SZ)]),
     "rec_gemm_b_image_bytes": (C.c_int, [_I32, _I32, C.POINTER(_I32), C.POINTER(_SZ)]),
     "rec_gemm_b_images": (C.c_int, [_I32, C.POINTER(GemmBImage), _P]),
+    "rec_gemm_reduce_batch": (C.c_int, [_I32, C.POINTER(GemmReduceJob), _P]),
     "rec_gemm_f32": (C.c_int, [C.POINTER(GemmDesc), _P, _P, _P, C.POINTER(GemmEpilogueArgs), _P, _SZ, _P]),
     "rec_gemm_f32_pair": (C.c_int, [C.POINTER(GemmDesc), _P, _P, _P, C.POINTER(GemmEpilogueArgs), C.POINTER(GemmDesc), _P, _P,
                                     _P, C.POINTER(GemmEpilogueArgs), _P, _SZ, _P]),
diff --git a/paddlerec_amd/csrc/deepfm_step.hip b/paddlerec_amd/csrc/deepfm_step.hip
--- a/paddlerec_amd/csrc/deepfm_step.hip
+++ b/paddlerec_amd/csrc/deepfm_step.hip
@@ -81,6 +81,8 @@
   size_t ws_bytes;
   void* ws_head;
   size_t ws_head_bytes;
+  void* ws_defer[REC_DEEPFM_MAX_LINEAR];
+  size_t ws_defer_bytes[REC_DEEPFM_MAX_LINEAR];
   void* ws_side;
   size_t ws_side_bytes;
   void* img_f[REC_DEEPFM_MAX_LINEAR];
@@ -121,6 +123,20 @@
   *out = align_up(need, 256);
   return REC_OK;
 }
+
+bool defer_reduce_on(const Shape& s, int64_t B) {
+  const char* v = getenv("REC_DEFER_REDUCE");
+  return !s.small && B >= 16384 && !(v && *v == '0');
+}
+
+rec_gemm_desc dw_desc(int in, int w, int64_t B, int split_k, int num_cus) {
+  rec_gemm_desc d{};
+  d.m = in; d.n = w; d.k = (int)B; d.lda = in; d.ldb = w; d.ldc = w; d.trans_a = 1; d.epilogue = REC_EPI_NONE;
+  d.split_k = split_k; d.num_cus = num_cus;
+  return d;
+}
+int dw0_split() { const char* v = getenv("REC_DW0_SPLIT"); return v && *v ? atoi(v) : 16; }
+int dw0_cus() { const char* v = getenv("REC_DW0_CUS"); return v && *v ? atoi(v) : 192; }
 
 int group_workspace(const rec_deepfm_net* net, const Shape& s, int64_t B, size_t* out) {
   size_t b = 0;
@@ -202,6 +218,22 @@
   if (int rc = call_workspace(net, s, B, &cw)) return rc;
   bf->ws = c.bytes(cw);
   bf->ws_bytes = cw;
+  for (int i = 0; i < REC_DEEPFM_MAX_LINEAR; ++i) {
+    bf->ws_defer[i] = nullptr;
+    bf->ws_defer_bytes[i] = 0;
+  }
+  if (defer_reduce_on(s, B)) {
+    const int n_run = (s.ctr_head || s.head) ? s.n - 1 : s.n;
+    int in = s.in0;
+    for (int i = 0; i < n_run; ++i) {
+      const rec_gemm_desc d = dw_desc(in, net->widths[i], B, i == 0 ? dw0_split() : 0, i == 0 ? dw0_cus() : 0);
+      size_t b = 0;
+      if (int rc = rec_gemm_f32_workspace_bytes(&d, &b)) return rc;
+      bf->ws_defer_bytes[i] = align_up(b, 256);
+      bf->ws_defer[i] = c.bytes(bf->ws_defer_bytes[i]);
+      in = net->widths[i];
+    }
+  }
   bf->ws_head = nullptr;
   bf->ws_head_bytes = 0;
   if (s.small && s.ctr_head) {
@@ -216,7 +248,8 @@
 
 int gemm(int64_t m, int n, int k, bool ta, bool tb, int epi, const float* A, const float* Bm, float* C,
          const float* bias, const float* aux0, int ld0, float* b_colsum, int split_k, const Buffers& bf, void* st,
-         const void* b_image = nullptr, int num_cus = 0, void* relu_bits = nullptr) {
+         const void* b_image = nullptr, int num_cus = 0, void* relu_bits = nullptr, rec_gemm_reduce_job* job = nullptr,
+         int job_ws = -1) {
   rec_gemm_desc d{};
   d.num_cus = num_cus;
   d.m = m; d.n = n; d.k = k;
@@ -226,6 +259,10 @@
   d.trans_a = ta; d.trans_b = tb; d.epilogue = epi; d.split_k = split_k;
   rec_gemm_epilogue_args x{};
   x.bias = bias; x.aux0 = aux0; x.ld_aux0 = ld0; x.b_colsum = b_colsum; x.b_image = b_image; x.relu_bits = relu_bits;
+  if (job) {
+    x.defer_reduce = job;
+    return rec_gemm_f32(&d, A, Bm, C, &x, bf.ws_defer[job_ws], bf.ws_defer_bytes[job_ws], st);
+  }
   return rec_gemm_f32(&d, A, Bm, C, &x, bf.ws, bf.ws_bytes, st);
 }
 
@@ -415,6 +452,8 @@
   const float* g0 = nullptr;
   float* d_flat = nullptr;
   bool dw0_done = false;
+  const bool defer = overlap && defer_reduce_on(s, B);
+  rec_gemm_reduce_job jobs[REC_DEEPFM_MAX_LINEAR] = {};
   for (int i = n_run - 1; i >= 0; --i) {
     const int in = i == 0 ? s.in0 : net->widths[i - 1], w = net->widths[i];
     if (i == 0) {
@@ -429,6 +468,12 @@
                    bf.img_t[0]));
       break;
     }
+    if (defer) {
+      REC_TRY(gemm(in, w, (int)B, true, false, REC_EPI_NONE, bf.act[i], g, net->gw[i], nullptr, nullptr, 0, net->gb[i], 0, bf,
+                   stream, nullptr, 0, nullptr, &jobs[i], i));
+      REC_TRY(gemm(B, in, w, false, true, REC_EPI_RELU_MASK, g, net->w[i], bf.g[gi], nullptr, bf.act[i], in, nullptr, 0, bf,
+                   stream, bf.img_t[i], 0, bf.relu_bits[i]));
+    } else
     REC_TRY(linear_backward(B, in, w, bf.act[i], g, net->w[i], net->gw[i], net->gb[i], bf.g[gi], bf.act[i], bf, stream,
                             bf.img_t[i], bf.relu_bits[i]));
     g = bf.g[gi];
@@ -494,12 +539,11 @@
                                    bf.seg_offset, bf.sorted_pos, bf.row_grad, &gl, bf.dz, &gl1, nullptr, net->rec,
                                    net->mv, hyper, sst));
   }
-  static const int dw0_split = [] { const char* v = getenv("REC_DW0_SPLIT"); return v && *v ? atoi(v) : 16; }();
-  static const int dw0_cus = [] { const char* v = getenv("REC_DW0_CUS"); return v && *v ? atoi(v) : 192; }();
   if (!dw0_done)
     REC_TRY(gemm(s.in0, net->widths[0], (int)B, true, false, REC_EPI_NONE, bf.feat, g0, gw0, nullptr, nullptr, 0,
-                 net->gb[0], overlap && B >= 16384 ? dw0_split : 0, bf, stream, nullptr,
-                 overlap && B >= 16384 ? dw0_cus : 0));
+                 net->gb[0], overlap && B >= 16384 ? dw0_split() : 0, bf, stream, nullptr,
+                 overlap && B >= 16384 ? dw0_cus() : 0, nullptr, defer ? &jobs[0] : nullptr, 0));
+  if (defer) REC_TRY(rec_gemm_reduce_batch(n_run, jobs, stream));
   if (s.compact)
     REC_TRY(rec_dense_fold_bwd_full(S, Dn, D, net->widths[0], net->dense_w, net->w[0], gw0, net->gw[0],
                                     net->g_dense_w, 1, stream));
diff --git a/paddlerec_amd/csrc/gemm_f32.hip b/paddlerec_amd/csrc/gemm_f32.hip
--- a/paddlerec_amd/csrc/gemm_f32.hip
+++ b/paddlerec_amd/csrc/gemm_f32.hip
@@ -198,20 +198,18 @@
 }
 
 template <int EPI>
-__global__ __launch_bounds__(kBlock) void splitk_reduce_kernel(int64_t M, int N, int64_t ldc,
-                                                               int splits,
-                                                               const float* __restrict__ partial,
-                                                               float* __restrict__ C, EpiArgs epi,
-                                                               const float* __restrict__ cpartial,
-                                                               float* __restrict__ colsum_out, int colsum_blocks) {
-  const int rblocks = (int)gridDim.x - colsum_blocks;
-  if ((int)blockIdx.x >= rblocks) {
-    const int j = ((int)blockIdx.x - rblocks) * kBlock + threadIdx.x;
+__device__ __forceinline__ void splitk_reduce_blocks(int bid, int nblk, int64_t M, int N, int64_t ldc, int splits,
+                                                     const float* __restrict__ partial, float* __restrict__ C,
+                                                     const EpiArgs& epi, const float* __restrict__ cpartial,
+                                                     float* __restrict__ colsum_out, int colsum_blocks) {
+  const int rblocks = nblk - colsum_blocks;
+  if (bid >= rblocks) {
+    const int j = (bid - rblocks) * kBlock + threadIdx.x;
     if (j < N) colsum_out[j] = colsum_fold(N, splits, cpartial, j);
     return;
   }
   const int64_t total = M * N;
-  for (int64_t e = (int64_t)blockIdx.x * kBlock + threadIdx.x; e < total;
+  for (int64_t e = (int64_t)bid * kBlock + threadIdx.x; e < total;
        e += (int64_t)rblocks * kBlock) {
     const int64_t i = e / N;
     const int j = (int)(e % N);
@@ -228,6 +226,39 @@
     C[i * ldc + j] = apply_epi<EPI>(t, i, j, epi);
     if (EPI == REC_EPI_CROSS && epi.out2) epi.out2[i * epi.ld2 + j] = t + epi.bias[j];
   }
+}
+
+template <int EPI>
+__global__ __launch_bounds__(kBlock) void splitk_reduce_kernel(int64_t M, int N, int64_t ldc,
+                                                               int splits,
+                                                               const float* __restrict__ partial,
+                                                               float* __restrict__ C, EpiArgs epi,
+                                                               const float* __restrict__ cpartial,
+                                                               float* __restrict__ colsum_out, int colsum_blocks) {
+  splitk_reduce_blocks<EPI>((int)blockIdx.x, (int)gridDim.x, M, N, ldc, splits, partial, C, epi, cpartial, colsum_out,
+                            colsum_blocks);
+}
+
+constexpr int kReduceBatchMax = 8;
+struct ReduceBatch {
+  const float* partial[kReduceBatchMax];
+  const float* cpartial[kReduceBatchMax];
+  float* C[kReduceBatchMax];
+  float* colsum[kReduceBatchMax];
+  int64_t M[kReduceBatchMax], ldc[kReduceBatchMax];
+  int N[kReduceBatchMax], splits[kReduceBatchMax], colsum_blocks[kReduceBatchMax];
+  unsigned first[kReduceBatchMax + 1];
+  int count;
+};
+__global__ __launch_bounds__(kBlock) void splitk_reduce_batch_kernel(const ReduceBatch b) {
+  int i = 0;
+#pragma unroll
+  for (int j = 1; j < kReduceBatchMax; ++j)
+    if (j < b.count && blockIdx.x >= b.first[j]) i = j;
+  const EpiArgs none{};
+  splitk_reduce_blocks<REC_EPI_NONE>((int)(blockIdx.x - b.first[i]), (int)(b.first[i + 1] - b.first[i]), b.M[i], b.N[i],
+                                     b.ldc[i], b.splits[i], b.partial[i], b.C[i], none, b.cpartial[i], b.colsum[i],
+                                     b.colsum_blocks[i]);
 }
 
 __global__ __launch_bounds__(kBlock) void colsum_reduce_kernel(int N, int splits,
@@ -748,24 +779,36 @@
                      d->n, (int64_t)d->ldc, p.splits, partial, C, e, cpart, colsum_out, cblocks);
 }
 
+static void defer_reduce(rec_gemm_reduce_job* job, const rec_gemm_desc* d, int splits, const float* partial, float* C,
+                         const float* cpart = nullptr, float* colsum_out = nullptr) {
+  job->partial = partial;
+  job->colsum_partial = cpart && colsum_out ? cpart : nullptr;
+  job->c = C;
+  job->colsum = cpart && colsum_out ? colsum_out : nullptr;
+  job->m = d->m; job->n = d->n; job->ldc = d->ldc;
+  job->splits = splits;
+}
+
+static int sane_cus(const rec_gemm_desc* d) { return d->num_cus > 0 && d->num_cus <= device_cus() ? d->num_cus : 0; }
+
 static bool x3_dw_eligible(const rec_gemm_desc* d, X3DwPlan* pl) {
   const char* v = getenv("REC_GEMM_BF16X3");
   const bool forced = !(v && *v == '1');
   const char* vd = getenv("REC_GEMM_BF16X3_DW");
   if (vd && *vd == '0') return false;
-  if (!x3_enabled() || !d->trans_a || d->trans_b || (d->split_k != 0 && !forced && d->num_cus <= 0) ||
+  if (!x3_enabled() || !d->trans_a || d->trans_b || (d->split_k != 0 && !forced && sane_cus(d) <= 0) ||
       d->epilogue != REC_EPI_NONE)
     return false;
   if (d->k < 8192 || d->m < 336 || d->m > 448 || d->n < 336 || d->n > 416) return false;
   if (d->lda % 4 || d->ldb % 4 || d->ldc % 4) return false;
-  const int cus = d->num_cus > 0 && d->num_cus < device_cus() ? d->num_cus : device_cus();
+  const int cus = sane_cus(d) > 0 ? sane_cus(d) : device_cus();
   return x3_dw_plan((int)d->m, d->n, d->k, cus, pl);
 }
 static size_t x3_dw_bytes(const rec_gemm_desc* d, const X3DwPlan& pl) {
   return align_up((size_t)pl.slices * d->m * d->ldc * sizeof(float), 256) + align_up((size_t)pl.slices * d->n * sizeof(float), 256);
 }
 static bool launch_x3_dw(const rec_gemm_desc* d, const float* A, const float* B, float* C, const EpiArgs& e, float* b_colsum,
-                         void* workspace, size_t workspace_bytes, hipStream_t st) {
+                         void* workspace, size_t workspace_bytes, hipStream_t st, rec_gemm_reduce_job* job = nullptr) {
   X3DwPlan pl;
   if (!x3_dw_eligible(d, &pl)) return false;
   if (((uintptr_t)A) % 16 || ((uintptr_t)B) % 16 || ((uintptr_t)C) % 16) return false;
@@ -776,7 +819,10 @@
     return false;
   GemmPlan sp{};
   sp.splits = pl.slices;
-  launch_reduce<REC_EPI_NONE>(d, sp, partial, C, e, st, b_colsum ? cpart : nullptr, b_colsum);
+  if (job)
+    defer_reduce(job, d, pl.slices, partial, C, b_colsum ? cpart : nullptr, b_colsum);
+  else
+    launch_reduce<REC_EPI_NONE>(d, sp, partial, C, e, st, b_colsum ? cpart : nullptr, b_colsum);
   set_route(REC_GEMM_ROUTE_X3_DW, -1, pl.slices);
   return true;
 }
@@ -860,6 +906,38 @@
   return REC_OK;
 }
 
+extern "C" int rec_gemm_reduce_batch(int32_t count, const rec_gemm_reduce_job* jobs, void* stream) {
+  REC_REQUIRE(count >= 0 && (count == 0 || jobs), REC_EINVAL, "bad arguments");
+  ReduceBatch b{};
+  int64_t blocks = 0;
+  auto flush = [&]() -> int {
+    if (b.count == 0) return REC_OK;
+    b.first[b.count] = (unsigned)blocks;
+    hipLaunchKernelGGL(splitk_reduce_batch_kernel, dim3((unsigned)blocks), dim3(kBlock), 0, (hipStream_t)stream, b);
+    b = ReduceBatch{};
+    blocks = 0;
+    return check_launch("rec_gemm_reduce_batch");
+  };
+  for (int32_t at = 0; at < count; ++at) {
+    const rec_gemm_reduce_job& j = jobs[at];
+    REC_REQUIRE(j.splits >= 0 && j.m >= 0 && j.n >= 0 && j.ldc >= j.n, REC_EINVAL, "job %d: bad sizes", at);
+    if (j.splits == 0 || j.m == 0 || j.n == 0) continue;
+    REC_REQUIRE(j.partial && j.c && (j.colsum_partial == nullptr) == (j.colsum == nullptr), REC_EINVAL,
+                "job %d: null pointer", at);
+    int64_t grid = (j.m * j.n + kBlock - 1) / kBlock;
+    if (grid > kNumCU * 8) grid = kNumCU * 8;
+    const int cblocks = j.colsum ? (j.n + kBlock - 1) / kBlock : 0;
+    const int i = b.count++;
+    b.partial[i] = j.partial; b.cpartial[i] = j.colsum_partial; b.C[i] = j.c; b.colsum[i] = j.colsum;
+    b.M[i] = j.m; b.ldc[i] = j.ldc; b.N[i] = j.n; b.splits[i] = j.splits; b.colsum_blocks[i] = cblocks;
+    b.first[i] = (unsigned)blocks;
+    blocks += grid + cblocks;
+    if (b.count == kReduceBatchMax)
+      if (int rc = flush()) return rc;
+  }
+  return flush();
+}
+
 extern "C" int rec_gemm_last_route(rec_gemm_route* out) {
   REC_REQUIRE(out, REC_EINVAL, "out is NULL");
   *out = g_gemm_route;
@@ -890,6 +968,8 @@
                       ((desc1->epilogue == REC_EPI_RELU_MASK || desc1->epilogue == REC_EPI_DSIGMOID) && y1->aux0 &&
                        y1->ld_aux0 >= desc1->n)) &&
                      !y1->b_colsum;
+  if (y0->defer_reduce) *y0->defer_reduce = rec_gemm_reduce_job{};
+  if (y1->defer_reduce) *y1->defer_reduce = rec_gemm_reduce_job{};
   if (shape) {
     EpiArgs e0{}, e1{};
     e1.aux0 = y1->aux0;
@@ -933,6 +1013,14 @@
   REC_REQUIRE(epi != REC_EPI_MOE || (x->row_scale && x->row_scale_stride >= 1), REC_EINVAL,
               "epilogue needs row_scale");
   hipStream_t st = (hipStream_t)stream;
+  rec_gemm_reduce_job* job = epi == REC_EPI_NONE ? x->defer_reduce : nullptr;
+  if (job) {
+    *job = rec_gemm_reduce_job{};
+    size_t need = 0;
+    if (int rc = rec_gemm_f32_workspace_bytes(desc, &need)) return rc;
+    REC_REQUIRE(need == 0 || (workspace && workspace_bytes >= need), REC_EWORKSPACE, "workspace %zu < %zu (deferred reduce)",
+                workspace_bytes, need);
+  }
   static const int nt_env = [] { const char* v = getenv("REC_GEMM_NT_STORE"); return v && *v ? atoi(v) : 0; }();
   const int nt_store = nt_env == 2 || (nt_env == 1 && epi == REC_EPI_RELU_MASK) ? 1 : 0;
   EpiArgs e{bias, aux0, aux1, x->row_scale, x->out2, ld_aux0, ld_aux1, x->row_scale_stride, x->ld_out2, nt_store, relu_bits};
@@ -969,14 +1057,18 @@
                        (int64_t)desc->ldc, part, b_colsum ? cpart2 : nullptr);
     GemmPlan sp;
     sp.splits = z;
-    launch_reduce<REC_EPI_NONE>(desc, sp, part, C, e, st);
-    if (b_colsum)
-      hipLaunchKernelGGL(colsum_reduce_kernel, dim3((desc->n + kBlock - 1) / kBlock), dim3(kBlock), 0, st,
-                         desc->n, z, (const float*)cpart2, b_colsum);
+    if (job) {
+      defer_reduce(job, desc, z, part, C, cpart2, b_colsum);
+    } else {
+      launch_reduce<REC_EPI_NONE>(desc, sp, part, C, e, st);
+      if (b_colsum)
+        hipLaunchKernelGGL(colsum_reduce_kernel, dim3((desc->n + kBlock - 1) / kBlock), dim3(kBlock), 0, st,
+                           desc->n, z, (const float*)cpart2, b_colsum);
+    }
     set_route(REC_GEMM_ROUTE_SKINNY_DW, -1, z);
     return check_launch("rec_gemm_f32 (skinny dW)");
   }
-  if (launch_x3_dw(desc, A, B, C, e, b_colsum, workspace, workspace_bytes, st)) return check_launch("rec_gemm_f32 (bf16x3 dW)");
+  if (launch_x3_dw(desc, A, B, C, e, b_colsum, workspace, workspace_bytes, st, job)) return check_launch("rec_gemm_f32 (bf16x3 dW)");
   if (!b_colsum && launch_x3(desc, A, B, C, e, x->b_image, workspace, workspace_bytes, st)) {
     set_route(REC_GEMM_ROUTE_X3);
     return check_launch("rec_gemm_f32 (bf16x3)");
@@ -1011,7 +1103,8 @@
   case E:                                                                 \
     if (partial) {                                                        \
       launch_epi<REC_EPI_NONE>(desc, p, A, B, C, e, partial, cpart, st);  \
-      if (!skip_reduce) launch_reduce<E>(desc, p, partial, C, e, st, cpart, b_colsum); \
+      if (job) defer_reduce(job, desc, p.splits, partial, C, cpart, b_colsum); \
+      else if (!skip_reduce) launch_reduce<E>(desc, p, partial, C, e, st, cpart, b_colsum); \
     } else {                                                              \
       launch_epi<E>(desc, p, A, B, C, e, nullptr, cpart, st);             \
     }                                                                     \
diff --git a/paddlerec_amd/deepfm.py b/paddlerec_amd/deepfm.py
--- a/paddlerec_amd/deepfm.py
+++ b/paddlerec_amd/deepfm.py
@@ -477,6 +477,14 @@
             if getattr(self, "_dw_stream", None) is None:
                 self._dw_stream, self._ws_dw = self.k.concurrent_stream(self.device), self.k.Workspace(self.device)
             kw.update(dw_stream=self._dw_stream, dw_ws=self._ws_dw)
+        reduces = None
+        if (overlap and not defer_all and not small and not pipe and B >= 16384 and allreduce is None
+                and "dw_stream" not in kw and hasattr(self.k, "GemmReduceBatch")
+                and os.environ.get("REC_DEFER_REDUCE", "1") != "0"):
+            reduces = getattr(self, "_reduces", None)
+            if reduces is None:
+                reduces = self._reduces = self.k.GemmReduceBatch(self.device, self.n_linear)
+            kw.update(defer_reduce=reduces)
         with self._timed("mlp_bwd"):
             if fused_head:
                 res = self.k.mlp_backward(g_head, acts, mlp_w[:-1], mlp_dw[:-1], self.mlp_db[:-1], self.ws_mlp, **kw,
@@ -532,6 +540,8 @@
         def tail_dense():
             with self._timed("mlp_bwd_dw0"):
                 finish_dw0()
+                if reduces is not None:
+                    reduces.run()
                 self._fold_backward()
             if allreduce is not None:
                 allreduce(self.dense.grad)
diff --git a/paddlerec_amd/ops.py b/paddlerec_amd/ops.py
--- a/paddlerec_amd/ops.py
+++ b/paddlerec_amd/ops.py
@@ -2671,8 +2671,27 @@
         return self.images[i]
 
 
+class GemmReduceBatch:
+
+    def __init__(self, device, slots):
+        self.jobs = (_lib.GemmReduceJob * slots)()
+        self.ws = [Workspace(device) for _ in range(slots)]
+        self.used = 0
+
+    def job(self, i):
+        self.used = max(self.used, i + 1)
+        return C.addressof(self.jobs[i])
+
+    def run(self):
+        n, self.used = self.used, 0
+        if n:
+            check(lib().rec_gemm_reduce_batch(n, self.jobs, _stream()), "rec_gemm_reduce_batch")
+            C.memset(self.jobs, 0, C.sizeof(self.jobs))
+
+
 def gemm(A, B, ws, trans_a=False, trans_b=False, epilogue="none", bias=None, aux0=None, aux1=None,
-         out=None, split_k=0, b_colsum=None, row_scale=None, out2=None, num_cus=0, b_image=None, relu_bits=None):
+         out=None, split_k=0, b_colsum=None, row_scale=None, out2=None, num_cus=0, b_image=None, relu_bits=None,
+         defer_reduce=None):
     d, x, out, need = _gemm_prepare(A, B, trans_a, trans_b, epilogue, bias, aux0, aux1, out, split_k, b_colsum, row_scale,
                                     out2, num_cus, b_image)
     if relu_bits is not None:
@@ -2687,6 +2706,10 @@
             x.relu_bits = relu_bits.data_ptr()
             if _recorder is not None:
                 _recorder.keep.append(relu_bits)
+    if defer_reduce is not None:
+        batch, slot = defer_reduce
+        x.defer_reduce = batch.job(slot)
+        ws = batch.ws[slot]
     w = ws.get(need)
     check(lib().rec_gemm_f32(C.byref(d), _p(A), _p(B), _p(out), C.byref(x), _p(w),
                              C.c_size_t(w.numel()), _stream()), "rec_gemm_f32")
@@ -2880,7 +2903,7 @@
 
 
 def mlp_backward(dy, acts, weights, dws, dbs, ws, defer_first=False, defer_all=False, dw_stream=None, dw_ws=None,
-                 defer_split=0, images_t=None, defer_cus=0):
+                 defer_split=0, images_t=None, defer_cus=0, defer_reduce=None):
     n = len(weights)
     g = dy
     imt = (lambda i: images_t[i]) if images_t is not None else (lambda i: None)
@@ -2916,12 +2939,14 @@
             d_in = gemm(g0, weights[0], ws, trans_b=True, b_image=imt(0))
             join()
             return d_in, (lambda: gemm(acts[0], g0, ws, trans_a=True, out=dws[0], b_colsum=dbs[0], split_k=defer_split,
-                                    num_cus=defer_cus))
+                                    num_cus=defer_cus, defer_reduce=(defer_reduce, 0) if defer_reduce is not None else None))
         if dw_stream is not None:
             dw_stream.wait_stream(cur)
             keep.append(g)
             with torch.cuda.stream(dw_stream):
                 gemm(acts[i], g, dw_ws if dw_ws is not None else ws, trans_a=True, out=dws[i], b_colsum=dbs[i])
+        elif defer_reduce is not None:
+            gemm(acts[i], g, ws, trans_a=True, out=dws[i], b_colsum=dbs[i], defer_reduce=(defer_reduce, i))
         else:
             g = linear_backward(acts[i], g, weights[i], ws, dws[i], dbs[i], relu_src=acts[i] if i > 0 else None,
                                 b_image=imt(i), relu_bits=rb(i) if i > 0 else None)
```

New measurement: 44.50 million samples/s (median of 6 runs). Within noise of the previous version (+0.7%).
